# GPUs/goVideoCompressor

Hardware: AMD Instinct MI355X
Metric: encoded frames/sec (whole node), 1080p30->H.264 CRF23 (higher is better)
Workload: dtype uint8 (8-bit 4:2:0 samples, int32 transforms)

## Files before the change

csrc/common/h264_cabac.h:

```cpp
#pragma once
#include <cstddef>
#include <cstdint>

#include "h264_cabac_tables.h"
#include "h264_mb.h"
#include "h264_tables.h"

namespace mivc {
namespace h264 {

#if defined(__HIPCC__) && defined(__HIP_DEVICE_COMPILE__)
MIVC_HD int cabac_clz32(uint32_t v) { return __clz(static_cast<int>(v)); }
#else
MIVC_HD int cabac_clz32(uint32_t v) { return v ? __builtin_clz(v) : 32; }
#endif

struct CabacBuf {
  uint8_t* p;
  size_t cap;
  size_t n;
  int overflow;
  MIVC_HD void put(int b) {
    if (n < cap) p[n] = static_cast<uint8_t>(b);
    else overflow = 1;
// ... 963 lines not shown
    nbits += 3;
    drain();
    if (nbits > 0) {
      low <<= 8 - nbits;
      nbits = 8;
      drain();
    }
    out.finish();
  }
};

template <class Sink>
struct CabacPendingOut {
  Sink sink;
  int pend = -1, nff = 0;
  MIVC_HD bool byte9(uint32_t v) {
    const int b = static_cast<int>(v & 0xFFu);
    bool ok = true;
    if (v >> 8) {
      if (pend < 0) ok = false;
      if (nff > 0) {
        sink.put(pend + 1);
        for (int k = 0; k < nff - 1; ++k) sink.put(0);
        pend = 0;
        nff = 0;
      } else {
        pend += 1;
      }
    }
    if (b == 0xFF) {
      ++nff;
    } else {
      if (pend >= 0) {
        sink.put(pend);
        for (int k = 0; k < nff; ++k) sink.put(0xFF);
      }
      pend = b;
      nff = 0;
    }
    return ok;
  }
  MIVC_HD void finish() {
    if (pend >= 0) sink.put(pend);
    for (int k = 0; k < nff; ++k) sink.put(0xFF);
    pend = -1;
    nff = 0;
  }
};

struct CabacBufRef {
  CabacBuf* b;
  MIVC_HD void put(int v) { b->put(v); }
};

struct CabacSliceStats {
  int skipped = 0, intra = 0, inter = 0;
};

MIVC_HD size_t cabac_write_slice_data(const CabacSliceInfo& si, CabacNb* nb, uint8_t* states, CabacBuf* out,
                                      const MbHeader* hdr, const int16_t* coef, int n, CabacEncoder* enc_out = nullptr,
                                      CabacSliceStats* st = nullptr) {
  const int end = si.first_mb + n;
  for (int a = si.first_mb; a < end; ++a)
    cabac_prepare_mb(si, hdr, a, cabac_block_mask(hdr[a], coef + static_cast<size_t>(a) * kCoefPerMb), nb[a]);
  cabac_qp_chain(si, nb, n);
  CabacEncoder e;
  cabac_init_contexts(states, si.slice_type == SLICE_I ? 0 : 1 , si.slice_qp);
  e.init(states, out);
  CabacMbCoder<CabacEncoder> coder(e, si, nb);
  for (int a = si.first_mb; a < end; ++a) {
    coder.code_mb(a, hdr[a], coef + static_cast<size_t>(a) * kCoefPerMb, a == end - 1);
    if (st) {
      if (nb[a].skip) ++st->skipped;
      else if (mbk_is_intra(nb[a].kind)) ++st->intra;
      else ++st->inter;
    }
  }
  if (enc_out) *enc_out = e;
  return out->n;
}

inline size_t cabac_write_slice_data_symbols(const CabacSliceInfo& si, CabacNb* nb, uint8_t* states, CabacBuf* out,
                                             const MbHeader* hdr, const int16_t* coef, int n, uint16_t* syms,
                                             size_t cap_syms, int* nsyms_out) {
  const int end = si.first_mb + n;
  for (int a = end - 1; a >= si.first_mb; --a)
    cabac_prepare_mb(si, hdr, a, cabac_block_mask(hdr[a], coef + static_cast<size_t>(a) * kCoefPerMb), nb[a]);
  cabac_qp_chain(si, nb, n);
  size_t total = 0;
  for (int a = si.first_mb; a < end; ++a) {
    CabacSymbolPacker<CabacCountEmit> cnt;
    CabacMbCoder<CabacSymbolPacker<CabacCountEmit>> c1(cnt, si, nb);
    c1.code_mb(a, hdr[a], coef + static_cast<size_t>(a) * kCoefPerMb, a == end - 1);
    cnt.flush_bypass();
    if (total + cnt.out.n > cap_syms) return 0;
    CabacSymbolPacker<CabacStoreEmit> st;
    st.out.p = syms + total;
    CabacMbCoder<CabacSymbolPacker<CabacStoreEmit>> c2(st, si, nb);
    c2.code_mb(a, hdr[a], coef + static_cast<size_t>(a) * kCoefPerMb, a == end - 1);
    st.flush_bypass();
    total += st.out.n;
  }
  if (nsyms_out) *nsyms_out = static_cast<int>(total);
  if (total == 0 || syms[total - 1] != 0xC001u) return 0;
  cabac_init_contexts(states, si.slice_type == SLICE_I ? 0 : 1, si.slice_qp);
  CabacSymbolCoder<CabacPendingOut<CabacBufRef>> e;
  e.out.sink.b = out;
  e.init();
  for (size_t i = 0; i + 1 < total; ++i) {
    e.step_nodrain(syms[i], states, 1, &kCabacRangeLPS[0][0], kCabacTransLPS);
    if ((i & 3) == 3) e.drain();
  }
  e.finish();
  return e.bad ? 0 : out->n;
}

}
}
```

csrc/common/h264_mb.h:

```cpp
#pragma once
#include <cstdint>

#include "h264_tables.h"

namespace mivc {
namespace h264 {

enum SliceType { SLICE_P = 0, SLICE_B = 1, SLICE_I = 2 };

enum MbKind : uint8_t {
  MBK_I4x4 = 0,
  MBK_I16x16 = 1,
  MBK_P16x16 = 2,
  MBK_PSKIP = 3,
  MBK_IPCM = 4,
  MBK_P16x8 = 5,
  MBK_P8x16 = 6,
  MBK_P8x8 = 7,
  MBK_I8x8 = 8,
  MBK_B16x16 = 9,
  MBK_B16x8 = 10,
  MBK_B8x16 = 11,
  MBK_B8x8 = 12,
  MBK_BDIRECT = 13,
};

MIVC_HD bool mbk_is_intra(int k) { return k == MBK_I4x4 || k == MBK_I16x16 || k == MBK_IPCM || k == MBK_I8x8; }
MIVC_HD bool mbk_is_b(int k) { return k >= MBK_B16x16 && k <= MBK_BDIRECT; }

enum : int {
  COEF_LUMA = 0,
  COEF_LUMA_DC = 256,
  COEF_CHROMA_DC = 272,
  COEF_CHROMA_AC = 280,
  kCoefPerMb = 408,
};

enum : uint8_t {
  MBF_SKIP = 1,
  MBF_T8x8 = 2,
  MBF_SUB4 = 4,
};

enum : int { kSubEntry = 80 };

struct alignas(16) MbHeader {
  uint8_t kind;
  uint8_t cbp;
  int8_t qp;
  uint8_t i16_mode;
  uint8_t chroma_mode;
  uint8_t flags;
  uint8_t sub_direct;
  uint8_t pad0;
  int8_t ref[2][4];
  int16_t mv[2][4][2];
  uint8_t i4_modes[16];
};
static_assert(sizeof(MbHeader) == 64, "MbHeader must stay 64 bytes (GPU kernels write it)");

}
}
```

csrc/host/bindings.cc:

```cpp
#include <pybind11/numpy.h>
#include <pybind11/pybind11.h>
#include <pybind11/stl.h>

#include <atomic>
#include <cstring>
#include <stdexcept>
#include <string>
#include <thread>

#include "../common/h264_enc_math.h"
#include "annexb.h"
#include "cabac_writer.h"
#include "cavlc_writer.h"
#include "cpu_encoder.h"
#include "decode_batch.h"
#include "h264_decoder.h"
#include "hevc_codec.h"
#include "hevc_dec.h"
#include "lowres.h"

namespace mivc {
int selftest_i4_taps(int trials, uint32_t seed);
namespace hevc {
std::vector<uint8_t> hevc_exercise(uint32_t seed);
}
}

namespace py = pybind11;
using namespace mivc;
using namespace mivc::h264;

namespace {

py::bytes to_bytes(const std::vector<uint8_t>& v) {
  return py::bytes(reinterpret_cast<const char*>(v.data()), v.size());
}

template <class T>
T dget(const py::dict& d, const char* k, T def) {
  if (d.contains(k)) return d[k].cast<T>();
  return def;
}

EncoderConfig cfg_from(const py::dict& d) {
  EncoderConfig c;
  c.width = dget<int>(d, "width", 0);
  c.height = dget<int>(d, "height", 0);
  c.fps = dget<double>(d, "fps", 30.0);
  c.qp = dget<int>(d, "qp", 26);
  c.crf = dget<double>(d, "crf", -1.0);
  c.keyint = dget<int>(d, "keyint", 250);
  c.me_range = dget<int>(d, "me_range", 16);
  c.subpel = dget<int>(d, "subpel", 2);
  c.use_i4x4 = dget<int>(d, "i4x4", 1);
  c.deblock = dget<int>(d, "deblock", 1);
  c.chroma_qp_offset = dget<int>(d, "chroma_qp_offset", 0);
  c.vui = dget<int>(d, "vui", 1);
  c.cabac = dget<int>(d, "cabac", 0);
  c.t8x8 = dget<int>(d, "t8x8", 0);
  c.bframes = dget<int>(d, "bframes", 0);
  c.pyramid = dget<int>(d, "pyramid", 0);
  c.refs = dget<int>(d, "refs", 1);
  c.weighted_bipred = dget<int>(d, "weighted_bipred", 0);
  c.weightp = dget<int>(d, "weightp", 0);
  c.constrained_intra = dget<int>(d, "constrained_intra", 0);
  c.level_idc = dget<int>(d, "level_idc", 0);
  c.bit_depth = dget<int>(d, "bit_depth", 8);
  if (c.bit_depth < 8 || c.bit_depth > 14) throw std::runtime_error("bit_depth in 8..14");
  c.bit_depth_chroma = dget<int>(d, "bit_depth_chroma", 0);
  if (c.bit_depth_chroma != 0 && (c.bit_depth_chroma < 8 || c.bit_depth_chroma > 14))
    throw std::runtime_error("bit_depth_chroma in 8..14");
  c.cqm = dget<int>(d, "cqm", 0);
  c.cqm_coded = dget<int>(d, "cqm_coded", 0xFF);
  if (c.cqm < 0 || c.cqm > 3) throw std::runtime_error("cqm in 0..3");
  if (d.contains("cqm4")) {
    auto a = py::array_t<uint8_t, py::array::c_style | py::array::forcecast>::ensure(d["cqm4"]);
    if (!a || a.size() != 96) throw std::runtime_error("cqm4: 6 x 16 weights");
    std::memcpy(c.cqm4, a.data(), 96);
  }
  if (d.contains("cqm8")) {
    auto a = py::array_t<uint8_t, py::array::c_style | py::array::forcecast>::ensure(d["cqm8"]);
    if (!a || a.size() != 128) throw std::runtime_error("cqm8: 2 x 64 weights");
    std::memcpy(c.cqm8, a.data(), 128);
  }
  if (c.refs < 1 || c.refs > 16) throw std::runtime_error("refs must be in 1..16");
  return c;
}

py::dict picture_to_dict(const DecodedPicture& p) {
  py::dict d;
  d["width"] = p.width;
  d["height"] = p.height;
  d["coded_width"] = p.coded_width;
  d["coded_height"] = p.coded_height;
// ... 520 lines not shown
    size_t bits = bw.bit_pos();
    bw.align_zero();
    return py::make_tuple(to_bytes(bw.bytes()), bits, tc);
  });
  m.def("table", [](const std::string& name) {
    std::vector<std::vector<int>> out;
    auto row = [&](const uint8_t* p, int n) { out.emplace_back(p, p + n); };
    if (name == "coeff_token_len") for (int t = 0; t < 4; ++t) row(kCoeffTokenLen[t], 68);
    else if (name == "coeff_token_bits") for (int t = 0; t < 4; ++t) row(kCoeffTokenBits[t], 68);
    else if (name == "chroma_dc_coeff_token") { row(kChromaDcCoeffTokenLen, 20); row(kChromaDcCoeffTokenBits, 20); }
    else if (name == "total_zeros_len") for (int t = 0; t < 15; ++t) row(kTotalZerosLen[t], 16);
    else if (name == "total_zeros_bits") for (int t = 0; t < 15; ++t) row(kTotalZerosBits[t], 16);
    else if (name == "chroma_dc_total_zeros_len") for (int t = 0; t < 3; ++t) row(kChromaDcTotalZerosLen[t], 4);
    else if (name == "chroma_dc_total_zeros_bits") for (int t = 0; t < 3; ++t) row(kChromaDcTotalZerosBits[t], 4);
    else if (name == "run_before_len") for (int t = 0; t < 7; ++t) row(kRunBeforeLen[t], 15);
    else if (name == "run_before_bits") for (int t = 0; t < 7; ++t) row(kRunBeforeBits[t], 15);
    else if (name == "intra_cbp") row(kGolombToIntraCbp, 48);
    else if (name == "inter_cbp") row(kGolombToInterCbp, 48);
    else if (name == "zigzag") row(kZigzag4x4, 16);
    else if (name == "lambda") out.emplace_back(kLambda, kLambda + 52);
    else if (name == "hevc_dct32") {
      for (int k = 0; k < 32; ++k) {
        std::vector<int> r(32);
        for (int n = 0; n < 32; ++n) r[n] = hevc::dct_coef(k, n);
        out.push_back(r);
      }
    }
    else throw std::runtime_error("unknown table " + name);
    return out;
  });

  m.def("selftest_i4_taps", &mivc::selftest_i4_taps);

  m.def("parameter_sets", [](const py::dict& cfg) {
    EncoderConfig c = cfg_from(cfg);
    return to_bytes(write_parameter_sets(make_sps(c), make_pps(c)));
  });

  m.def(
      "write_slice",
      [](const py::dict& cfg, const py::dict& fp, py::array_t<uint8_t, py::array::c_style> hdr,
         py::array_t<int16_t, py::array::c_style> coef) {
        EncoderConfig c = cfg_from(cfg);
        SPS sps = make_sps(c);
        PPS pps = make_pps(c);
        int nmb = sps.width_mbs * sps.height_mbs;
        if (hdr.size() != static_cast<py::ssize_t>(nmb * sizeof(MbHeader))) throw std::runtime_error("header array has wrong size");
        if (coef.size() != static_cast<py::ssize_t>(nmb) * kCoefPerMb) throw std::runtime_error("coef array has wrong size");
        SliceHeader sh = slice_header_from(c, sps, pps, fp);
        const int num = dget<int>(fp, "num_mbs", nmb - sh.first_mb);
        if (sh.first_mb < 0 || num < 1 || sh.first_mb + num > nmb) throw std::runtime_error("write_slice: bad MB range");
        SliceStats st;
        std::vector<uint8_t> nal;
        {
          py::gil_scoped_release rel;
          const MbHeader* mh = reinterpret_cast<const MbHeader*>(hdr.data());
          nal = pps.entropy_coding_mode ? write_slice_nal_cabac(sps, pps, sh, mh, coef.data(), num, &st)
                                        : write_slice_nal(sps, pps, sh, mh, coef.data(), num, &st);
        }
        py::dict stats;
        stats["bits"] = st.bits;
        stats["skipped"] = st.skipped;
        stats["intra"] = st.intra;
        stats["coded_inter"] = st.coded_inter;
        return py::make_tuple(to_bytes(nal), stats);
      },
      py::arg("cfg"), py::arg("frame"), py::arg("hdr"), py::arg("coef"));

  m.def("cabac_slice_data_two_ways", [](const py::dict& cfg, const py::dict& fp, py::array_t<uint8_t, py::array::c_style> hdr,
                                         py::array_t<int16_t, py::array::c_style> coef) {
    EncoderConfig c = cfg_from(cfg);
    c.cabac = 1;
    SPS sps = make_sps(c);
    PPS pps = make_pps(c);
    int nmb = sps.width_mbs * sps.height_mbs;
    if (hdr.size() != static_cast<py::ssize_t>(nmb * sizeof(MbHeader))) throw std::runtime_error("header array has wrong size");
    if (coef.size() != static_cast<py::ssize_t>(nmb) * kCoefPerMb) throw std::runtime_error("coef array has wrong size");
    SliceHeader sh = slice_header_from(c, sps, pps, fp);
    const MbHeader* mh = reinterpret_cast<const MbHeader*>(hdr.data());
    std::vector<uint8_t> a = cabac_slice_data(sps, pps, sh, mh, coef.data(), nmb);
    int nsyms = 0;
    std::vector<uint8_t> b = cabac_slice_data_symbols(sps, pps, sh, mh, coef.data(), nmb, &nsyms);
    return py::make_tuple(to_bytes(a), to_bytes(b), nsyms);
  });

  m.def(
      "decode",
      [](py::bytes data, bool skip_deblock) {
        std::string s = data;
        Decoder dec;
        dec.set_skip_deblock(skip_deblock);
        {
          py::gil_scoped_release rel;
          dec.decode(reinterpret_cast<const uint8_t*>(s.data()), s.size());
          dec.flush();
        }
        py::list out;
        for (const DecodedPicture& p : dec.out()) out.append(picture_to_dict(p));
        return out;
      },
      py::arg("data"), py::arg("skip_deblock") = false);

  m.def(
      "parse",
      [](const std::vector<py::bytes>& segments, int threads) {
        std::vector<std::string> in;
        for (const py::bytes& b : segments) in.emplace_back(b);
        std::vector<ParsedSegment> res;
        {
          py::gil_scoped_release rel;
          res = h264_parse_many(in, threads);
        }
        py::list out;
        for (ParsedSegment& r : res) out.append(segment_to_dict(r));
        return out;
      },
      py::arg("segments"), py::arg("threads") = 1);

  py::class_<H264Batch>(m, "H264Batch")
      .def("__len__", [](const H264Batch& b) { return b.segs.size(); })
      .def("info", [](const H264Batch& b, int i) { return segment_info(b.segs.at(i)); })
      .def("segment", [](H264Batch& b, int i) { return segment_to_dict(b.segs.at(i)); })
      .def("layout",
           [](const H264Batch& b, int t, const std::vector<int>& slots, int nmb) {
             H264StepLayout L = b.layout(t, slots, nmb);
             py::dict d;
             d["hdr"] = L.hdr;
             d["mask"] = L.mask;
             d["off"] = L.off;
             d["bs"] = L.bs;
             d["wp"] = L.wp;
             d["coef"] = L.coef;
             d["sub"] = L.sub;
             d["total"] = L.total;
             return d;
           })
      .def("pack",
           [](const H264Batch& b, int t, const std::vector<int>& slots, int nmb, uintptr_t dst, size_t capacity,
              int threads) {
             H264StepLayout L = b.layout(t, slots, nmb);
             if (L.total > capacity) throw std::invalid_argument("H264Batch.pack: buffer too small");
             py::gil_scoped_release rel;
             b.pack(t, slots, nmb, reinterpret_cast<uint8_t*>(dst), threads);
           },
           py::arg("t"), py::arg("slots"), py::arg("nmb"), py::arg("dst"), py::arg("capacity"), py::arg("threads") = 4);
  m.def(
      "parse_batch",
      [](const std::vector<py::bytes>& segments, int threads) {
        std::vector<std::string> in;
        for (const py::bytes& b : segments) in.emplace_back(b);
        auto* batch = new H264Batch();
        {
          py::gil_scoped_release rel;
          batch->segs = h264_parse_many(in, threads);
        }
        return batch;
      },
      py::arg("segments"), py::arg("threads") = 1, py::return_value_policy::take_ownership);

  m.def("hevc_parameter_sets", [](const py::dict& cfg) { return to_bytes(hevc::hevc_parameter_sets(hevc_cfg_from(cfg))); });
  m.def(
      "hevc_write_slice",
      [](const py::dict& cfg, const py::dict& fp, py::array_t<uint8_t, py::array::c_style> ctu,
         py::array_t<uint8_t, py::array::c_style> cu, py::array_t<int16_t, py::array::c_style> cy,
         py::array_t<int16_t, py::array::c_style> cb, py::array_t<int16_t, py::array::c_style> cr) {
        hevc::HevcConfig c = hevc_cfg_from(cfg);
// ... 593 lines not shown
```

csrc/host/cabac_writer.cc:

```cpp
#include "cabac_writer.h"

#include <stdexcept>

#include "../common/h264_cabac.h"

namespace mivc {
namespace h264 {

std::vector<uint8_t> cabac_slice_data(const SPS& sps, const PPS& pps, const SliceHeader& sh, const MbHeader* mbs,
                                      const int16_t* coef, int num_mbs, SliceStats* stats) {
  if (!pps.entropy_coding_mode) throw std::runtime_error("CABAC writer called with a CAVLC PPS");
  if (sh.cabac_init_idc != 0) throw std::runtime_error("CABAC writer codes cabac_init_idc 0 only");
  if (pps.constrained_intra_pred) throw std::runtime_error("CABAC writer: constrained intra prediction is CAVLC-only");
  const int nmb = sps.width_mbs * sps.height_mbs;
  if (sh.first_mb < 0 || num_mbs <= 0 || sh.first_mb + num_mbs > nmb) throw std::runtime_error("bad MB range");
  for (int a = sh.first_mb; a < sh.first_mb + num_mbs; ++a) {
    const int k = mbs[a].kind;
    if (k == MBK_IPCM) throw std::runtime_error("I_PCM records are not written by the CABAC writer");
    if (sh.slice_type == SLICE_I && !mbk_is_intra(k)) throw std::runtime_error("inter MB in an I slice");
    if (sh.slice_type == SLICE_P && mbk_is_b(k)) throw std::runtime_error("B MB in a P slice");
    if (sh.slice_type == SLICE_B && !mbk_is_intra(k) && !mbk_is_b(k)) throw std::runtime_error("P MB in a B slice");
    if (k == MBK_I8x8 && !pps.transform_8x8_mode) throw std::runtime_error("I8x8 MB without transform_8x8_mode");
  }
  CabacSliceInfo si{};
  si.slice_type = sh.slice_type;
  si.wmb = sps.width_mbs;
  si.hmb = sps.height_mbs;
  si.first_mb = sh.first_mb;
  si.num_ref[0] = sh.num_ref_idx_l0_active;
  si.num_ref[1] = sh.num_ref_idx_l1_active;
  si.t8x8_mode = pps.transform_8x8_mode;
  si.slice_qp = pps.pic_init_qp + sh.slice_qp_delta;
  std::vector<CabacNb> nb(static_cast<size_t>(nmb));
  std::vector<uint8_t> out(static_cast<size_t>(num_mbs) * 160 + 4096);
  uint8_t states[kCabacContexts];
  for (int attempt = 0; attempt < 2; ++attempt) {
    CabacBuf buf{out.data(), out.size(), 0, 0};
    CabacEncoder e;
    CabacSliceStats st{};
    cabac_write_slice_data(si, nb.data(), states, &buf, mbs, coef, num_mbs, &e, &st);
    if (e.bad) throw std::runtime_error("CABAC carry past the start of the slice");
    if (!buf.overflow) {
      out.resize(buf.n);
      if (stats) {
        stats->skipped = st.skipped;
        stats->intra = st.intra;
        stats->coded_inter = st.inter;
      }
      return out;
    }
    out.assign(buf.n + 64, 0);
  }
  throw std::runtime_error("CABAC output buffer overflow");
}

std::vector<uint8_t> cabac_slice_data_symbols(const SPS& sps, const PPS& pps, const SliceHeader& sh, const MbHeader* mbs,
                                              const int16_t* coef, int num_mbs, int* nsyms) {
  const int nmb = sps.width_mbs * sps.height_mbs;
  CabacSliceInfo si{};
  si.slice_type = sh.slice_type;
  si.wmb = sps.width_mbs;
  si.hmb = sps.height_mbs;
  si.first_mb = sh.first_mb;
  si.num_ref[0] = sh.num_ref_idx_l0_active;
  si.num_ref[1] = sh.num_ref_idx_l1_active;
  si.t8x8_mode = pps.transform_8x8_mode;
  si.slice_qp = pps.pic_init_qp + sh.slice_qp_delta;
  std::vector<CabacNb> nb(static_cast<size_t>(nmb));
  std::vector<uint16_t> syms(static_cast<size_t>(num_mbs) * 20000 + 1024);
  std::vector<uint8_t> out(static_cast<size_t>(num_mbs) * 4000 + 4096);
  uint8_t states[kCabacContexts];
  CabacBuf buf{out.data(), out.size(), 0, 0};
  cabac_write_slice_data_symbols(si, nb.data(), states, &buf, mbs, coef, num_mbs, syms.data(), syms.size(), nsyms);
  if (buf.overflow) throw std::runtime_error("CABAC symbol path overflow");
  out.resize(buf.n);
  return out;
}

std::vector<uint8_t> write_slice_nal_cabac(const SPS& sps, const PPS& pps, const SliceHeader& sh, const MbHeader* mbs,
                                           const int16_t* coef, int num_mbs, SliceStats* stats) {
  BitWriter bw;
  write_slice_header(bw, sh, sps, pps);
  while (!bw.byte_aligned()) bw.put_bit(1);
  std::vector<uint8_t> data = cabac_slice_data(sps, pps, sh, mbs, coef, num_mbs, stats);
  bw.append_bytes(data.data(), data.size());
  std::vector<uint8_t> nal;
  nal.reserve(bw.bytes().size() + bw.bytes().size() / 64 + 16);
  append_nal(nal, sh.nal_ref_idc, sh.nal_unit_type, bw.bytes());
  if (stats) stats->bits = static_cast<int>(nal.size() * 8);
  return nal;
}

}
}
```

csrc/host/cabac_writer.h:

```cpp
#pragma once
#include <cstdint>
#include <vector>

#include "../common/h264_mb.h"
#include "cavlc_writer.h"
#include "h264_syntax.h"

namespace mivc {
namespace h264 {

std::vector<uint8_t> write_slice_nal_cabac(const SPS& sps, const PPS& pps, const SliceHeader& sh, const MbHeader* mbs,
                                           const int16_t* coef, int num_mbs, SliceStats* stats = nullptr);

std::vector<uint8_t> cabac_slice_data(const SPS& sps, const PPS& pps, const SliceHeader& sh, const MbHeader* mbs,
                                      const int16_t* coef, int num_mbs, SliceStats* stats = nullptr);

std::vector<uint8_t> cabac_slice_data_symbols(const SPS& sps, const PPS& pps, const SliceHeader& sh, const MbHeader* mbs,
                                              const int16_t* coef, int num_mbs, int* nsyms);

}
}
```

csrc/kernels/bindings_hip.cc:

```cpp
#include <pybind11/pybind11.h>
#include <pybind11/stl.h>

#include <cstdint>
#include <stdexcept>
#include <vector>

#include "../common/hevc_ctu_coder.h"
#include "hevc_decode.h"
#include "route.h"

namespace py = pybind11;

extern "C" {
long long mivc_hevc_entropy_state_bytes(int W, int H);
int mivc_launch_hevc_entropy(const void* pic, int B, const int* qp, const void* ctu, const void* cu, const void* col,
                             const unsigned long long* nzmap, const int16_t* cy, const int16_t* cb, const int16_t* cr,
                             uint8_t* state, long long state_bytes, uint8_t* out, unsigned cap, unsigned* sizes,
                             int* errs, unsigned long long* offs, unsigned long long* offs_host, uint8_t* dst,
                             unsigned long long dst_cap, int* overflow, void* stream, unsigned long long* prof,
                             int* gprog, void* gctx);
int mivc_launch_hevc_decode(const mivc::gpu::HevcDecParams* p, int stage, void* stream);
void mivc_launch_synth(void* y, void* u, void* v, int width, int height, int slots, int frames, int frame0,
                       uint32_t seed, int bit_depth, int slot0, void* stream, int kind);
void mivc_launch_prep(const uint8_t* in_y, const uint8_t* in_u, const uint8_t* in_v, int w, int h,
                      int64_t in_stride_y, int64_t in_stride_c, int nframes, uint8_t* out_y, uint8_t* out_u,
                      uint8_t* out_v, int ow, int oh, int W, int H, void* stream, const int* fsel);
void mivc_launch_rgb_to_i420(const uint8_t* rgb, int w, int h, int nframes, uint8_t* y, uint8_t* u, uint8_t* v,
                             void* stream);
void mivc_launch_me(int B, int wmb, int hmb, const uint8_t* src_y, const uint8_t* ref_y, const int16_t* pred_mv,
                    int16_t* out_mv, int* out_cost, uint8_t* out_pred, int* out_intra_cost, const int* qp, int range,
                    int subpel, uint8_t* hp, const int8_t* aq, int planes_ready, int early_sad, void* stream,
                    const int* gate_cost, int gate_thresh, const int16_t* cost_mv, const void* route, int nbuf,
                    int role, int want, const int16_t* seed_mv);
void mivc_launch_me_ref_select(int B, int wmb, int hmb, int nref, int16_t* mv, int16_t* mv8, int* cost, uint8_t* pred,
                               const int16_t* xmv, const int* xcost, const uint8_t* xpred, int8_t* mref, const int* qp,
                               const int8_t* aq, void* stream, const void* route);
void mivc_launch_b_spatial(int B, int wmb, int hmb, void* hdr, const void* col, const uint8_t* src, const uint8_t* ref1,
                           const uint8_t* hp1, const uint8_t* const* ref0k, const uint8_t* const* hp0k, const int* w1,
                           int nref, uint8_t* pred_out, int* err, void* stream, const int* intra_cost, int* cost,
                           const int* qp, const int8_t* aq, int bias, const void* route, int nbuf);
void mivc_launch_b_direct(int B, int wmb, int hmb, const void* col, const int* dsf, const int* direct_copy, int nref,
                          int16_t* dmv, int8_t* dref, int16_t* pm0, int16_t* pm1, void* stream, const void* route,
                          int nbuf, uint8_t* czero, const int8_t* cmap);
void mivc_launch_b_spatial_exact(int B, int wmb, int hmb, void* hdr, const int* intra_cost, const int* cost,
                                 const uint8_t* czero, uint8_t* fix, void* stream, const void* route, int slice_rows,
                                 int tol);
void mivc_launch_b_spatial_fixup(int B, int wmb, int hmb, const void* hdr, const uint8_t* fix, const uint8_t* ref0,
                                 const uint8_t* hp0, const uint8_t* ref1, const uint8_t* hp1, uint8_t* pred_out,
                                 void* stream, const void* route, int nbuf);
void mivc_launch_p_refine(int B, int wmb, int hmb, const uint8_t* src_y, const uint8_t* ref, const uint8_t* hp,
                          const int16_t* mv_in, int16_t* mv_out, int* cost, const int16_t* pm, uint8_t* pred,
                          const int* qp, const int8_t* aq, void* stream, const void* route, int nbuf,
                          const uint8_t* chg_in, uint8_t* chg_out);
void mivc_launch_b_decide(int B, int wmb, int hmb, const uint8_t* src_y, const uint8_t* ref0, const uint8_t* ref1,
                          const uint8_t* hp0, const uint8_t* hp1, const int16_t* mv0, const int16_t* mv1,
                          const int* cost0, const int* cost1, const uint8_t* pred0, const uint8_t* pred1,
                          const int16_t* pm0, const int16_t* pm1, const int16_t* dmv, const int* qp, const int8_t* aq,
                          void* hdr, uint8_t* pred_out, int* cost_out, void* stream, const int* w1, int nref,
                          const int8_t* dref, const uint8_t* const* ref0k, const uint8_t* const* hp0k,
                          int direct_only, int bparts, int have_direct, int spatial, int dbias, const void* route,
                          int nbuf, const uint8_t* czero);
void mivc_launch_aq_offsets(int B, int wmb, int hmb, const uint8_t* sy, const uint8_t* su, const uint8_t* sv,
                            float strength, const float* extra, long long extra_stride, int8_t* out, void* stream,
                            const void* route);
void mivc_launch_mbtree(int B, int F, int lbw, int lbh, const int* blk_cost, const int* blk_mv, void* prop,
                        float strength, float* out, void* stream);
void mivc_launch_qp_fixup(int B, int wmb, int hmb, void* hdr, const int16_t* coef, const uint8_t* nz, uint8_t* flags,
                          const int* slice_qp, void* stream, int slice_rows, const uint8_t* pre, const void* route);
int mivc_launch_prep_aq(const uint8_t* in_y, const uint8_t* in_u, const uint8_t* in_v, int w, int h, int64_t in_stride_y,
                        int64_t in_stride_c, int B, uint8_t* out_y, uint8_t* out_u, uint8_t* out_v, int W, int H,
                        const int* fsel, float strength, const float* extra, long long extra_stride, int8_t* out,
                        void* stream, const void* route);
void mivc_launch_aq_terms(int B, int wmb, int hmb, const uint8_t* sy, const uint8_t* su, const uint8_t* sv, float* terms,
                          void* stream);
void mivc_launch_aq_auto_finish(int B, int nmb, const float* terms, int mode, float strength, const float* extra,
                                long long extra_stride, int8_t* out, void* stream, const void* route);
int mivc_launch_prep_aq_terms(const uint8_t* in_y, const uint8_t* in_u, const uint8_t* in_v, int w, int h,
                              int64_t in_stride_y, int64_t in_stride_c, int B, uint8_t* out_y, uint8_t* out_u,
                              uint8_t* out_v, int W, int H, const int* fsel, float* terms, void* stream);
void mivc_launch_me_halfpel(int B, int W, int H, const uint8_t* ref_y, uint8_t* hp, void* stream, const void* route,
                            int nbuf);
void mivc_launch_encode_inter(int B, int wmb, int hmb, const uint8_t* src_y, const uint8_t* src_u,
                              const uint8_t* src_v, const uint8_t* ref_y, const uint8_t* ref_u, const uint8_t* ref_v,
                              uint8_t* rec_y, uint8_t* rec_u, uint8_t* rec_v, const uint8_t* pred_y,
                              const int16_t* mv, const int* me_cost, const int* intra_cost, const int* qp,
                              int chroma_qp_offset, void* hdr, int16_t* coef, uint8_t* nz, uint8_t* intra_flag,
                              int* intra_count, const int8_t* aq, const uint8_t* ref1_u, const uint8_t* ref1_v,
                              int bmode, int t8, const int16_t* mv8, void* stream, const int* w1, int nref,
                              const uint8_t* const* xref_u, const uint8_t* const* xref_v, const int8_t* mref,
                              const int* wp, int trellis, float trellis_lambda, const void* route, int nbuf,
                              uint8_t* qp_flags);
void mivc_launch_wp_stats16(const uint16_t* y, const uint16_t* u, const uint16_t* v, int w, int h, int npics,
                            unsigned long long* out, void* stream);
void mivc_launch_wp_stats(const uint8_t* y, const uint8_t* u, const uint8_t* v, int w, int h, int npics,
                          unsigned long long* out, void* stream);
void mivc_launch_wp_src(const uint8_t* src, uint8_t* dst, const int* wt, int B, long long plane_bytes, void* stream);
void mivc_launch_p_part8(int B, int wmb, int hmb, const uint8_t* src_y, const uint8_t* ref, const uint8_t* hp,
                         const int16_t* mv, const int16_t* pm, int* cost, uint8_t* pred, int16_t* mv8, const int* qp,
                         const int8_t* aq, int overhead, int min_satd, void* stream, const void* route, int nbuf,
                         const int* bits16, const uint8_t* dir16);
void mivc_launch_encode_intra(int B, int wmb, int hmb, const uint8_t* src_y, const uint8_t* src_u,
                              const uint8_t* src_v, uint8_t* rec_y, uint8_t* rec_u, uint8_t* rec_v, const int* qp,
                              int chroma_qp_offset, void* hdr, int16_t* coef, uint8_t* nz,
                              const uint8_t* intra_flag, const int* intra_count, int* err, int use_i4x4,
                              const int8_t* aq, void* stream, int use_i8x8, const void* route, int nbuf,
                              int slice_rows, int trellis, float trellis_lambda, int* gprog, long long gprog_ints);
void mivc_launch_deblock(int B, int wmb, int hmb, uint8_t* rec_y, uint8_t* rec_u, uint8_t* rec_v, const void* hdr,
                         const uint8_t* nz, int chroma_qp_offset, int alpha_off, int beta_off, int* err,
                         void* stream, const void* route, int nbuf);
void mivc_launch_decode_picture_dpb(int B, int wmb, int hmb, int dpb_n, uint8_t* dpb_y, uint8_t* dpb_u, uint8_t* dpb_v,
                                    const int16_t* cur_idx, const int16_t* reftab, const int16_t* wp, const int16_t* sub,
                                    const void* hdr, const uint32_t* mask, const uint32_t* off,
                                    const int16_t* coef, const int8_t* run, int any_inter, int chroma_qp_offset,
                                    uint8_t* nz, int* err, void* stream);
void mivc_launch_deblock_dpb(int B, int wmb, int hmb, int dpb_n, uint8_t* dpb_y, uint8_t* dpb_u, uint8_t* dpb_v,
                             const int16_t* cur_idx, const void* hdr, const uint8_t* nz, const uint8_t* bs,
                             int chroma_qp_offset, int alpha_off, int beta_off, int* err, void* stream);
void mivc_launch_decode_picture_dpb16(int B, int wmb, int hmb, int dpb_n, uint16_t* dpb_y, uint16_t* dpb_u,
                                      uint16_t* dpb_v, const int16_t* cur_idx, const int16_t* reftab, const int16_t* wp,
                                      const int16_t* sub, const void* hdr, const uint32_t* mask, const uint32_t* off,
                                      const int16_t* coef, const int8_t* run, int any_inter, int chroma_qp_offset, int bd,
                                      uint8_t* nz, int* err, void* stream);
void mivc_launch_deblock_dpb16(int B, int wmb, int hmb, int dpb_n, uint16_t* dpb_y, uint16_t* dpb_u, uint16_t* dpb_v,
                               const int16_t* cur_idx, const void* hdr, const uint8_t* bs, int chroma_qp_offset,
                               int alpha_off, int beta_off, int bd, int* err, void* stream);
int mivc_launch_scale(const void* in, int w, int h, long long in_stride, long long in_pitch, void* out, int ow, int oh,
                      int W, int H, long long out_stride, long long out_pitch, int nframes, const int* fx,
                      const int16_t* cx, int tx, const int* fy, const int16_t* cy, int ty, int tile_w, int tile_h,
                      int in_cols, int in_rows, int bd, void* stream);
void mivc_launch_hevc_intra(int B, int W, int H, const uint16_t* sy, const uint16_t* su, const uint16_t* sv,
                            uint16_t* ry, uint16_t* ru, uint16_t* rv, void* ctu, void* cu, int16_t* cy, int16_t* cu_,
                            int16_t* cv, const int* qp, const int8_t* run, int* cand, int bd, int analyze, int recon,
                            int* err, int sdh, const uint8_t* ctb_mask, void* stream, int ctu64);
void mivc_launch_hevc_inter(int B, int W, int H, const uint16_t* sy, const uint16_t* su, const uint16_t* sv,
                            const uint16_t* fy, const uint16_t* fu, const uint16_t* fv, uint16_t* ry, uint16_t* ru,
                            uint16_t* rv, void* ctu, void* cu, int16_t* cy, int16_t* cu_, int16_t* cv, const int* qp,
                            const int8_t* run, const int* cand, const int16_t* mv, const int* me_cost, int bd,
                            int tu_split, int sdh, int intra_bias, void* stream, const int16_t* mvb,
                            const uint8_t* dirb, const uint16_t* f1y, const uint16_t* f1u, const uint16_t* f1v,
                            const int16_t* wp, const uint16_t* const* xref, const int16_t* mv8);
void mivc_launch_hevc_b(int mode, int B, int wmb, int hmb, const uint8_t* src_y, const uint8_t* ref0, const uint8_t* ref1,
                        const uint8_t* hp0, const uint8_t* hp1, const int16_t* mv0, const int16_t* mv1, const int* cost0,
                        const int* cost1, const int16_t* pm0, const int16_t* pm1, const int16_t* tmv, const uint8_t* tdir,
                        const int16_t* mvb_in, const uint8_t* dir_in, int16_t* mvb_out, uint8_t* dir_out, int* cost,
                        int* bits, const int* qp, const int8_t* aq, void* stream, int bslice, int max_merge, int ctu64, const uint8_t* chg_in, uint8_t* chg_out,
                        int nref0, const uint8_t* const* xref, const uint8_t* const* xhp, const int16_t* xmv,
                        const int* xcost, const int16_t* xpm);
void mivc_launch_hevc_deblock(int B, int W, int H, int bd, uint16_t* y, uint16_t* u, uint16_t* v, const void* cu,
                              const void* ctu, const int8_t* run, void* stream);
void mivc_launch_hevc_aq(int B, int W, int H, int bd, const uint16_t* sy, const uint16_t* su, const uint16_t* sv,
                         const int* qp, float strength, const float* extra, long long extra_stride, int extra_rows,
                         int* ctb_qp, int8_t* mb_aq, void* stream);
void mivc_launch_hevc_pack_levels(int B, int W, int H, const int16_t* cy, const int16_t* cb, const int16_t* cr,
                                  unsigned long long* nzmap, int* cnt, unsigned* off, long long cap_blocks, int16_t* out,
                                  int* err, void* stream);
void mivc_launch_hevc_merge_refine(int B, int wmb, int hmb, const uint8_t* src_y, const uint8_t* ref, const uint8_t* hp,
                                   const int16_t* mv_in, int16_t* mv_out, int* cost, const int16_t* pm, const int* qp,
                                   const int8_t* aq, void* stream);
void mivc_launch_hevc_aq_terms(int B, int W, int H, int bd, const uint16_t* sy, const uint16_t* su, const uint16_t* sv,
                               float* terms, void* stream);
void mivc_launch_hevc_aq_auto_finish(int B, int W, int H, const float* terms, const int* qp, int mode, float strength,
                                     const float* extra, long long extra_stride, int extra_rows, int* ctb_qp,
                                     int8_t* mb_aq, void* stream);
void mivc_launch_hevc_qp_fixup(int B, int W, int H, void* ctu, const void* cu, const int* qp, const int8_t* run,
                               int wpp, void* stream, int ctu64);
void mivc_launch_hevc_sao(int B, int W, int H, int bd, const uint16_t* dy, const uint16_t* du, const uint16_t* dv,
                          uint16_t* y, uint16_t* u, uint16_t* v, const uint16_t* sy, const uint16_t* su,
                          const uint16_t* sv, void* ctu, const int* qp, const int8_t* run, int enable, void* stream, int ctu64);
size_t mivc_cavlc_mb_bytes();
size_t mivc_cabac_nb_bytes();
int mivc_cabac_gap();
void mivc_launch_cabac_bin(int B, int wmb, int hmb, const void* hdr, const int16_t* coef, uint32_t* mask, void* nb,
                           int* cnt, long long* off, int* tot, uint16_t* pool, long long pool_cap,
                           long long* pool_used, long long* base, int* total, const int* slot_qp, int slice_type,
                           int num_ref_l0, int num_ref_l1, int t8x8_mode, int* err, void* stream, const void* route,
                           int slice_rows);
void mivc_launch_cabac_code(int L, int B, uint16_t* pool, const long long* base, const int* total,
                            const uint32_t* hdr_bits, const int* hdr_nbits, const int* slot_qp,
                            unsigned long long itypes, int* bytes, uint8_t* out, long long* out_off, int* err,
                            uint8_t* host_out, long long host_cap, void* stream);
void mivc_launch_cavlc(int B, int wmb, int hmb, const void* hdr, const int16_t* coef, void* mbs, int* len,
                       long long* off, int* trail, long long* total_bits, int* slot_bytes, uint32_t* words,
                       long long cap_words, const uint32_t* hdr_bits, const int* hdr_nbits, int pslice, int slice_qp,
                       const int* slot_qp, uint8_t* out, long long* out_off, const uint8_t* nz, void* stream);
void mivc_launch_satd_blocks(const uint8_t* src, const uint8_t* pred, int* out, int n, int mode, void* stream);
void mivc_launch_trellis_blocks(const int* w, int* out, int n, int qp, int mode, int skip_dc, void* stream);
void mivc_launch_sse(int B, int W, int H, int w, int h, const uint8_t* sy, const uint8_t* su, const uint8_t* sv,
                     const uint8_t* ry, const uint8_t* ru, const uint8_t* rv, unsigned long long* sse,
                     float* ssim_sum, void* stream, const void* route, int nbuf);
long long mivc_lookahead_low_bytes(int w, int h, int N);
int mivc_launch_lookahead_multi(const uint8_t* low, int w, int h, int N, int F, const int* blk_cost, const int* blk_mv,
                                int D, int range, unsigned long long* out, void* stream, const float* wt);
int mivc_launch_hevc_prep_frame(int B, const void* sy, const void* su, const void* sv, long long ss_y, long long ss_c,
                                int pitch_y, int pitch_c, int bps, int w, int h, uint16_t* dy, uint16_t* du,
                                uint16_t* dv, uint8_t* d8, int W, int H, int shift, int bd, void* stream);
int mivc_launch_hevc_proxy8(const uint16_t* src, uint8_t* dst, long long n, int shift, void* stream);
int mivc_launch_lookahead(const uint8_t* y, int w, int h, long long fstride, int N, int F, uint8_t* low,
                          unsigned long long* frame_cost, int* blk_cost, int* blk_mv, int range, void* stream,
                          uint8_t* low4, int* mv4, unsigned long long* cost4, float* wt, unsigned long long* wstats,
                          float thr_mean, float thr_scale, int stage);
long long mivc_lookahead_quarter_bytes(int w, int h, int N);
}

namespace {
template <class T>
T* P(uintptr_t p) {
  return reinterpret_cast<T*>(p);
}
void* S(uintptr_t s) { return reinterpret_cast<void*>(s); }
}

PYBIND11_MODULE(_hip, m) {
  m.doc() = "govideocompressor_amd gfx950 kernels (raw-pointer launch shims)";
  m.attr("arch") = "gfx950";
  m.def("route_bytes", []() { return static_cast<int>(sizeof(mivc::gpu::SlotRoute)); });

  m.def("synth", [](uintptr_t y, uintptr_t u, uintptr_t v, int w, int h, int slots, int frames, int frame0,
                    uint32_t seed, uintptr_t stream, int bit_depth, int slot0, int kind) {
    if (bit_depth != 8 && bit_depth != 10) throw std::invalid_argument("synth: bit_depth must be 8 or 10");
    if (kind < 0 || kind > 6) throw std::invalid_argument("synth: content kind 0..6");
    mivc_launch_synth(P<void>(y), P<void>(u), P<void>(v), w, h, slots, frames, frame0, seed, bit_depth, slot0,
                      S(stream), kind);
  }, py::arg("y"), py::arg("u"), py::arg("v"), py::arg("w"), py::arg("h"), py::arg("slots"), py::arg("frames"),
     py::arg("frame0"), py::arg("seed"), py::arg("stream"), py::arg("bit_depth") = 8, py::arg("slot0") = 0,
     py::arg("kind") = 0);
  m.def("prep", [](uintptr_t iy, uintptr_t iu, uintptr_t iv, int w, int h, int64_t sy, int64_t sc, int n,
                   uintptr_t oy, uintptr_t ou, uintptr_t ov, int ow, int oh, int W, int H, uintptr_t stream,
                   uintptr_t fsel) {
    if (ow != w || oh != h) throw std::invalid_argument("prep: resample with ops.scale (scale.hip) first");
    if (W < w || H < h || w < 2 || h < 2) throw std::invalid_argument("prep: bad geometry");
    mivc_launch_prep(P<uint8_t>(iy), P<uint8_t>(iu), P<uint8_t>(iv), w, h, sy, sc, n, P<uint8_t>(oy), P<uint8_t>(ou),
                     P<uint8_t>(ov), ow, oh, W, H, S(stream), P<int>(fsel));
  }, py::arg("iy"), py::arg("iu"), py::arg("iv"), py::arg("w"), py::arg("h"), py::arg("sy"), py::arg("sc"), py::arg("n"),
     py::arg("oy"), py::arg("ou"), py::arg("ov"), py::arg("ow"), py::arg("oh"), py::arg("W"), py::arg("H"),
     py::arg("stream"), py::arg("fsel") = 0);
  m.def("rgb_to_i420", [](uintptr_t rgb, int w, int h, int n, uintptr_t y, uintptr_t u, uintptr_t v,
                          uintptr_t stream) {
    mivc_launch_rgb_to_i420(P<uint8_t>(rgb), w, h, n, P<uint8_t>(y), P<uint8_t>(u), P<uint8_t>(v), S(stream));
  });
  m.def("me", [](int B, int wmb, int hmb, uintptr_t src, uintptr_t ref, uintptr_t pred_mv, uintptr_t out_mv,
                 uintptr_t out_cost, uintptr_t out_pred, uintptr_t out_intra, uintptr_t qp, int range, int subpel,
                 uintptr_t stream, uintptr_t hp, uintptr_t aq, int planes_ready, int early_sad, uintptr_t gate_cost,
                 int gate_thresh, uintptr_t cost_mv, uintptr_t route, int nbuf, int role, int want, uintptr_t seed_mv) {
    if (planes_ready && !hp) throw std::invalid_argument("me: planes_ready needs the hp buffer");
    if (route && (nbuf < 1 || role < 0 || role > 4 || (want != 0 && want != 1) || !planes_ready))
      throw std::invalid_argument("me: a routed search needs nbuf, a role (list-0 0..3 / list-1 4), want P/B and the planes");
    mivc_launch_me(B, wmb, hmb, P<uint8_t>(src), P<uint8_t>(ref), P<int16_t>(pred_mv), P<int16_t>(out_mv),
                   P<int>(out_cost), P<uint8_t>(out_pred), P<int>(out_intra), P<int>(qp), range, subpel,
                   P<uint8_t>(hp), P<int8_t>(aq), planes_ready, early_sad, S(stream), P<int>(gate_cost), gate_thresh,
                   P<int16_t>(cost_mv), P<void>(route), nbuf, role, want, P<int16_t>(seed_mv));
  }, py::arg("B"), py::arg("wmb"), py::arg("hmb"), py::arg("src"), py::arg("ref"), py::arg("pred_mv"),
     py::arg("out_mv"), py::arg("out_cost"), py::arg("out_pred"), py::arg("out_intra"), py::arg("qp"),
     py::arg("range"), py::arg("subpel"), py::arg("stream"), py::arg("hp") = 0, py::arg("aq") = 0,
     py::arg("planes_ready") = 0, py::arg("early_sad") = 0, py::arg("gate_cost") = 0, py::arg("gate_thresh") = 0,
     py::arg("cost_mv") = 0, py::arg("route") = 0, py::arg("nbuf") = 0, py::arg("role") = 0, py::arg("want") = 0,
     py::arg("seed_mv") = 0);
  m.def("me_ref_select", [](int B, int wmb, int hmb, int nref, uintptr_t mv, uintptr_t mv8, uintptr_t cost,
                            uintptr_t pred, uintptr_t xmv, uintptr_t xcost, uintptr_t xpred, uintptr_t mref,
                            uintptr_t qp, uintptr_t aq, uintptr_t stream, uintptr_t route) {
    if (nref < 2 || nref > 4) throw std::invalid_argument("me_ref_select: nref in 2..4");
    mivc_launch_me_ref_select(B, wmb, hmb, nref, P<int16_t>(mv), P<int16_t>(mv8), P<int>(cost), P<uint8_t>(pred),
                              P<int16_t>(xmv), P<int>(xcost), P<uint8_t>(xpred), P<int8_t>(mref), P<int>(qp),
                              P<int8_t>(aq), S(stream), P<void>(route));
  }, py::arg("B"), py::arg("wmb"), py::arg("hmb"), py::arg("nref"), py::arg("mv"), py::arg("mv8"), py::arg("cost"),
     py::arg("pred"), py::arg("xmv"), py::arg("xcost"), py::arg("xpred"), py::arg("mref"), py::arg("qp"), py::arg("aq"),
     py::arg("stream"), py::arg("route") = 0);
  m.def("b_spatial", [](int B, int wmb, int hmb, uintptr_t hdr, uintptr_t col, uintptr_t src, uintptr_t ref1,
                        uintptr_t hp1, std::vector<uintptr_t> ref0k, std::vector<uintptr_t> hp0k, std::vector<int> w1,
                        uintptr_t pred_out, uintptr_t err, uintptr_t stream, uintptr_t intra_cost, uintptr_t cost,
                        uintptr_t qp, uintptr_t aq, int bias, uintptr_t route, int nbuf) {
    const size_t n = ref0k.size();
    if (n < 1 || n > 4 || hp0k.size() != n || w1.size() != n)
      throw std::invalid_argument("b_spatial: 1..4 list-0 pictures with planes and weights");
    if (hmb > 272 || wmb > 480) throw std::invalid_argument("b_spatial: at most 272 MB rows and 480 columns");
    const uint8_t* rk[4];
    const uint8_t* hk[4];
    for (size_t i = 0; i < n; ++i) {
      rk[i] = P<uint8_t>(ref0k[i]);
      hk[i] = P<uint8_t>(hp0k[i]);
    }
    mivc_launch_b_spatial(B, wmb, hmb, P<void>(hdr), P<void>(col), P<uint8_t>(src), P<uint8_t>(ref1), P<uint8_t>(hp1),
                          rk, hk, w1.data(), static_cast<int>(n), P<uint8_t>(pred_out), P<int>(err), S(stream),
                          P<int>(intra_cost), P<int>(cost), P<int>(qp), P<int8_t>(aq), bias, P<void>(route), nbuf);
  }, py::arg("B"), py::arg("wmb"), py::arg("hmb"), py::arg("hdr"), py::arg("col"), py::arg("src"), py::arg("ref1"),
     py::arg("hp1"), py::arg("ref0k"), py::arg("hp0k"), py::arg("w1"), py::arg("pred_out"), py::arg("err"),
     py::arg("stream"), py::arg("intra_cost"), py::arg("cost"), py::arg("qp"), py::arg("aq"), py::arg("bias"),
     py::arg("route") = 0, py::arg("nbuf") = 0);
  m.def("b_direct", [](int B, int wmb, int hmb, uintptr_t col, std::vector<int> dsf, std::vector<int> direct_copy,
                       uintptr_t dmv, uintptr_t pm0, uintptr_t pm1, uintptr_t stream, uintptr_t dref, uintptr_t route,
                       int nbuf, uintptr_t czero, uintptr_t cmap) {
    if (dsf.empty() || dsf.size() > 4 || dsf.size() != direct_copy.size())
      throw std::invalid_argument("b_direct: one (dsf, direct_copy) pair per list-0 picture, at most 4");
    if (route && nbuf < 1) throw std::invalid_argument("b_direct: a routed launch needs the pool size");
    if (cmap && !dref) throw std::invalid_argument("b_direct: a co-located map needs the dref output");
    mivc_launch_b_direct(B, wmb, hmb, P<void>(col), dsf.data(), direct_copy.data(), static_cast<int>(dsf.size()),
                         P<int16_t>(dmv), P<int8_t>(dref), P<int16_t>(pm0), P<int16_t>(pm1), S(stream), P<void>(route),
                         nbuf, P<uint8_t>(czero), P<int8_t>(cmap));
// ... 48 lines not shown
      hk[i] = P<uint8_t>(hp0k[i - 1]);
    }
    mivc_launch_b_decide(B, wmb, hmb, P<uint8_t>(src), P<uint8_t>(ref0), P<uint8_t>(ref1), P<uint8_t>(hp0),
                         P<uint8_t>(hp1), P<int16_t>(mv0), P<int16_t>(mv1), P<int>(cost0), P<int>(cost1),
                         P<uint8_t>(pred0), P<uint8_t>(pred1), P<int16_t>(pm0), P<int16_t>(pm1), P<int16_t>(dmv),
                         P<int>(qp), P<int8_t>(aq), P<void>(hdr), P<uint8_t>(pred_out), P<int>(cost_out), S(stream),
                         w1.data(), static_cast<int>(n), (n > 1 || route) ? P<int8_t>(dref) : nullptr, rk, hk, direct_only,
                         bparts, have_direct, spatial, dbias, P<void>(route), nbuf, P<uint8_t>(czero));
  }, py::arg("B"), py::arg("wmb"), py::arg("hmb"), py::arg("src"), py::arg("ref0"), py::arg("ref1"), py::arg("hp0"),
     py::arg("hp1"), py::arg("mv0"), py::arg("mv1"), py::arg("cost0"), py::arg("cost1"), py::arg("pred0"),
     py::arg("pred1"), py::arg("pm0"), py::arg("pm1"), py::arg("dmv"), py::arg("qp"), py::arg("aq"), py::arg("hdr"),
     py::arg("pred_out"), py::arg("cost_out"), py::arg("stream"), py::arg("w1") = std::vector<int>{32},
     py::arg("dref") = 0, py::arg("ref0k") = std::vector<uintptr_t>{}, py::arg("hp0k") = std::vector<uintptr_t>{},
     py::arg("direct_only") = 0, py::arg("bparts") = 0, py::arg("have_direct") = 0, py::arg("spatial") = 0, py::arg("dbias") = 0,
     py::arg("route") = 0, py::arg("nbuf") = 0, py::arg("czero") = 0);
  m.def("aq_offsets", [](int B, int wmb, int hmb, uintptr_t sy, uintptr_t su, uintptr_t sv, float strength,
                         uintptr_t out, uintptr_t stream, uintptr_t extra, long long extra_stride, uintptr_t route) {
    mivc_launch_aq_offsets(B, wmb, hmb, P<uint8_t>(sy), P<uint8_t>(su), P<uint8_t>(sv), strength, P<float>(extra),
                           extra_stride, P<int8_t>(out), S(stream), P<void>(route));
  }, py::arg("B"), py::arg("wmb"), py::arg("hmb"), py::arg("sy"), py::arg("su"), py::arg("sv"), py::arg("strength"),
     py::arg("out"), py::arg("stream"), py::arg("extra") = 0, py::arg("extra_stride") = 0, py::arg("route") = 0);
  m.def("mbtree", [](int B, int F, int lbw, int lbh, uintptr_t blk_cost, uintptr_t blk_mv, uintptr_t prop,
                     float strength, uintptr_t out, uintptr_t stream) {
    mivc_launch_mbtree(B, F, lbw, lbh, P<int>(blk_cost), P<int>(blk_mv), P<void>(prop), strength, P<float>(out),
                       S(stream));
  });
  m.def("qp_fixup", [](int B, int wmb, int hmb, uintptr_t hdr, uintptr_t coef, uintptr_t nz, uintptr_t flags,
                       uintptr_t slice_qp, uintptr_t stream, int slice_rows, uintptr_t pre, uintptr_t route) {
    if ((pre != 0) != (route != 0)) throw std::invalid_argument("qp_fixup: pre and route go together");
    mivc_launch_qp_fixup(B, wmb, hmb, P<void>(hdr), P<int16_t>(coef), P<uint8_t>(nz), P<uint8_t>(flags),
                         P<int>(slice_qp), S(stream), slice_rows, P<uint8_t>(pre), P<void>(route));
  }, py::arg("B"), py::arg("wmb"), py::arg("hmb"), py::arg("hdr"), py::arg("coef"), py::arg("nz"), py::arg("flags"),
     py::arg("slice_qp"), py::arg("stream"), py::arg("slice_rows") = 0, py::arg("pre") = 0, py::arg("route") = 0);
  m.def("prep_aq", [](uintptr_t iy, uintptr_t iu, uintptr_t iv, int w, int h, int64_t sy, int64_t sc, int n,
                      uintptr_t oy, uintptr_t ou, uintptr_t ov, int W, int H, float strength, uintptr_t out,
                      uintptr_t stream, uintptr_t fsel, uintptr_t extra, long long extra_stride, uintptr_t route) {
    if (W < w || H < h || w < 2 || h < 2) throw std::invalid_argument("prep_aq: bad geometry");
    if (!out) throw std::invalid_argument("prep_aq: needs the offset buffer");
    return mivc_launch_prep_aq(P<uint8_t>(iy), P<uint8_t>(iu), P<uint8_t>(iv), w, h, sy, sc, n, P<uint8_t>(oy),
                               P<uint8_t>(ou), P<uint8_t>(ov), W, H, P<int>(fsel), strength, P<float>(extra),
                               extra_stride, P<int8_t>(out), S(stream), P<void>(route)) != 0;
  }, py::arg("iy"), py::arg("iu"), py::arg("iv"), py::arg("w"), py::arg("h"), py::arg("sy"), py::arg("sc"), py::arg("n"),
     py::arg("oy"), py::arg("ou"), py::arg("ov"), py::arg("W"), py::arg("H"), py::arg("strength"), py::arg("out"),
     py::arg("stream"), py::arg("fsel") = 0, py::arg("extra") = 0, py::arg("extra_stride") = 0, py::arg("route") = 0);
  m.def("aq_terms", [](int B, int wmb, int hmb, uintptr_t sy, uintptr_t su, uintptr_t sv, uintptr_t terms,
                       uintptr_t stream) {
    if (B < 1 || wmb < 1 || hmb < 1) throw std::invalid_argument("aq_terms: bad geometry");
    if (!sy || !su || !sv || !terms) throw std::invalid_argument("aq_terms: needs the planes and the term buffer");
    mivc_launch_aq_terms(B, wmb, hmb, P<uint8_t>(sy), P<uint8_t>(su), P<uint8_t>(sv), P<float>(terms), S(stream));
  }, py::arg("B"), py::arg("wmb"), py::arg("hmb"), py::arg("sy"), py::arg("su"), py::arg("sv"), py::arg("terms"),
     py::arg("stream"));
  m.def("prep_aq_terms", [](uintptr_t iy, uintptr_t iu, uintptr_t iv, int w, int h, int64_t sy, int64_t sc, int n,
                            uintptr_t oy, uintptr_t ou, uintptr_t ov, int W, int H, uintptr_t terms, uintptr_t stream,
                            uintptr_t fsel) {
    if (W < w || H < h || w < 2 || h < 2 || n < 1) throw std::invalid_argument("prep_aq_terms: bad geometry");
    if (!terms) throw std::invalid_argument("prep_aq_terms: needs the term buffer");
    return mivc_launch_prep_aq_terms(P<uint8_t>(iy), P<uint8_t>(iu), P<uint8_t>(iv), w, h, sy, sc, n, P<uint8_t>(oy),
                                     P<uint8_t>(ou), P<uint8_t>(ov), W, H, P<int>(fsel), P<float>(terms),
                                     S(stream)) != 0;
  }, py::arg("iy"), py::arg("iu"), py::arg("iv"), py::arg("w"), py::arg("h"), py::arg("sy"), py::arg("sc"), py::arg("n"),
     py::arg("oy"), py::arg("ou"), py::arg("ov"), py::arg("W"), py::arg("H"), py::arg("terms"), py::arg("stream"),
     py::arg("fsel") = 0);
  m.def("aq_auto_finish", [](int B, int nmb, uintptr_t terms, int mode, float strength, uintptr_t out, uintptr_t stream,
                             uintptr_t extra, long long extra_stride, uintptr_t route) {
    if (B < 1 || nmb < 1) throw std::invalid_argument("aq_auto_finish: bad geometry");
    if (mode != 2 && mode != 3) throw std::invalid_argument("aq_auto_finish: mode must be 2 or 3");
    if (!terms || !out) throw std::invalid_argument("aq_auto_finish: needs the term and the offset buffer");
    mivc_launch_aq_auto_finish(B, nmb, P<float>(terms), mode, strength, P<float>(extra), extra_stride, P<int8_t>(out),
                               S(stream), P<void>(route));
  }, py::arg("B"), py::arg("nmb"), py::arg("terms"), py::arg("mode"), py::arg("strength"), py::arg("out"),
     py::arg("stream"), py::arg("extra") = 0, py::arg("extra_stride") = 0, py::arg("route") = 0);
  m.def("me_halfpel", [](int B, int W, int H, uintptr_t ref, uintptr_t hp, uintptr_t stream, uintptr_t route, int nbuf) {
    if (route && nbuf < 1) throw std::invalid_argument("me_halfpel: a routed launch needs the pool size");
    mivc_launch_me_halfpel(B, W, H, P<uint8_t>(ref), P<uint8_t>(hp), S(stream), P<void>(route), nbuf);
  }, py::arg("B"), py::arg("W"), py::arg("H"), py::arg("ref"), py::arg("hp"), py::arg("stream"), py::arg("route") = 0,
     py::arg("nbuf") = 0);
  m.def("encode_inter",
        [](int B, int wmb, int hmb, uintptr_t sy, uintptr_t su, uintptr_t sv, uintptr_t fy, uintptr_t fu,
           uintptr_t fv, uintptr_t ry, uintptr_t ru, uintptr_t rv, uintptr_t pred, uintptr_t mv, uintptr_t me_cost,
           uintptr_t intra_cost, uintptr_t qp, int cqo, uintptr_t hdr, uintptr_t coef, uintptr_t nz,
           uintptr_t intra_flag, uintptr_t intra_count, uintptr_t stream, uintptr_t aq, uintptr_t ref1_u,
           uintptr_t ref1_v, int bmode, int t8, uintptr_t mv8, std::vector<int> w1, std::vector<uintptr_t> xref_u,
           std::vector<uintptr_t> xref_v, uintptr_t mref, uintptr_t wp, int trellis, float trellis_lambda,
           uintptr_t route, int nbuf, uintptr_t qp_flags) {
          if (bmode && (!ref1_u || !ref1_v)) throw std::invalid_argument("encode_inter: B mode needs the list-1 chroma");
          const size_t n = xref_u.size() + 1;
          if (n > 4 || xref_v.size() != xref_u.size()) throw std::invalid_argument("encode_inter: at most 4 list-0 pictures");
          if ((n > 1 || route) && !bmode && !mref)
            throw std::invalid_argument("encode_inter: P pictures with several references need mref");
          if (route && (nbuf < 1 || n > 1)) throw std::invalid_argument("encode_inter: routed launches take pools");
          std::vector<int> w(n, w1.empty() ? 32 : w1[0]);
          for (size_t i = 0; i < n && i < w1.size(); ++i) w[i] = w1[i];
          const uint8_t* xu[4] = {nullptr, nullptr, nullptr, nullptr};
          const uint8_t* xv[4] = {nullptr, nullptr, nullptr, nullptr};
          for (size_t i = 1; i < n; ++i) {
            xu[i] = P<uint8_t>(xref_u[i - 1]);
            xv[i] = P<uint8_t>(xref_v[i - 1]);
          }
          mivc_launch_encode_inter(B, wmb, hmb, P<uint8_t>(sy), P<uint8_t>(su), P<uint8_t>(sv), P<uint8_t>(fy),
                                   P<uint8_t>(fu), P<uint8_t>(fv), P<uint8_t>(ry), P<uint8_t>(ru), P<uint8_t>(rv),
                                   P<uint8_t>(pred), P<int16_t>(mv), P<int>(me_cost), P<int>(intra_cost), P<int>(qp),
                                   cqo, P<void>(hdr), P<int16_t>(coef), P<uint8_t>(nz), P<uint8_t>(intra_flag),
                                   P<int>(intra_count), P<int8_t>(aq), P<uint8_t>(ref1_u), P<uint8_t>(ref1_v), bmode,
                                   t8, P<int16_t>(mv8), S(stream), w.data(), static_cast<int>(n), xu, xv,
                                   bmode ? nullptr : P<int8_t>(mref), P<int>(wp), trellis, trellis_lambda, P<void>(route),
                                   nbuf, P<uint8_t>(qp_flags));
        }, py::arg("B"), py::arg("wmb"), py::arg("hmb"), py::arg("sy"), py::arg("su"), py::arg("sv"), py::arg("fy"),
        py::arg("fu"), py::arg("fv"), py::arg("ry"), py::arg("ru"), py::arg("rv"), py::arg("pred"), py::arg("mv"),
        py::arg("me_cost"), py::arg("intra_cost"), py::arg("qp"), py::arg("cqo"), py::arg("hdr"), py::arg("coef"),
        py::arg("nz"), py::arg("intra_flag"), py::arg("intra_count"), py::arg("stream"), py::arg("aq") = 0,
        py::arg("ref1_u") = 0, py::arg("ref1_v") = 0, py::arg("bmode") = 0, py::arg("t8") = 0, py::arg("mv8") = 0,
        py::arg("w1") = std::vector<int>{32}, py::arg("xref_u") = std::vector<uintptr_t>{},
        py::arg("xref_v") = std::vector<uintptr_t>{}, py::arg("mref") = 0, py::arg("wp") = 0, py::arg("trellis") = 0,
        py::arg("trellis_lambda") = 1.0f, py::arg("route") = 0, py::arg("nbuf") = 0, py::arg("qp_flags") = 0);
  m.def("wp_stats16", [](uintptr_t y, uintptr_t u, uintptr_t v, int w, int h, int npics, uintptr_t out, uintptr_t stream) {
    if (w % 2 || h % 2 || npics <= 0) throw std::invalid_argument("wp_stats16: even picture sizes, npics > 0");
    mivc_launch_wp_stats16(P<uint16_t>(y), P<uint16_t>(u), P<uint16_t>(v), w, h, npics, P<unsigned long long>(out),
                           S(stream));
  });
  m.def("wp_stats", [](uintptr_t y, uintptr_t u, uintptr_t v, int w, int h, int npics, uintptr_t out, uintptr_t stream) {
    if (w % 2 || h % 2 || (w * h) % 4) throw std::invalid_argument("wp_stats: even picture sizes");
    mivc_launch_wp_stats(P<uint8_t>(y), P<uint8_t>(u), P<uint8_t>(v), w, h, npics, P<unsigned long long>(out),
                         S(stream));
  });
  m.def("wp_src", [](uintptr_t src, uintptr_t dst, uintptr_t wt, int B, long long plane_bytes, uintptr_t stream) {
    if (plane_bytes % 4) throw std::invalid_argument("wp_src: plane size must be a multiple of 4");
    mivc_launch_wp_src(P<uint8_t>(src), P<uint8_t>(dst), P<int>(wt), B, plane_bytes, S(stream));
  });
  m.def("p_part8", [](int B, int wmb, int hmb, uintptr_t src, uintptr_t ref, uintptr_t hp, uintptr_t mv, uintptr_t pm,
                      uintptr_t cost, uintptr_t pred, uintptr_t mv8, uintptr_t qp, uintptr_t aq, int overhead,
                      int min_satd, uintptr_t stream, uintptr_t route, int nbuf, uintptr_t bits16, uintptr_t dir16) {
    if (!hp || !mv8) throw std::invalid_argument("p_part8: needs the half-sample planes and an mv8 buffer");
    if (!pred && !bits16) throw std::invalid_argument("p_part8: the H.264 form rewrites pred");
    mivc_launch_p_part8(B, wmb, hmb, P<uint8_t>(src), P<uint8_t>(ref), P<uint8_t>(hp), P<int16_t>(mv), P<int16_t>(pm),
                        P<int>(cost), P<uint8_t>(pred), P<int16_t>(mv8), P<int>(qp), P<int8_t>(aq), overhead, min_satd,
                        S(stream), P<void>(route), nbuf, P<int>(bits16), P<uint8_t>(dir16));
  }, py::arg("B"), py::arg("wmb"), py::arg("hmb"), py::arg("src"), py::arg("ref"), py::arg("hp"), py::arg("mv"),
     py::arg("pm"), py::arg("cost"), py::arg("pred"), py::arg("mv8"), py::arg("qp"), py::arg("aq"), py::arg("overhead"),
     py::arg("min_satd"), py::arg("stream"), py::arg("route") = 0, py::arg("nbuf") = 0, py::arg("bits16") = 0,
     py::arg("dir16") = 0);
  m.def("encode_intra", [](int B, int wmb, int hmb, uintptr_t sy, uintptr_t su, uintptr_t sv, uintptr_t ry,
                           uintptr_t ru, uintptr_t rv, uintptr_t qp, int cqo, uintptr_t hdr, uintptr_t coef,
                           uintptr_t nz, uintptr_t intra_flag, uintptr_t intra_count, uintptr_t err, int use_i4x4,
                           uintptr_t stream, uintptr_t aq, int use_i8x8, uintptr_t route, int nbuf, int slice_rows,
                           int trellis, float trellis_lambda, uintptr_t gprog, long long gprog_ints) {
    mivc_launch_encode_intra(B, wmb, hmb, P<uint8_t>(sy), P<uint8_t>(su), P<uint8_t>(sv), P<uint8_t>(ry),
                             P<uint8_t>(ru), P<uint8_t>(rv), P<int>(qp), cqo, P<void>(hdr), P<int16_t>(coef),
                             P<uint8_t>(nz), P<uint8_t>(intra_flag), P<int>(intra_count), P<int>(err), use_i4x4,
                             P<int8_t>(aq), S(stream), use_i8x8, P<void>(route), nbuf, slice_rows, trellis,
                             trellis_lambda, P<int>(gprog), gprog_ints);
  }, py::arg("B"), py::arg("wmb"), py::arg("hmb"), py::arg("sy"), py::arg("su"), py::arg("sv"), py::arg("ry"),
     py::arg("ru"), py::arg("rv"), py::arg("qp"), py::arg("cqo"), py::arg("hdr"), py::arg("coef"), py::arg("nz"),
     py::arg("intra_flag"), py::arg("intra_count"), py::arg("err"), py::arg("use_i4x4"), py::arg("stream"),
     py::arg("aq") = 0, py::arg("use_i8x8") = 0, py::arg("route") = 0, py::arg("nbuf") = 0, py::arg("slice_rows") = 0,
     py::arg("trellis") = 0, py::arg("trellis_lambda") = 1.0f, py::arg("gprog") = 0, py::arg("gprog_ints") = 0);
  m.def("deblock", [](int B, int wmb, int hmb, uintptr_t ry, uintptr_t ru, uintptr_t rv, uintptr_t hdr, uintptr_t nz,
                      int cqo, int alpha_off, int beta_off, uintptr_t err, uintptr_t stream, uintptr_t route, int nbuf) {
    mivc_launch_deblock(B, wmb, hmb, P<uint8_t>(ry), P<uint8_t>(ru), P<uint8_t>(rv), P<void>(hdr), P<uint8_t>(nz),
                        cqo, alpha_off, beta_off, P<int>(err), S(stream), P<void>(route), nbuf);
  }, py::arg("B"), py::arg("wmb"), py::arg("hmb"), py::arg("ry"), py::arg("ru"), py::arg("rv"), py::arg("hdr"),
     py::arg("nz"), py::arg("cqo"), py::arg("alpha_off"), py::arg("beta_off"), py::arg("err"), py::arg("stream"),
     py::arg("route") = 0, py::arg("nbuf") = 0);
  m.def("decode_picture_dpb", [](int B, int wmb, int hmb, int dpb_n, uintptr_t y, uintptr_t u, uintptr_t v,
                                 uintptr_t cur_idx, uintptr_t reftab, uintptr_t wp, uintptr_t sub,
                                 uintptr_t hdr, uintptr_t mask, uintptr_t off, uintptr_t coef, uintptr_t run,
                                 int any_inter, int cqo, uintptr_t nz, uintptr_t err, uintptr_t stream) {
    if (dpb_n < 1 || dpb_n > 32767) throw std::invalid_argument("decode_picture_dpb: dpb_n must be 1..32767");
    mivc_launch_decode_picture_dpb(B, wmb, hmb, dpb_n, P<uint8_t>(y), P<uint8_t>(u), P<uint8_t>(v), P<int16_t>(cur_idx),
                                   P<int16_t>(reftab), P<int16_t>(wp), P<int16_t>(sub), P<void>(hdr),
                                   P<uint32_t>(mask), P<uint32_t>(off), P<int16_t>(coef), P<int8_t>(run), any_inter,
                                   cqo, P<uint8_t>(nz), P<int>(err), S(stream));
  });
  m.def("deblock_dpb", [](int B, int wmb, int hmb, int dpb_n, uintptr_t y, uintptr_t u, uintptr_t v, uintptr_t cur_idx,
                          uintptr_t hdr, uintptr_t nz, uintptr_t bs, int cqo, int alpha_off, int beta_off, uintptr_t err,
                          uintptr_t stream) {
    if (dpb_n < 1 || dpb_n > 32767) throw std::invalid_argument("deblock_dpb: dpb_n must be 1..32767");
    mivc_launch_deblock_dpb(B, wmb, hmb, dpb_n, P<uint8_t>(y), P<uint8_t>(u), P<uint8_t>(v), P<int16_t>(cur_idx),
                            P<void>(hdr), P<uint8_t>(nz), P<uint8_t>(bs), cqo, alpha_off, beta_off, P<int>(err),
                            S(stream));
  });
  m.def("decode_picture_dpb16", [](int B, int wmb, int hmb, int dpb_n, uintptr_t y, uintptr_t u, uintptr_t v,
                                   uintptr_t cur_idx, uintptr_t reftab, uintptr_t wp, uintptr_t sub,
                                   uintptr_t hdr, uintptr_t mask, uintptr_t off, uintptr_t coef, uintptr_t run,
                                   int any_inter, int cqo, int bit_depth, uintptr_t nz, uintptr_t err,
                                   uintptr_t stream) {
    if (dpb_n < 1 || dpb_n > 32767) throw std::invalid_argument("decode_picture_dpb16: dpb_n must be 1..32767");
    if (bit_depth != 9 && bit_depth != 10) throw std::invalid_argument("decode_picture_dpb16: bit_depth must be 9 or 10");
    mivc_launch_decode_picture_dpb16(B, wmb, hmb, dpb_n, P<uint16_t>(y), P<uint16_t>(u), P<uint16_t>(v),
                                     P<int16_t>(cur_idx), P<int16_t>(reftab), P<int16_t>(wp), P<int16_t>(sub),
                                     P<void>(hdr), P<uint32_t>(mask), P<uint32_t>(off), P<int16_t>(coef),
                                     P<int8_t>(run), any_inter, cqo, bit_depth, P<uint8_t>(nz), P<int>(err), S(stream));
  });
  m.def("deblock_dpb16", [](int B, int wmb, int hmb, int dpb_n, uintptr_t y, uintptr_t u, uintptr_t v,
                            uintptr_t cur_idx, uintptr_t hdr, uintptr_t bs, int cqo, int alpha_off, int beta_off,
                            int bit_depth, uintptr_t err, uintptr_t stream) {
    if (dpb_n < 1 || dpb_n > 32767) throw std::invalid_argument("deblock_dpb16: dpb_n must be 1..32767");
    if (bit_depth != 9 && bit_depth != 10) throw std::invalid_argument("deblock_dpb16: bit_depth must be 9 or 10");
// ... 175 lines not shown
  m.def("hevc_qp_fixup", [](int B, int W, int H, uintptr_t ctu, uintptr_t cu, uintptr_t qp, uintptr_t run, int wpp,
                            uintptr_t stream, int ctu64) {
    mivc_launch_hevc_qp_fixup(B, W, H, P<void>(ctu), P<void>(cu), P<int>(qp), P<int8_t>(run), wpp, S(stream), ctu64);
  }, py::arg("B"), py::arg("W"), py::arg("H"), py::arg("ctu"), py::arg("cu"), py::arg("qp"), py::arg("run"),
     py::arg("wpp"), py::arg("stream"), py::arg("ctu64") = 0);
  m.def("hevc_sao", [](int B, int W, int H, int bd, uintptr_t dy, uintptr_t du, uintptr_t dv, uintptr_t y, uintptr_t u,
                       uintptr_t v, uintptr_t sy, uintptr_t su, uintptr_t sv, uintptr_t ctu, uintptr_t qp, uintptr_t run,
                       int enable, uintptr_t stream, int ctu64) {
    mivc_launch_hevc_sao(B, W, H, bd, P<uint16_t>(dy), P<uint16_t>(du), P<uint16_t>(dv), P<uint16_t>(y), P<uint16_t>(u),
                         P<uint16_t>(v), P<uint16_t>(sy), P<uint16_t>(su), P<uint16_t>(sv), P<void>(ctu), P<int>(qp),
                         P<int8_t>(run), enable, S(stream), ctu64);
  }, py::arg("B"), py::arg("W"), py::arg("H"), py::arg("bd"), py::arg("dy"), py::arg("du"), py::arg("dv"), py::arg("y"),
     py::arg("u"), py::arg("v"), py::arg("sy"), py::arg("su"), py::arg("sv"), py::arg("ctu"), py::arg("qp"),
     py::arg("run"), py::arg("enable"), py::arg("stream"), py::arg("ctu64") = 0);
  m.def("hevc_decode_stage", [](const py::dict& p, int stage, uintptr_t stream) {
    mivc::gpu::HevcDecParams a{};
    auto I = [&](const char* k) -> long long {
      if (!p.contains(k)) throw std::runtime_error(std::string("hevc_decode_stage: missing ") + k);
      return p[k].cast<long long>();
    };
    auto Q = [&](const char* k) -> uintptr_t { return p.contains(k) ? p[k].cast<uintptr_t>() : 0; };
    a.B = static_cast<int>(I("B"));
    a.W = static_cast<int>(I("W"));
    a.H = static_cast<int>(I("H"));
    a.D = static_cast<int>(I("D"));
    a.bd = static_cast<int>(I("bd"));
    a.bdc = static_cast<int>(I("bdc"));
    a.log2_ctb = static_cast<int>(I("log2_ctb"));
    a.wctb = static_cast<int>(I("wctb"));
    a.hctb = static_cast<int>(I("hctb"));
    const std::vector<uintptr_t> dpb = p["dpb"].cast<std::vector<uintptr_t>>();
    const std::vector<uintptr_t> res = p["res"].cast<std::vector<uintptr_t>>();
    const std::vector<uintptr_t> tmp = p["tmp"].cast<std::vector<uintptr_t>>();
    for (int c = 0; c < 3; ++c) {
      a.dpb[c] = reinterpret_cast<uint16_t*>(dpb.at(c));
      a.res[c] = reinterpret_cast<int16_t*>(res.at(c));
      a.tmp[c] = reinterpret_cast<uint16_t*>(tmp.at(c));
    }
    a.cur = P<int8_t>(Q("cur"));
    a.reftab = P<int8_t>(Q("reftab"));
    a.run = P<int8_t>(Q("run"));
    a.meta = P<int32_t>(Q("meta"));
    a.mvf = P<uint8_t>(Q("mvf"));
    a.mvf_sub = P<uint8_t>(Q("mvf_sub"));
    a.bs = P<uint8_t>(Q("bs"));
    a.ctbs = P<uint8_t>(Q("ctbs"));
    a.sao = P<uint8_t>(Q("sao"));
    a.tus = P<uint8_t>(Q("tus"));
    a.tu_base = P<int32_t>(Q("tu_base"));
    a.coefs = P<int16_t>(Q("coefs"));
    a.coef_base = P<int64_t>(Q("coef_base"));
    a.ops = P<uint8_t>(Q("ops"));
    a.op_base = P<int32_t>(Q("op_base"));
    a.ctb_ops = P<uint32_t>(Q("ctb_ops"));
    a.refs = P<uint8_t>(Q("refs"));
    a.ref_base = P<int32_t>(Q("ref_base"));
    a.slices = P<uint8_t>(Q("slices"));
    a.slice_base = P<int32_t>(Q("slice_base"));
    a.scaling = P<uint8_t>(Q("scaling"));
    a.max_tus = static_cast<int>(I("max_tus"));
    a.err = P<int>(Q("err"));
    if (p.contains("out")) {
      const std::vector<uintptr_t> out = p["out"].cast<std::vector<uintptr_t>>();
      for (int c = 0; c < 3; ++c) a.out[c] = reinterpret_cast<void*>(out.at(c));
      a.out_u8 = static_cast<int>(I("out_u8"));
      a.Fo = static_cast<int>(I("Fo"));
      a.out_w = static_cast<int>(I("out_w"));
      a.out_h = static_cast<int>(I("out_h"));
      a.crop_x = static_cast<int>(I("crop_x"));
      a.crop_y = static_cast<int>(I("crop_y"));
      a.disp = P<int16_t>(Q("disp"));
    }
    if (!a.cur || !a.run || !a.meta || !a.mvf || !a.err) throw std::runtime_error("hevc_decode_stage: null pointer");
    const int r = mivc_launch_hevc_decode(&a, stage, S(stream));
    if (r != 0) throw std::runtime_error("hevc_decode_stage: launch failed (" + std::to_string(r) + ")");
  });
  m.def("cavlc_mb_bytes", []() { return mivc_cavlc_mb_bytes(); });
  m.def("cabac_nb_bytes", []() { return mivc_cabac_nb_bytes(); });
  m.def("cabac_gap", []() { return mivc_cabac_gap(); });
  m.def("cabac_bin", [](int B, int wmb, int hmb, uintptr_t hdr, uintptr_t coef, uintptr_t mask, uintptr_t nb,
                        uintptr_t cnt, uintptr_t off, uintptr_t tot, uintptr_t pool, long long pool_cap,
                        uintptr_t pool_used, uintptr_t base, uintptr_t total, uintptr_t slot_qp, int slice_type,
                        int num_ref_l0, int num_ref_l1, int t8x8_mode, uintptr_t err, uintptr_t stream, uintptr_t route,
                        int slice_rows) {
    if ((pool & 15) != 0) throw std::invalid_argument("cabac_bin: symbol pool must be 16-byte aligned");
    if (B < 1 || wmb < 1 || hmb < 1) throw std::invalid_argument("cabac_bin: bad geometry");
    mivc_launch_cabac_bin(B, wmb, hmb, P<void>(hdr), P<int16_t>(coef), P<uint32_t>(mask), P<void>(nb), P<int>(cnt),
                          P<long long>(off), P<int>(tot), P<uint16_t>(pool), pool_cap, P<long long>(pool_used),
                          P<long long>(base), P<int>(total), P<int>(slot_qp), slice_type, num_ref_l0, num_ref_l1,
                          t8x8_mode, P<int>(err), S(stream), P<void>(route), slice_rows);
  }, py::arg("B"), py::arg("wmb"), py::arg("hmb"), py::arg("hdr"), py::arg("coef"), py::arg("mask"), py::arg("nb"),
     py::arg("cnt"), py::arg("off"), py::arg("tot"), py::arg("pool"), py::arg("pool_cap"), py::arg("pool_used"),
     py::arg("base"), py::arg("total"), py::arg("slot_qp"), py::arg("slice_type"), py::arg("num_ref_l0"),
     py::arg("num_ref_l1"), py::arg("t8x8_mode"), py::arg("err"), py::arg("stream"), py::arg("route") = 0,
     py::arg("slice_rows") = 0);
  m.def("cabac_code", [](int L, int B, uintptr_t pool, uintptr_t base, uintptr_t total, uintptr_t hdr_bits,
                         uintptr_t hdr_nbits, uintptr_t slot_qp, unsigned long long itypes, uintptr_t bytes,
                         uintptr_t out, uintptr_t out_off, uintptr_t err, uintptr_t stream, uintptr_t host_out,
                         long long host_cap) {
    if (B < 1 || L < 1 || L % B != 0 || L / B > 64) throw std::invalid_argument("cabac_code: L must be G * B, G <= 64");
    if ((out & 15) || (host_out & 15)) throw std::invalid_argument("cabac_code: output buffers must be 16-byte aligned");
    mivc_launch_cabac_code(L, B, P<uint16_t>(pool), P<long long>(base), P<int>(total), P<uint32_t>(hdr_bits),
                           P<int>(hdr_nbits), P<int>(slot_qp), itypes, P<int>(bytes), P<uint8_t>(out),
                           P<long long>(out_off), P<int>(err), P<uint8_t>(host_out), host_cap, S(stream));
  });
  m.def("cavlc", [](int B, int wmb, int hmb, uintptr_t hdr, uintptr_t coef, uintptr_t mbs, uintptr_t len, uintptr_t off,
                    uintptr_t trail, uintptr_t total_bits, uintptr_t slot_bytes, uintptr_t words, long long cap_words,
                    uintptr_t hdr_bits, uintptr_t hdr_nbits, int pslice, int slice_qp, uintptr_t slot_qp,
                    uintptr_t out, uintptr_t out_off, uintptr_t stream, uintptr_t nz) {
    mivc_launch_cavlc(B, wmb, hmb, P<void>(hdr), P<int16_t>(coef), P<void>(mbs), P<int>(len), P<long long>(off),
                      P<int>(trail), P<long long>(total_bits), P<int>(slot_bytes), P<uint32_t>(words), cap_words,
                      P<uint32_t>(hdr_bits), P<int>(hdr_nbits), pslice, slice_qp, P<int>(slot_qp), P<uint8_t>(out),
                      P<long long>(out_off), P<uint8_t>(nz), S(stream));
  }, py::arg("B"), py::arg("wmb"), py::arg("hmb"), py::arg("hdr"), py::arg("coef"), py::arg("mbs"), py::arg("len"),
     py::arg("off"), py::arg("trail"), py::arg("total_bits"), py::arg("slot_bytes"), py::arg("words"),
     py::arg("cap_words"), py::arg("hdr_bits"), py::arg("hdr_nbits"), py::arg("pslice"), py::arg("slice_qp"),
     py::arg("slot_qp"), py::arg("out"), py::arg("out_off"), py::arg("stream"), py::arg("nz") = 0);
  m.def("sse", [](int B, int W, int H, int w, int h, uintptr_t sy, uintptr_t su, uintptr_t sv, uintptr_t ry,
                  uintptr_t ru, uintptr_t rv, uintptr_t sse, uintptr_t ssim, uintptr_t stream, uintptr_t route, int nbuf) {
    if (B <= 0 || W <= 0 || H <= 0 || W % 16 || H % 2) throw std::invalid_argument("sse: coded width must be a multiple of 16, height even");
    if (w < 2 || h < 2 || w > W || h > H || w % 2 || h % 2)
      throw std::invalid_argument("sse: the display window must be even and lie inside the coded size");
    if (route && nbuf < 1) throw std::invalid_argument("sse: a routed launch needs the pool size");
    mivc_launch_sse(B, W, H, w, h, P<uint8_t>(sy), P<uint8_t>(su), P<uint8_t>(sv), P<uint8_t>(ry), P<uint8_t>(ru),
                    P<uint8_t>(rv), P<unsigned long long>(sse), P<float>(ssim), S(stream), P<void>(route), nbuf);
  }, py::arg("B"), py::arg("W"), py::arg("H"), py::arg("w"), py::arg("h"), py::arg("sy"), py::arg("su"), py::arg("sv"),
     py::arg("ry"), py::arg("ru"), py::arg("rv"), py::arg("sse"), py::arg("ssim"), py::arg("stream"),
     py::arg("route") = 0, py::arg("nbuf") = 0);
  m.def("satd_blocks", [](uintptr_t src, uintptr_t pred, uintptr_t out, int n, int mode, uintptr_t stream) {
    if (n <= 0) throw std::invalid_argument("satd_blocks: n must be positive");
    mivc_launch_satd_blocks(P<uint8_t>(src), P<uint8_t>(pred), P<int>(out), n, mode, S(stream));
  });
  m.def("trellis_blocks", [](uintptr_t w, uintptr_t out, int n, int qp, int mode, int skip_dc, uintptr_t stream) {
    if (n <= 0 || qp < 0 || qp > 51) throw std::invalid_argument("trellis_blocks: n > 0, 0 <= qp <= 51");
    mivc_launch_trellis_blocks(P<int>(w), P<int>(out), n, qp, mode, skip_dc, S(stream));
  });
  m.def("lookahead_low_bytes", [](int w, int h, int n) { return mivc_lookahead_low_bytes(w, h, n); });
  m.def("lookahead_quarter_bytes", [](int w, int h, int n) { return mivc_lookahead_quarter_bytes(w, h, n); });
  m.def("lookahead_multi", [](uintptr_t low, int w, int h, int n, int f, uintptr_t blk_cost, uintptr_t blk_mv, int D,
                              int range, uintptr_t out, uintptr_t stream, uintptr_t wt) {
    const int r = mivc_launch_lookahead_multi(P<uint8_t>(low), w, h, n, f, P<int>(blk_cost), P<int>(blk_mv), D, range,
                                              P<unsigned long long>(out), S(stream), P<float>(wt));
    if (r != 0) throw std::invalid_argument("lookahead_multi: bad arguments (" + std::to_string(r) + ")");
  }, py::arg("low"), py::arg("w"), py::arg("h"), py::arg("n"), py::arg("f"), py::arg("blk_cost"), py::arg("blk_mv"),
     py::arg("D"), py::arg("range"), py::arg("out"), py::arg("stream"), py::arg("wt") = 0);
  m.def("lookahead", [](uintptr_t y, int w, int h, long long fstride, int n, int f, uintptr_t low, uintptr_t frame_cost,
                        uintptr_t blk_cost, int range, uintptr_t stream, uintptr_t blk_mv, uintptr_t low4, uintptr_t mv4,
                        uintptr_t cost4, uintptr_t wt, uintptr_t wstats, float thr_mean, float thr_scale, int stage) {
    int rc = mivc_launch_lookahead(P<uint8_t>(y), w, h, fstride, n, f, P<uint8_t>(low),
                                   P<unsigned long long>(frame_cost), P<int>(blk_cost), P<int>(blk_mv), range,
                                   S(stream), P<uint8_t>(low4), P<int>(mv4), P<unsigned long long>(cost4), P<float>(wt),
                                   P<unsigned long long>(wstats), thr_mean, thr_scale, stage);
    if (rc != 0) throw std::invalid_argument("lookahead: bad geometry or range (4, 6, 8)");
  }, py::arg("y"), py::arg("w"), py::arg("h"), py::arg("fstride"), py::arg("n"), py::arg("f"), py::arg("low"),
     py::arg("frame_cost"), py::arg("blk_cost"), py::arg("range"), py::arg("stream"), py::arg("blk_mv") = 0,
     py::arg("low4") = 0, py::arg("mv4") = 0, py::arg("cost4") = 0, py::arg("wt") = 0, py::arg("wstats") = 0,
     py::arg("thr_mean") = 2.0f, py::arg("thr_scale") = 0.08f, py::arg("stage") = 3);
}
```

csrc/kernels/cabac.hip:

```cpp
#include "kcommon.h"
#include "../common/h264_cabac.h"

namespace mivc {
namespace gpu {

using h264::CabacNb;
using h264::CabacSliceInfo;
using h264::MbHeader;

constexpr int kCabacGap = 64;
constexpr int kArithReadAhead = 160;

struct CabacBinArgs {
  Geom g;
  const MbHeader* hdr;
  const int16_t* coef;
  uint32_t* mask;
  CabacNb* nb;
  int* cnt;
  long long* off;
  int* tot;
  uint16_t* pool;
  long long pool_cap;
  long long* pool_used;
  long long* base;
  int* total;
  const int* slot_qp;
  int slice_type;
  int num_ref_l0, num_ref_l1;
  int t8x8_mode;
  int* err;
  const SlotRoute* rt;
  int slice_mbs, per_slot;
};

__device__ __forceinline__ int slice_first(const CabacBinArgs& a, int mb) { return (mb / a.slice_mbs) * a.slice_mbs; }
__device__ __forceinline__ int slice_end(const CabacBinArgs& a, int mb) {
  return min(slice_first(a, mb) + a.slice_mbs, a.g.nmb());
}
__device__ __forceinline__ int slice_index(const CabacBinArgs& a, int slot, int mb) {
  return slot * a.per_slot + mb / a.slice_mbs;
}

__device__ __forceinline__ CabacSliceInfo slice_info(const CabacBinArgs& a, int slot, int mb) {
  CabacSliceInfo si{};
  si.slice_type = a.rt ? a.rt[slot].kind : a.slice_type;
  si.wmb = a.g.wmb;
  si.hmb = a.g.hmb;
  si.first_mb = slice_first(a, mb);
  si.num_ref[0] = a.rt ? (a.rt[slot].kind == SK_I ? 1 : a.rt[slot].n0) : a.num_ref_l0;
  si.num_ref[1] = a.num_ref_l1;
  si.t8x8_mode = a.t8x8_mode;
  si.slice_qp = a.slot_qp[slot];
  return si;
}

constexpr int kMaskSpan = 16;

__global__ __launch_bounds__(64) void cabac_mask(CabacBinArgs a) {
  const Geom& g = a.g;
  const int lane = threadIdx.x, sub = lane & 31;
  const int slot = blockIdx.y;
  for (int it = 0; it < kMaskSpan; ++it) {
  const int mb = (blockIdx.x * kMaskSpan + it) * 2 + (lane >> 5);
  if ((blockIdx.x * kMaskSpan + it) * 2 >= g.nmb()) break;
  const bool live = mb < g.nmb();
  const size_t o = static_cast<size_t>(slot) * g.nmb() + (live ? mb : 0);
  const int16_t* c = a.coef + o * h264::kCoefPerMb;
  const bool i16 = a.hdr[o].kind == h264::MBK_I16x16;
  bool nz = false;
  if (sub < 16 || (sub >= 19 && sub < 27)) {
    const int16_t* p = sub < 16 ? c + h264::COEF_LUMA + sub * 16 : c + h264::COEF_CHROMA_AC + (sub - 19) * 16;
    const uint4 q0 = reinterpret_cast<const uint4*>(p)[0];
    const uint4 q1 = reinterpret_cast<const uint4*>(p)[1];
    const bool skip_dc = sub >= 19 || i16;
    nz = ((skip_dc ? (q0.x & 0xFFFF0000u) : q0.x) | q0.y | q0.z | q0.w | q1.x | q1.y | q1.z | q1.w) != 0;
  } else if (sub == 16) {
    const uint4 q0 = reinterpret_cast<const uint4*>(c + h264::COEF_LUMA_DC)[0];
    const uint4 q1 = reinterpret_cast<const uint4*>(c + h264::COEF_LUMA_DC)[1];
    nz = i16 && (q0.x | q0.y | q0.z | q0.w | q1.x | q1.y | q1.z | q1.w) != 0;
  } else if (sub == 17 || sub == 18) {
    const uint2 q = reinterpret_cast<const uint2*>(c + h264::COEF_CHROMA_DC)[sub - 17];
    nz = (q.x | q.y) != 0;
  }
  const unsigned long long bal = __ballot(nz);
  const uint32_t m = static_cast<uint32_t>((bal >> (lane & 32)) & 0x7FFFFFFull);
  if (live && sub == 0) a.mask[o] = m;
  }
}

static_assert(sizeof(CabacNb) % 16 == 0, "CabacNb rows leave as 16-byte chunks");
__global__ __launch_bounds__(64) void cabac_prep(CabacBinArgs a) {
  __shared__ __attribute__((aligned(16))) CabacNb s_nb[64];
  const int mb0 = blockIdx.x * 64, mb = mb0 + threadIdx.x, slot = blockIdx.y, nmb = a.g.nmb();
  const size_t base = static_cast<size_t>(slot) * nmb;
  if (mb < nmb) {
    const CabacSliceInfo si = slice_info(a, slot, mb);
    h264::cabac_prepare_mb(si, a.hdr + base, mb, a.mask[base + mb], s_nb[threadIdx.x]);
  }
  __syncthreads();
  const int n16 = min(64, nmb - mb0) * static_cast<int>(sizeof(CabacNb) / 16);
  const uint4* src = reinterpret_cast<const uint4*>(s_nb);
  uint4* dst = reinterpret_cast<uint4*>(a.nb + base + mb0);
  for (int i = threadIdx.x; i < n16; i += 64) dst[i] = src[i];
}

__device__ __forceinline__ long long wave_scan_add(long long v) {
  const int lane = threadIdx.x & 63;
#pragma unroll
  for (int o = 1; o < 64; o <<= 1) {
    const long long y = __shfl_up(v, o, 64);
    if (lane >= o) v += y;
  }
  return v;
}
__device__ __forceinline__ int wave_scan_max(int v) {
  const int lane = threadIdx.x & 63;
#pragma unroll
  for (int o = 1; o < 64; o <<= 1) {
    const int y = __shfl_up(v, o, 64);
    if (lane >= o) v = max(v, y);
  }
  return v;
}

__global__ __launch_bounds__(64) void cabac_chain(CabacBinArgs a) {
  const int slot = blockIdx.x / a.per_slot, first = (blockIdx.x - slot * a.per_slot) * a.slice_mbs;
  const int n = min(a.g.nmb() - first, a.slice_mbs), lane = threadIdx.x;
  CabacNb* nb = a.nb + static_cast<size_t>(slot) * a.g.nmb() + first;
  const int per = (n + 63) / 64;
  const int i0 = lane * per, i1 = min(n, i0 + per);
  auto has = [&](int i) { return !nb[i].skip && (nb[i].cbp != 0 || nb[i].kind == h264::MBK_I16x16); };
  int ld = -1;
  for (int i = i0; i < i1; ++i)
    if (has(i)) ld = i;
  const int incl = wave_scan_max(ld);
  ld = __shfl_up(incl, 1, 64);
  if (lane == 0) ld = -1;
  int last_qp = ld >= 0 ? nb[ld].qp : a.slot_qp[slot];
  for (int i = i0; i < i1; ++i) {
    if (has(i)) {
      int d = nb[i].qp - last_qp;
      if (d < -26) d += 52;
      if (d > 25) d -= 52;
      nb[i].dqp = static_cast<int8_t>(d);
      last_qp = nb[i].qp;
    } else {
      nb[i].dqp = 0;
    }
  }
  __builtin_amdgcn_fence(__ATOMIC_RELEASE, "workgroup");
  __builtin_amdgcn_wave_barrier();
  __builtin_amdgcn_fence(__ATOMIC_ACQUIRE, "workgroup");
  for (int i = lane; i < n; i += 64)
    nb[i].prev_dqp_nz = static_cast<uint8_t>(i > 0 && has(i - 1) && nb[i - 1].dqp != 0);
}

__global__ __launch_bounds__(64) void cabac_count(CabacBinArgs a) {
  const int mb = blockIdx.x * 64 + threadIdx.x, slot = blockIdx.y, n = a.g.nmb();
  if (mb >= n) return;
  const CabacSliceInfo si = slice_info(a, slot, mb);
  const size_t base = static_cast<size_t>(slot) * n;
  h264::CabacSymbolPacker<h264::CabacCountEmit> s;
  h264::CabacMbCoder<h264::CabacSymbolPacker<h264::CabacCountEmit>> coder(s, si, a.nb + base);
  coder.code_mb(mb, a.hdr[base + mb], a.coef + (base + mb) * h264::kCoefPerMb, mb == slice_end(a, mb) - 1);
  s.flush_bypass();
  a.cnt[base + mb] = s.out.n;
}

__global__ __launch_bounds__(64) void cabac_offsets(CabacBinArgs a) {
// ... 231 lines not shown
    uint4 t[8];
#pragma unroll
    for (int k = 0; k < 8; ++k) t[k] = q[k];
#pragma unroll
    for (int k = 0; k < 8; ++k) my[k] = t[k];
  }
  const int hbytes = a.hdr_nbits[l] >> 3;
  for (int i = 0; i < hbytes; ++i) c.out.put(static_cast<uint8_t>(a.hdr_bits[l * 16 + (i >> 2)] >> (24 - 8 * (i & 3))));
  c.out.start(hbytes);
  c.init();
  const int n = total - 1;
  for (int b0 = 0; b0 < n; b0 += kArithBlock) {
    const uint4* nq = q + (b0 >> 3) + 8;
    const uint4 n0 = nq[0], n1 = nq[1], n2 = nq[2], n3 = nq[3], n4 = nq[4], n5 = nq[5], n6 = nq[6], n7 = nq[7];
    const int m = min(kArithBlock, n - b0);
    for (int ch = 0; ch * 8 < m; ++ch) {
      const uint4 cw = my[ch];
      const int mm = min(8, m - ch * 8);
      auto sym = [&](uint32_t w, int k) { return k < mm ? w : 0x8000u; };
      fast_step(c, sym(cw.x & 0xFFFFu, 0), st + lane, tab);
      fast_step(c, sym(cw.x >> 16, 1), st + lane, tab);
      fast_step(c, sym(cw.y & 0xFFFFu, 2), st + lane, tab);
      fast_step(c, sym(cw.y >> 16, 3), st + lane, tab);
      c.drain();
      fast_step(c, sym(cw.z & 0xFFFFu, 4), st + lane, tab);
      fast_step(c, sym(cw.z >> 16, 5), st + lane, tab);
      fast_step(c, sym(cw.w & 0xFFFFu, 6), st + lane, tab);
      fast_step(c, sym(cw.w >> 16, 7), st + lane, tab);
      c.drain();
    }
    my[0] = n0;
    my[1] = n1;
    my[2] = n2;
    my[3] = n3;
    my[4] = n4;
    my[5] = n5;
    my[6] = n6;
    my[7] = n7;
    c.out.flush_words();
  }
  c.finish();
  const bool bad = c.bad || c.out.n > c.out.cap;
  a.bytes[l] = bad ? -1 : static_cast<int>(c.out.n);
  if (bad) atomicOr(a.err, 8);
}

__global__ __launch_bounds__(256) void cabac_compact(CabacCodeArgs a) {
  const int l = blockIdx.x;
  __shared__ unsigned long long s_off, s_tot;
  if (threadIdx.x == 0) s_off = s_tot = 0;
  __syncthreads();
  unsigned long long part = 0, tot = 0;
  for (int s = threadIdx.x; s < a.L; s += blockDim.x) {
    const unsigned long long r16 = a.bytes[s] > 0 ? ((static_cast<unsigned long long>(a.bytes[s]) + 15ull) & ~15ull) : 0ull;
    tot += r16;
    if (s < l) part += r16;
  }
  atomicAdd(&s_off, part);
  atomicAdd(&s_tot, tot);
  __syncthreads();
  const long long off = static_cast<long long>(s_off);
  const bool host = a.host_out && static_cast<long long>(s_tot) <= a.host_cap;
  if (threadIdx.x == 0) a.out_off[l] = off;
  const int nbytes = a.bytes[l];
  if (nbytes <= 0) return;
  const uint4* src = reinterpret_cast<const uint4*>(a.pool + a.base[l]);
  uint4* dst = reinterpret_cast<uint4*>((host ? a.host_out : a.out) + off);
  for (int i = threadIdx.x; i < (nbytes + 15) / 16; i += blockDim.x) dst[i] = src[i];
}

}
}

using namespace mivc::gpu;

extern "C" size_t mivc_cabac_nb_bytes() { return sizeof(CabacNb); }
extern "C" int mivc_cabac_gap() { return kCabacGap; }
extern "C" int mivc_cabac_read_ahead() { return kArithReadAhead; }

extern "C" void mivc_launch_cabac_bin(int B, int wmb, int hmb, const void* hdr, const int16_t* coef, uint32_t* mask,
                                      void* nb, int* cnt, long long* off, int* tot, uint16_t* pool,
                                      long long pool_cap, long long* pool_used, long long* base, int* total,
                                      const int* slot_qp, int slice_type, int num_ref_l0, int num_ref_l1,
                                      int t8x8_mode, int* err, void* stream, const void* route, int slice_rows) {
  CabacBinArgs a;
  const int rows = (slice_rows > 0 && slice_rows < hmb) ? slice_rows : hmb;
  a.slice_mbs = rows * wmb;
  a.per_slot = (hmb + rows - 1) / rows;
  a.rt = static_cast<const SlotRoute*>(route);
  a.g = Geom{B, wmb, hmb, wmb * 16, hmb * 16};
  a.hdr = static_cast<const MbHeader*>(hdr);
  a.coef = coef;
  a.mask = mask;
  a.nb = static_cast<CabacNb*>(nb);
  a.cnt = cnt;
  a.off = off;
  a.tot = tot;
  a.pool = pool;
  a.pool_cap = pool_cap;
  a.pool_used = pool_used;
  a.base = base;
  a.total = total;
  a.slot_qp = slot_qp;
  a.slice_type = slice_type;
  a.num_ref_l0 = num_ref_l0;
  a.num_ref_l1 = num_ref_l1;
  a.t8x8_mode = t8x8_mode;
  a.err = err;
  hipStream_t s = static_cast<hipStream_t>(stream);
  const int nmb = wmb * hmb;
  const dim3 mbgrid((nmb + 63) / 64, B);
  hipLaunchKernelGGL(cabac_mask, dim3((nmb + 2 * kMaskSpan - 1) / (2 * kMaskSpan), B), dim3(64), 0, s, a);
  hipLaunchKernelGGL(cabac_prep, mbgrid, dim3(64), 0, s, a);
  hipLaunchKernelGGL(cabac_chain, dim3(B * a.per_slot), dim3(64), 0, s, a);
  hipLaunchKernelGGL(cabac_count, mbgrid, dim3(64), 0, s, a);
  hipLaunchKernelGGL(cabac_offsets, dim3(B * a.per_slot), dim3(64), 0, s, a);
  hipLaunchKernelGGL(cabac_alloc, dim3(1), dim3(64), 0, s, a);
  hipLaunchKernelGGL(cabac_bins, mbgrid, dim3(64), 0, s, a);
}

extern "C" void mivc_launch_cabac_code(int L, int B, uint16_t* pool, const long long* base, const int* total,
                                       const uint32_t* hdr_bits, const int* hdr_nbits, const int* slot_qp,
                                       unsigned long long itypes, int* bytes, uint8_t* out, long long* out_off,
                                       int* err, uint8_t* host_out, long long host_cap, void* stream) {
  CabacCodeArgs a;
  a.L = L;
  a.B = B;
  a.pool = pool;
  a.base = base;
  a.total = total;
  a.hdr_bits = hdr_bits;
  a.hdr_nbits = hdr_nbits;
  a.slot_qp = slot_qp;
  a.itypes = itypes;
  a.bytes = bytes;
  a.out = out;
  a.out_off = out_off;
  a.err = err;
  a.host_out = nullptr;
  a.host_cap = 0;
  if (host_out) {
    void* dp = nullptr;
    if (hipHostGetDevicePointer(&dp, host_out, 0) == hipSuccess && dp) {
      a.host_out = static_cast<uint8_t*>(dp);
      a.host_cap = host_cap;
    }
  }
  hipStream_t s = static_cast<hipStream_t>(stream);
  a.lpw = 64;
  hipLaunchKernelGGL(cabac_arith, dim3((L + 63) / 64), dim3(64), 0, s, a);
  hipLaunchKernelGGL(cabac_compact, dim3(L), dim3(256), 0, s, a);
}
```

csrc/kernels/encode_inter.hip:

```cpp
#include "h264_trellis.h"
#include "mb_row.h"

namespace mivc {
namespace gpu {

using h264::MbHeader;

struct InterArgs {
  Geom g;
  const uint8_t *src_y, *src_u, *src_v;
  const uint8_t *ref_y, *ref_u, *ref_v;
  uint8_t *rec_y, *rec_u, *rec_v;
  const uint8_t* pred_y;
  const int16_t* mv;
  const int16_t* mv8;
  const int* me_cost;
  const int* intra_cost;
  const int* qp;
  const int8_t* aq;
  int chroma_qp_offset;
  MbHeader* hdr;
  int16_t* coef;
  uint8_t* nz;
  uint8_t* intra_flag;
  int* intra_count;
  const uint8_t *ref1_u, *ref1_v;
  int bmode;
  int w1[4];
  int t8;
  const uint8_t* refs_u[4];
  const uint8_t* refs_v[4];
  const int8_t* mref;
  const int* wp;
  int trellis;
  float trellis_lambda;
  const SlotRoute* rt;
  int nbuf;
  uint8_t* qp_flags;
};


__device__ __forceinline__ int wp_sample(int p, int w, int o, int d) {
  return h264::clip1((d >= 1 ? ((p * w + (1 << (d - 1))) >> d) : p * w) + o);
}


typedef unsigned short v2u16 __attribute__((ext_vector_type(2)));
__device__ __forceinline__ v2u16 as_v2u16(uint32_t x) { return __builtin_bit_cast(v2u16, x); }
__device__ __forceinline__ uint32_t as_u32(v2u16 x) { return __builtin_bit_cast(uint32_t, x); }
__device__ __forceinline__ v2u16 splat_u16(int v) {
  return v2u16{static_cast<unsigned short>(v), static_cast<unsigned short>(v)};
}
__device__ __forceinline__ int pair_lo(uint32_t p) { return static_cast<int>(p & 0xFFFFu); }
__device__ __forceinline__ int pair_hi(uint32_t p) { return static_cast<int>(p >> 16); }
__device__ __forceinline__ uint32_t make_pair(int lo, int hi) {
  return static_cast<uint32_t>(lo) | (static_cast<uint32_t>(hi) << 16);
}
__device__ __forceinline__ uint32_t pairs_to_u8x4(const uint32_t (&p)[2]) {
  return __builtin_amdgcn_perm(p[1], p[0], 0x06040200u);
}

__device__ __forceinline__ void chroma_mc4x4(const uint8_t* refc, int cw, int CH, int px0, int py0, int mvx, int mvy,
                                             uint32_t (&pp)[4][2]) {
  const int xf = mvx & 7, yf = mvy & 7;
  const int xi = px0 + (mvx >> 3), yi = py0 + (mvy >> 3);
  uint32_t ra[5][2], rb[5][2];
  if (xi >= 0 && xi + 8 <= cw && yi >= 0 && yi + 5 <= CH) {
    const uint32_t s = static_cast<uint32_t>(xi & 3) * 0x00010001u;
    const uint32_t sa0 = 0x0c010c00u + s, sa1 = 0x0c030c02u + s, sb0 = 0x0c020c01u + s, sb1 = 0x0c040c03u + s;
#pragma unroll
    for (int r = 0; r < 5; ++r) {
      const uint8_t* row = refc + static_cast<size_t>(yi + r) * cw;
      const int a = xi & ~3;
      const uint32_t w0 = *reinterpret_cast<const uint32_t*>(row + a), w1 = *reinterpret_cast<const uint32_t*>(row + a + 4);
      ra[r][0] = __builtin_amdgcn_perm(w1, w0, sa0);
      ra[r][1] = __builtin_amdgcn_perm(w1, w0, sa1);
      rb[r][0] = __builtin_amdgcn_perm(w1, w0, sb0);
      rb[r][1] = __builtin_amdgcn_perm(w1, w0, sb1);
    }
  } else {
#pragma unroll
    for (int r = 0; r < 5; ++r) {
      const uint8_t* row = refc + static_cast<size_t>(clampi(yi + r, 0, CH - 1)) * cw;
      int c[5];
#pragma unroll
      for (int i = 0; i < 5; ++i) c[i] = row[clampi(xi + i, 0, cw - 1)];
      ra[r][0] = make_pair(c[0], c[1]);
      ra[r][1] = make_pair(c[2], c[3]);
      rb[r][0] = make_pair(c[1], c[2]);
      rb[r][1] = make_pair(c[3], c[4]);
    }
  }
  const v2u16 wA = splat_u16((8 - xf) * (8 - yf)), wB = splat_u16(xf * (8 - yf)), wC = splat_u16((8 - xf) * yf),
              wD = splat_u16(xf * yf), half = splat_u16(32);
#pragma unroll
  for (int y = 0; y < 4; ++y)
#pragma unroll
    for (int h = 0; h < 2; ++h)
      pp[y][h] = as_u32((half + wA * as_v2u16(ra[y][h]) + wB * as_v2u16(rb[y][h]) + wC * as_v2u16(ra[y + 1][h]) +
                         wD * as_v2u16(rb[y + 1][h])) >> 6);
}

__device__ __forceinline__ void store_levels(int16_t* dst, const int* v) {
  uint32_t w[8];
#pragma unroll
  for (int i = 0; i < 8; ++i) w[i] = (static_cast<uint32_t>(v[2 * i]) & 0xFFFFu) | (static_cast<uint32_t>(v[2 * i + 1]) << 16);
  reinterpret_cast<uint4*>(dst)[0] = make_uint4(w[0], w[1], w[2], w[3]);
  reinterpret_cast<uint4*>(dst)[1] = make_uint4(w[4], w[5], w[6], w[7]);
}

__device__ __forceinline__ int decimate_score(const int* scan, int start) {
  int score = 0, last = start - 1;
  bool big = false;
#pragma unroll
  for (int i = 0; i < 16; ++i) {
    if (i < start) continue;
    const int v = scan[i];
    const bool nzv = v != 0;
    big |= v > 1 || v < -1;
    const int run = i - last - 1;
    const int t = run == 0 ? 3 : (run <= 2 ? 2 : (run <= 5 ? 1 : 0));
// ... 148 lines not shown
          uint32_t w = 0;
#pragma unroll
          for (int b = 0; b < 4; ++b) w |= ((__builtin_popcount(col & (4 * j + b)) & 1) ? 0xFFu : 0x01u) << (8 * b);
          hp[j] = static_cast<int>(w);
          hn[j] = static_cast<int>(w ^ 0xFEFEFEFEu);
        }
        int sa = 0;
#pragma unroll
        for (int t = 0; t < 4; ++t) {
          const bool neg = __builtin_popcount(t & grp) & 1;
          mfma_i32x4 d = __builtin_amdgcn_mfma_i32_16x16x64_i8(neg ? hn : hp, sop, mfma_i32x4{0, 0, 0, 0}, 0, 0, 0);
          d = __builtin_amdgcn_mfma_i32_16x16x64_i8(neg ? hp : hn, pop, d, 0, 0, 0);
          sa += abs(d[0]) + abs(d[1]) + abs(d[2]) + abs(d[3]);
        }
        sa = sum_row_groups(sa);
        const int sa8d = __shfl(sum4((sa + 2) >> 2), 4 * q, 64);
        const int satd16 = sum16(satd);
        use8 = mine && sa8d < satd16;
        use8_wave = __ballot(use8);
        wave_sync();
        if (use8_wave) {
          if (use8) {
            dct8_pass(dd + (2 * k) * 8, 1);
            dct8_pass(dd + (2 * k + 1) * 8, 1);
          }
          wave_sync();
          if (use8) {
            dct8_pass(dd + 2 * k, 8);
            dct8_pass(dd + 2 * k + 1, 8);
          }
          wave_sync();
          const int qbits8 = 16 + qp / 6;
          const int m = qp % 6;
          if (a.trellis >= 2) {
            float z[16];
            int nzc = 0;
            if (use8) {
              const float inv = exp2f(-static_cast<float>(qbits8));
#pragma unroll
              for (int i = 0; i < 16; ++i) {
                const int pos = kZz8[k * 16 + i];
                const int mf8 = kQuant8MF[m][pos8(pos & 7, pos >> 3)];
                z[i] = static_cast<float>(dd[pos]) * static_cast<float>(mf8) * inv;
                nzc |= h264::quant_coef(dd[pos], mf8, qbits8, 11) != 0;
              }
            }
            const int nz1 = quad_bcast<1>(nzc), nz2 = quad_bcast<2>(nzc), nz3 = quad_bcast<3>(nzc);
            const bool later = (k < 1 && nz1) || (k < 2 && nz2) || (k < 3 && nz3);
            if (use8) trellis_lite8_chunk(z, lv, a.trellis_lambda * 0.136f, later);
          } else if (use8) {
#pragma unroll
            for (int i = 0; i < 16; ++i) {
              const int pos = kZz8[k * 16 + i];
              lv[i] = h264::quant_coef(dd[pos], kQuant8MF[m][pos8(pos & 7, pos >> 3)], qbits8, 11);
            }
          }
          int lastnz = -1, firstnz = -1, inner = 0, big = 0;
          if (use8) {
#pragma unroll
            for (int i = 0; i < 16; ++i) {
              const int idx = k * 16 + i;
              const int v = lv[i];
              const bool nzv = v != 0;
              big |= v > 1 || v < -1;
              const int run = idx - lastnz - 1;
              inner += (nzv && firstnz >= 0) ? (run <= 3 ? 3 : (run <= 11 ? 2 : (run <= 23 ? 1 : 0))) : 0;
              firstnz = (nzv && firstnz < 0) ? idx : firstnz;
              lastnz = nzv ? idx : lastnz;
            }
          }
          const int l0 = quad_bcast<0>(lastnz), l1 = quad_bcast<1>(lastnz), l2 = quad_bcast<2>(lastnz);
          const int prev = max(k > 0 ? l0 : -1, max(k > 1 ? l1 : -1, k > 2 ? l2 : -1));
          const int run0 = firstnz - prev - 1;
          const int sc = inner + (firstnz >= 0 ? (run0 <= 3 ? 3 : (run0 <= 11 ? 2 : (run0 <= 23 ? 1 : 0))) : 0);
          const int big8 = sum4(big), sc8 = sum4(sc);
          const int scb = big8 ? 9 : sc8;
          const int total8 = sum16(k == 0 ? scb : 0);
          keep8 = use8 && scb >= 4 && total8 >= 6;
        }
      }
    }

    bool any = false;
    if (use8_wave) {
      if (use8) {
#pragma unroll
        for (int i = 0; i < 16; ++i) lv[i] = keep8 ? lv[i] : 0;
        store_levels(coef + h264::COEF_LUMA + l * 16, lv);
        const int m = qp % 6, q6 = qp / 6;
#pragma unroll
        for (int i = 0; i < 16; ++i) {
          const int pos = kZz8[k * 16 + i];
          const int ls = 16 * kNorm8[m][pos8(pos & 7, pos >> 3)];
          const int c = lv[i];
          dd[pos] = q6 >= 6 ? (c * ls) << (q6 - 6) : (c * ls + (1 << (5 - q6))) >> (6 - q6);
        }
      }
      wave_sync();
      if (use8) {
        idct8_pass(dd + (2 * k) * 8, 1);
        idct8_pass(dd + (2 * k + 1) * 8, 1);
      }
      wave_sync();
      if (use8) {
        idct8_pass(dd + 2 * k, 8);
        idct8_pass(dd + 2 * k + 1, 8);
      }
      wave_sync();
      if (use8) {
        any = keep8;
#pragma unroll
        for (int y = 0; y < 4; ++y)
#pragma unroll
          for (int x = 0; x < 4; ++x) res[y * 4 + x] = (dd[(oy + y) * 8 + ox + x] + 32) >> 6;
      }
    }
    if (work && !use8) {
      int sv[16];
#pragma unroll
      for (int i = 0; i < 16; ++i) {
        sv[i] = keep4 ? lv[h264::kZigzag4x4[i]] : 0;
        any |= sv[i] != 0;
      }
      store_levels(coef + h264::COEF_LUMA + l * 16, sv);
      int dv[3];
#pragma unroll
      for (int c = 0; c < 3; ++c) dv[c] = h264::kDequantV[qp % 6][c];
#pragma unroll
      for (int r = 0; r < 16; ++r) res[r] = keep4 ? (lv[r] * dv[h264::kPosClass[r]]) << (qp / 6) : 0;
      if (any) h264::inverse_core4x4(res);
    }
    const bool t8_coded = ((__ballot(keep8) >> (16 * q)) & 0xFFFFu) != 0;
    if (a.qp_flags) {
      const uint64_t luma_any = __ballot(any);
      if (live && l == 0) a.qp_flags[o] = !work ? 2 : (((luma_any >> (16 * q)) & 0xFFFFu) != 0 ? 1 : 0);
    }
    if (work) {
      uint8_t* recy = a.rec_y + rcur * g.ysize() + static_cast<size_t>(Y0 + lby) * W + X0 + lbx;
#pragma unroll
      for (int y = 0; y < 4; ++y) {
        int v4[4];
#pragma unroll
        for (int x = 0; x < 4; ++x)
          v4[x] = h264::clip1(static_cast<int>(__builtin_amdgcn_ubfe(prw[y], 8 * x, 8)) + (any ? res[y * 4 + x] : 0));
        *reinterpret_cast<uint32_t*>(recy + static_cast<size_t>(y) * W) = pack4_u8(v4);
      }
      a.nz[o * 16 + (lbx >> 2) + lby] = any;
      if (l < 2) reinterpret_cast<uint4*>(coef + h264::COEF_LUMA_DC)[l] = make_uint4(0, 0, 0, 0);
      if (l == 0) {
        h->qp = static_cast<int8_t>(qp);
        h->i16_mode = 0;
        h->chroma_mode = 0;
        h->flags = t8_coded ? h264::MBF_T8x8 : 0;
        a.intra_flag[o] = 0;
        if (!a.bmode) {
          const int mvx = a.mv[o * 2], mvy = a.mv[o * 2 + 1];
          const uint32_t mvw = (static_cast<uint32_t>(mvx) & 0xFFFFu) | (static_cast<uint32_t>(mvy) << 16);
          uint4 q4 = make_uint4(mvw, mvw, mvw, mvw);
          if (a.mv8) q4 = *reinterpret_cast<const uint4*>(a.mv8 + o * 8);
          h->kind = (q4.x == q4.y && q4.z == q4.w) ? (q4.x == q4.z ? h264::MBK_P16x16 : h264::MBK_P16x8)
                                                   : ((q4.x == q4.z && q4.y == q4.w) ? h264::MBK_P8x16 : h264::MBK_P8x8);
          uint4* mvp = reinterpret_cast<uint4*>(&h->mv[0][0][0]);
          mvp[0] = q4;
          const uint32_t r = a.mref ? static_cast<uint32_t>(a.mref[o]) * 0x01010101u : 0u;
          *reinterpret_cast<uint2*>(&h->ref[0][0]) = make_uint2(r, 0xFFFFFFFFu);
        }
      }
    }
  }

}

__global__ __launch_bounds__(64) void encode_inter_chroma(InterArgs a) {
  const Geom& g = a.g;
  const int lane = threadIdx.x, m = lane >> 3, comp = (lane >> 2) & 1, cb = lane & 3;
  const int nmb = g.nmb();
  int ux, slot;
  xcd_unit_slot(ux, slot);
  if (!route_active(a.rt, slot, a.bmode ? SK_B : SK_P)) return;
  const size_t rcur = route_index(a.rt, a.nbuf, slot, RO_CUR);
  const int cw = g.cw(), CH = g.ch();
  const int mb0 = ux * kMbsPerChromaWave;
  const bool live = mb0 + m < nmb;
  const int dm = live ? m : nmb - 1 - mb0;
  int mx = mb0 % g.wmb + dm, my = mb0 / g.wmb;
  while (__ballot(mx >= g.wmb)) {
    const bool wrap = mx >= g.wmb;
    mx -= wrap ? g.wmb : 0;
    my += wrap ? 1 : 0;
  }
  const size_t o = static_cast<size_t>(slot) * nmb + mb0 + dm;
  const bool work = live && !(a.intra_cost[o] < a.me_cost[o]);
  const int qpc = h264::chroma_qp(clampi(a.qp[slot] + (a.aq ? a.aq[o] : 0), 0, 51), a.chroma_qp_offset);
  const MbHeader* h = a.hdr + o;
  int16_t* coef = a.coef + o * h264::kCoefPerMb;
  const int cbx = (cb & 1) * 4, cby = (cb >> 1) * 4;

  int lv[16];
  int res[16];
  uint32_t prw[4];
  int mfc[3], dvc[3];
  int dc = 0, score = 0;
  if (work) {
#pragma unroll
    for (int c = 0; c < 3; ++c) {
      mfc[c] = h264::kQuantMF[qpc % 6][c];
      dvc[c] = h264::kDequantV[qpc % 6][c];
    }
    const uint8_t* srcc = (comp == 0 ? a.src_u : a.src_v) + slot * g.csize();
    const int px0 = mx * 8 + cbx, py0 = my * 8 + cby;
    uint32_t pp[4][2];
    if (!a.bmode) {
      const int cmx = a.mv8 ? a.mv8[o * 8 + cb * 2] : a.mv[o * 2], cmy = a.mv8 ? a.mv8[o * 8 + cb * 2 + 1] : a.mv[o * 2 + 1];
      const int r = a.mref ? a.mref[o] : 0;
      chroma_mc4x4((comp == 0 ? a.refs_u[r] : a.refs_v[r]) + route_index(a.rt, a.nbuf, slot, RO_L0 + r) * g.csize(), cw,
                   CH, px0, py0, cmx, cmy, pp);
      if (a.wp && r == 0) {
        const int* wt = a.wp + slot * 8;
        const int w = wt[3 + 2 * comp], wo = wt[4 + 2 * comp], d = wt[7];
        if (w != (1 << d) || wo != 0) {
#pragma unroll
          for (int y = 0; y < 4; ++y)
#pragma unroll
            for (int hh = 0; hh < 2; ++hh)
              pp[y][hh] = make_pair(wp_sample(pair_lo(pp[y][hh]), w, wo, d), wp_sample(pair_hi(pp[y][hh]), w, wo, d));
        }
      }
    } else {
      const int r0 = h->ref[0][cb];
      const bool u0 = r0 >= 0, u1 = h->ref[1][cb] >= 0;
      const int w1 = a.rt ? a.rt[slot].w1[r0 & 3] : a.w1[r0 & 3];
      uint32_t p1[4][2];
      if (u0) chroma_mc4x4((comp == 0 ? a.refs_u[r0 & 3] : a.refs_v[r0 & 3]) +
                               route_index(a.rt, a.nbuf, slot, RO_L0 + (r0 & 3)) * g.csize(), cw, CH, px0, py0,
                           h->mv[0][cb][0], h->mv[0][cb][1], pp);
      if (u1) chroma_mc4x4((comp == 0 ? a.ref1_u : a.ref1_v) + route_index(a.rt, a.nbuf, slot, RO_L1) * g.csize(), cw,
                           CH, px0, py0,
                           h->mv[1][cb][0], h->mv[1][cb][1], p1);
      const bool bi = u0 && u1;
      if (__ballot(bi && (w1 < 0 || w1 > 64)) == 0) {
        const v2u16 k0 = splat_u16(64 - w1), k1 = splat_u16(w1), half = splat_u16(32);
#pragma unroll
        for (int y = 0; y < 4; ++y)
#pragma unroll
          for (int hh = 0; hh < 2; ++hh) {
            const uint32_t b2 = as_u32((half + as_v2u16(pp[y][hh]) * k0 + as_v2u16(p1[y][hh]) * k1) >> 6);
            pp[y][hh] = u0 ? (u1 ? b2 : pp[y][hh]) : p1[y][hh];
          }
      } else {
#pragma unroll
        for (int y = 0; y < 4; ++y)
#pragma unroll
          for (int hh = 0; hh < 2; ++hh) {
            const int lo = h264::clip1((pair_lo(pp[y][hh]) * (64 - w1) + pair_lo(p1[y][hh]) * w1 + 32) >> 6);
            const int hi = h264::clip1((pair_hi(pp[y][hh]) * (64 - w1) + pair_hi(p1[y][hh]) * w1 + 32) >> 6);
            pp[y][hh] = u0 ? (u1 ? make_pair(lo, hi) : pp[y][hh]) : p1[y][hh];
          }
      }
    }
    uint32_t sw[4];
#pragma unroll
    for (int y = 0; y < 4; ++y) sw[y] = *reinterpret_cast<const uint32_t*>(srcc + static_cast<size_t>(py0 + y) * cw + px0);
#pragma unroll
    for (int y = 0; y < 4; ++y) {
#pragma unroll
      for (int x = 0; x < 4; ++x)
        res[y * 4 + x] = static_cast<int>(__builtin_amdgcn_ubfe(sw[y], 8 * x, 8)) -
                         ((x & 1) ? pair_hi(pp[y][x >> 1]) : pair_lo(pp[y][x >> 1]));
      prw[y] = pairs_to_u8x4(pp[y]);
    }
    h264::forward_core4x4(res);
    dc = res[0];
    const int qbits = 15 + qpc / 6;
    if (a.trellis >= 2) {
      trellis_lite4x4(res, lv, mfc, qbits, trellis_lambda4(a.trellis_lambda, qpc), 1);
    } else {
#pragma unroll
      for (int r = 0; r < 16; ++r)
        lv[r] = r == 0 ? 0 : h264::quant_coef(res[r], mfc[h264::kPosClass[r]], qbits, 11);
    }
    int scan[16];
#pragma unroll
    for (int i = 0; i < 16; ++i) scan[i] = lv[h264::kZigzag4x4[i]];
    score = decimate_score(scan, 1);
  }
  const int d0 = quad_bcast<0>(dc), d1 = quad_bcast<1>(dc), d2 = quad_bcast<2>(dc), d3 = quad_bcast<3>(dc);
  const int score_c = sum4(score);
  const bool keep_ac = score_c >= 7;
  bool any_c = false;
  if (work) {
    const int f[4] = {d0 + d1 + d2 + d3, d0 - d1 + d2 - d3, d0 + d1 - d2 - d3, d0 - d1 - d2 + d3};
    int cl[4];
#pragma unroll
    for (int i = 0; i < 4; ++i) cl[i] = h264::quant_coef(f[i], mfc[0], 15 + qpc / 6 + 1, 11);
    int sv[16];
    bool any_ac = false;
#pragma unroll
    for (int i = 0; i < 16; ++i) {
      sv[i] = (keep_ac && i > 0) ? lv[h264::kZigzag4x4[i]] : 0;
      any_ac |= sv[i] != 0;
    }
    store_levels(coef + h264::COEF_CHROMA_AC + (comp * 4 + cb) * 16, sv);
    if (cb == 0) {
      auto p2 = [](int lo, int hi) { return (static_cast<uint32_t>(lo) & 0xFFFFu) | (static_cast<uint32_t>(hi) << 16); };
      *reinterpret_cast<uint2*>(coef + h264::COEF_CHROMA_DC + comp * 4) = make_uint2(p2(cl[0], cl[1]), p2(cl[2], cl[3]));
    }
    const int c0 = cl[0], c1 = cl[1], c2 = cl[2], c3 = cl[3];
    const int fcb = cb == 0 ? c0 + c1 + c2 + c3 : (cb == 1 ? c0 - c1 + c2 - c3 : (cb == 2 ? c0 + c1 - c2 - c3 : c0 - c1 - c2 + c3));
    const int ls = 16 * dvc[0];
#pragma unroll
    for (int r = 0; r < 16; ++r) res[r] = (keep_ac && r > 0) ? (lv[r] * dvc[h264::kPosClass[r]]) << (qpc / 6) : 0;
    res[0] = ((fcb * ls) << (qpc / 6)) >> 5;
    const bool any = any_ac || c0 || c1 || c2 || c3;
    any_c = any;
    if (any) h264::inverse_core4x4(res);
    uint8_t* recc = (comp == 0 ? a.rec_u : a.rec_v) + rcur * g.csize() + static_cast<size_t>(my * 8 + cby) * cw + mx * 8 + cbx;
#pragma unroll
    for (int y = 0; y < 4; ++y) {
      int v4[4];
#pragma unroll
      for (int x = 0; x < 4; ++x)
        v4[x] = h264::clip1(static_cast<int>(__builtin_amdgcn_ubfe(prw[y], 8 * x, 8)) + (any ? res[y * 4 + x] : 0));
      *reinterpret_cast<uint32_t*>(recc + static_cast<size_t>(y) * cw) = pack4_u8(v4);
    }
  }
  if (a.qp_flags) {
    const uint64_t chroma_any = __ballot(any_c);
    if (work && (lane & 7) == 0 && ((chroma_any >> (8 * m)) & 0xFFu) != 0) a.qp_flags[o] = 1;
  }
}

}
}

using namespace mivc::gpu;

extern "C" void mivc_launch_encode_inter(int B, int wmb, int hmb, const uint8_t* src_y, const uint8_t* src_u,
                                         const uint8_t* src_v, const uint8_t* ref_y, const uint8_t* ref_u,
                                         const uint8_t* ref_v, uint8_t* rec_y, uint8_t* rec_u, uint8_t* rec_v,
                                         const uint8_t* pred_y, const int16_t* mv, const int* me_cost,
                                         const int* intra_cost, const int* qp, int chroma_qp_offset, void* hdr,
                                         int16_t* coef, uint8_t* nz, uint8_t* intra_flag, int* intra_count,
                                         const int8_t* aq, const uint8_t* ref1_u, const uint8_t* ref1_v, int bmode,
                                         int t8, const int16_t* mv8, void* stream, const int* w1, int nref,
                                         const uint8_t* const* xref_u, const uint8_t* const* xref_v,
                                         const int8_t* mref, const int* wp, int trellis, float trellis_lambda,
                                         const void* route, int nbuf, uint8_t* qp_flags) {
  InterArgs a;
  a.qp_flags = qp_flags;
  a.rt = static_cast<const SlotRoute*>(route);
  a.nbuf = nbuf;
  a.trellis = trellis;
  a.trellis_lambda = trellis_lambda;
  a.wp = bmode ? nullptr : wp;
  for (int r = 0; r < 4; ++r) {
    const int rr = r < nref ? r : 0;
    a.refs_u[r] = rr == 0 ? ref_u : xref_u[rr];
    a.refs_v[r] = rr == 0 ? ref_v : xref_v[rr];
  }
  a.mref = mref;
  for (int r = 0; r < 4; ++r) a.w1[r] = w1[r < nref ? r : 0];
  a.g = Geom{B, wmb, hmb, wmb * 16, hmb * 16};
  a.src_y = src_y;
  a.src_u = src_u;
  a.src_v = src_v;
  a.ref_y = ref_y;
  a.ref_u = ref_u;
  a.ref_v = ref_v;
  a.rec_y = rec_y;
  a.rec_u = rec_u;
  a.rec_v = rec_v;
  a.pred_y = pred_y;
  a.mv = mv;
  a.mv8 = bmode ? nullptr : mv8;
  a.me_cost = me_cost;
  a.intra_cost = intra_cost;
  a.qp = qp;
  a.chroma_qp_offset = chroma_qp_offset;
  a.hdr = static_cast<MbHeader*>(hdr);
  a.coef = coef;
  a.nz = nz;
  a.intra_flag = intra_flag;
  a.intra_count = intra_count;
  a.aq = aq;
  a.ref1_u = ref1_u;
  a.ref1_v = ref1_v;
  a.bmode = bmode;
  a.t8 = t8;
  hipLaunchKernelGGL(encode_inter_mb, dim3(mb_row_grid(wmb * hmb), B), dim3(64), 0, static_cast<hipStream_t>(stream), a);
  hipLaunchKernelGGL(encode_inter_chroma, dim3(chroma_wave_grid(wmb * hmb), B), dim3(64), 0, static_cast<hipStream_t>(stream), a);
}
```

govideocompressor_amd/models/h264_gpu.py:

```python
from __future__ import annotations

import concurrent.futures as cf
import math
import os
import time
from dataclasses import dataclass

import numpy as np
import torch

from ..ops import native
from .gop import PicPlan, col_to_list0, dpb_frames, fixed_types, gop_plan, h264_plan

MB_HDR_BYTES = 64
NO_COST = 0x3FFFFFFF
ROUTE_DTYPE = np.dtype([("kind", "i1"), ("cur", "i1"), ("n0", "i1"), ("l1", "i1"), ("l0", "i1", (4,)),
                        ("w1", "<i2", (4,)), ("dsf", "<i2", (4,)), ("dcopy", "i1", (4,)), ("flags", "u1"),
                        ("col_l1", "i1"), ("disp", "<i2")])
assert ROUTE_DTYPE.itemsize == 32
COL_NONE = -128


def col_map_row(cur: PicPlan, col: PicPlan) -> np.ndarray:
    return np.array([[COL_NONE if m is None else m - r for r, m in enumerate(row)] for row in col_to_list0(cur, col)],
# ... 229 lines not shown
            raise ValueError("entropy must be 'gpu' or 'cpu'")
        if isinstance(params.aq_mode, bool) or params.aq_mode not in (0, 1, 2, 3):
            raise ValueError("aq_mode must be 0 (off), 1 (variance), 2 (auto-variance) or 3 (auto-variance, biased)")
        if params.eff_slices() > 1 and params.direct == "spatial" and params.eff_bframes() and params.spatial_wavefront:
            raise ValueError("slices > 1: spatial direct needs the fast path (spatial_wavefront=False)")
        self.entropy = entropy
        self.p = params
        self.slice_rows = params.slice_rows()
        self.S = params.eff_slices()
        self.B = int(slots)
        self.dev = _resolve(device)
        self.hip = native.hip()
        self.host = native.host()
        self.aq_strength = float(params.aq_strength) if params.aq_mode else 0.0
        self.aq_auto = int(params.aq_mode) if (params.aq_mode in (2, 3) and self.aq_strength > 0) else 0
        if self.aq_auto and not hasattr(self.hip, "aq_auto_finish"):
            raise RuntimeError("aq_mode 2 / 3 need a kernel library with the auto-variance AQ kernels (rebuild)")
        self.wmb = (params.width + 15) // 16
        self.hmb = (params.height + 15) // 16
        self.W, self.H = self.wmb * 16, self.hmb * 16
        self.nmb = self.wmb * self.hmb
        self._mbtree = None
        self._wp = self._wp_steps = None
        B, H, W, nmb, dev = self.B, self.H, self.W, self.nmb, self.dev
        u8, i16, i32 = torch.uint8, torch.int16, torch.int32

        def planes():
            return (torch.zeros((B, H, W), dtype=u8, device=dev),
                    torch.zeros((B, H // 2, W // 2), dtype=u8, device=dev),
                    torch.zeros((B, H // 2, W // 2), dtype=u8, device=dev))

        self.src = planes()
        self.nb = params.eff_bframes()
        self.nref = params.eff_refs()
        self.nref_frames = dpb_frames(self.nref, params.eff_pyramid(), self.nb)
        self.nbuf = self.nref_frames + 2
        NB = self.nbuf
        self.rec_pool = (torch.zeros((B, NB, H, W), dtype=u8, device=dev),
                         torch.zeros((B, NB, H // 2, W // 2), dtype=u8, device=dev),
                         torch.zeros((B, NB, H // 2, W // 2), dtype=u8, device=dev))
        self.rec = [tuple(p[:, i] for p in self.rec_pool) for i in range(NB)]
        self.hp_bytes = 3 * (H + 8) * (W + 8)
        self.hp_pool = torch.empty(B * NB * self.hp_bytes + 64, dtype=u8, device=dev)
        self.hdr = [torch.zeros((B, nmb, MB_HDR_BYTES), dtype=u8, device=dev) for _ in range(2)]
        self.coef = [torch.zeros((B, nmb, COEF_PER_MB), dtype=i16, device=dev) for _ in range(2)]
        self.nz = torch.zeros((B, nmb, 16), dtype=u8, device=dev)
        self.mv = torch.zeros((B, nmb, 2), dtype=i16, device=dev)
        self.mv_tmp = torch.zeros((B, nmb, 2), dtype=i16, device=dev)
        self.mv8 = torch.zeros((B, nmb, 4, 2), dtype=i16, device=dev)
        self.prev_mv = torch.zeros((B, nmb, 2), dtype=i16, device=dev)
        self.me_cost = torch.zeros((B, nmb), dtype=i32, device=dev)
        self.intra_cost = torch.zeros((B, nmb), dtype=i32, device=dev)
        self.pred = torch.zeros((B, nmb, 256), dtype=u8, device=dev)
        self.mref = torch.zeros((B, nmb), dtype=torch.int8, device=dev)
        self.dref = torch.zeros((B, nmb, 4), dtype=torch.int8, device=dev)
        self.seed = [torch.zeros((B, nmb, 2), dtype=i16, device=dev) for _ in range(2)]
        self._slot_ar = torch.arange(B, device=dev)
        if self.nref > 1:
            K = self.nref - 1
            self.xmv = torch.zeros((K, B, nmb, 2), dtype=i16, device=dev)
            self.xcost = torch.zeros((K, B, nmb), dtype=i32, device=dev)
            self.xpred = torch.zeros((K, B, nmb, 256), dtype=u8, device=dev)
            self.xpm = torch.zeros((B, nmb, 2), dtype=i16, device=dev)
        if self.nb:
            self.mv1 = torch.zeros((B, nmb, 2), dtype=i16, device=dev)
            self.me_cost1 = torch.zeros((B, nmb), dtype=i32, device=dev)
            self.pred1 = torch.zeros((B, nmb, 256), dtype=u8, device=dev)
            self.pred_b = torch.zeros((B, nmb, 256), dtype=u8, device=dev)
            self.cost_b = torch.zeros((B, nmb), dtype=i32, device=dev)
            self.pm0 = torch.zeros((B, nmb, 2), dtype=i16, device=dev)
            self.pm1 = torch.zeros((B, nmb, 2), dtype=i16, device=dev)
            self.dmv = torch.zeros((B, nmb, 16), dtype=i16, device=dev)
            self.czero = torch.zeros((B, nmb), dtype=u8, device=dev)
            self.sfix = torch.zeros((B, nmb), dtype=u8, device=dev)
            self.col_pool = torch.zeros((B, NB, nmb, MB_HDR_BYTES), dtype=u8, device=dev)
        if params.eff_weightp():
            self.src_me = torch.zeros((B, H, W), dtype=u8, device=dev)
        self.intra_flag = torch.zeros((B, nmb), dtype=u8, device=dev)
        self.aq = torch.zeros((B, nmb), dtype=torch.int8, device=dev)
        if self.aq_auto:
            self.aq_terms = torch.zeros((B, nmb), dtype=torch.float32, device=dev)
        self.qp_flags = torch.zeros((B, nmb), dtype=u8, device=dev)
        self.qp_pre = torch.zeros((B, nmb), dtype=u8, device=dev)
        self.intra_count = torch.zeros((B,), dtype=i32, device=dev)
        self.qp = torch.zeros((B,), dtype=i32, device=dev)
        self.err_bufs = [torch.zeros((1,), dtype=i32, device=dev) for _ in range(2)]
        self.err = self.err_bufs[0]
        self.h_err = [torch.zeros((1,), dtype=i32).pin_memory() for _ in range(2)]
        self._batch_no = 0
        self._ring_last: list = [None, None]
        self._inflight: list = []
        self.p_intra_mbs = torch.zeros((), dtype=torch.int64, device=dev)
        self.far_ref_mbs = torch.zeros((), dtype=torch.int64, device=dev)
        self.sfix_mbs = torch.zeros((), dtype=torch.int64, device=dev)
        self.sconv_mbs = torch.zeros((), dtype=torch.int64, device=dev)
        self.una_mbs = torch.zeros((), dtype=torch.int64, device=dev)
        self._una_count = bool(params.eff_pyramid() and params.direct == "temporal")
        self.keep_records = False
        self.last_records = None
        if entropy == "cpu":
            self.h_hdr = [torch.empty((B, nmb, MB_HDR_BYTES), dtype=u8).pin_memory() for _ in range(2)]
            self.h_coef = [torch.empty((B, nmb, COEF_PER_MB), dtype=i16).pin_memory() for _ in range(2)]
        elif params.cabac:
            self._alloc_cabac(cabac_group)
        else:
            i64 = torch.int64
            mbb = int(self.hip.cavlc_mb_bytes())
            self.cap_words = nmb * 128 + 64
            self.cav_mbs = torch.zeros((B, nmb, mbb), dtype=u8, device=dev)
            self.cav_len = torch.zeros((B, nmb), dtype=i32, device=dev)
            self.cav_off = torch.zeros((B, nmb), dtype=i64, device=dev)
            self.cav_trail = torch.zeros((B,), dtype=i32, device=dev)
            self.cav_total = torch.zeros((B,), dtype=i64, device=dev)
            self.cav_words = torch.zeros((B, self.cap_words), dtype=torch.int32, device=dev)
            self.cav_out_off = torch.zeros((B,), dtype=i64, device=dev)
            self.cav_hdr_bits = [torch.zeros((B, 16), dtype=i32, device=dev) for _ in range(2)]
            self.cav_hdr_nbits = [torch.zeros((B,), dtype=i32, device=dev) for _ in range(2)]
            self.h_hdr_bits = [torch.zeros((B, 16), dtype=i32).pin_memory() for _ in range(2)]
            self.h_hdr_nbits = [torch.zeros((B,), dtype=i32).pin_memory() for _ in range(2)]
            self.cav_sizes = [torch.zeros((B,), dtype=i32, device=dev) for _ in range(2)]
            self.h_sizes = [torch.zeros((B,), dtype=i32).pin_memory() for _ in range(2)]
            self.cav_out = [torch.zeros((B * self.cap_words * 4,), dtype=u8, device=dev) for _ in range(2)]
            self.h_out: list = [None, None, None]
            self.out_done = [torch.cuda.Event() for _ in range(2)]
            self.copy_pool = cf.ThreadPoolExecutor(max_workers=1)
        self.copy_stream = torch.cuda.Stream(device=dev)
        self.copy_done = [torch.cuda.Event() for _ in range(2)]
        self.compute_done = [torch.cuda.Event() for _ in range(2)]
        nthreads = entropy_threads or min(16, max(2, (os.cpu_count() or 4)))
        self.entropy_threads = nthreads
        self.pool = cf.ThreadPoolExecutor(max_workers=nthreads)
        self.cfg = params.host_cfg()
        self.timings: dict[str, float] = {}
        self.stats: dict[str, float] = {}
        from ..obs.timers import EventTimer
        self.stage_timer = EventTimer(enabled=os.environ.get("MIVC_STAGE_TIMING", "0") == "1")

    def _alloc_cabac(self, group: int | None, grow: int = 1):
        B, nmb, dev = self.B, self.nmb, self.dev
        u8, i32, i64 = torch.uint8, torch.int32, torch.int64
        G = int(group or os.environ.get("MIVC_CABAC_GROUP", 20))
        if not 1 <= G <= 64:
            raise ValueError("cabac_group must be in 1..64")
        self.cab_G = G
        per_mb = int(os.environ.get("MIVC_CABAC_SYMS_PER_MB", 96)) * grow
        peak_mb = int(os.environ.get("MIVC_CABAC_PEAK_SYMS_PER_MB", 768)) * grow
        self.cab_grow = grow
        gap = int(self.hip.cabac_gap())
        L = G * B * self.S
        self.cab_pool_cap = B * nmb * (G * per_mb + peak_mb) + L * (gap + 8) + 64
        self.cab_pool = [torch.empty((self.cab_pool_cap + 64,), dtype=torch.int16, device=dev) for _ in range(2)]
        self.cab_pool_used = torch.zeros((2,), dtype=i64, device=dev)
        comp_cap = (self.cab_pool_cap * 5) // 4 + 80 * L
        self.cab_comp = [torch.empty((comp_cap,), dtype=u8, device=dev) for _ in range(2)]
        self.cab_comp_off = [torch.zeros((L,), dtype=i64, device=dev) for _ in range(2)]
        self.cab_base = [torch.zeros((L,), dtype=i64, device=dev) for _ in range(2)]
        self.cab_total = [torch.zeros((L,), dtype=i32, device=dev) for _ in range(2)]
        self.cab_bytes = [torch.zeros((L,), dtype=i32, device=dev) for _ in range(2)]
        self.h_cab_bytes = [torch.zeros((L,), dtype=i32).pin_memory() for _ in range(2)]
        self.h_pool_used = [torch.zeros((1,), dtype=i64).pin_memory() for _ in range(2)]
        self.cab_hdr_bits = [torch.zeros((L, 16), dtype=i32, device=dev) for _ in range(2)]
        self.cab_hdr_nbits = [torch.zeros((L,), dtype=i32, device=dev) for _ in range(2)]
        self.h_cab_hdr_bits = [torch.zeros((L, 16), dtype=i32).pin_memory() for _ in range(2)]
        self.h_cab_hdr_nbits = [torch.zeros((L,), dtype=i32).pin_memory() for _ in range(2)]
        self.cab_mask = torch.zeros((B, nmb), dtype=i32, device=dev)
        self.cab_nb = torch.zeros((B, nmb, int(self.hip.cabac_nb_bytes())), dtype=u8, device=dev)
        self.cab_cnt = torch.zeros((B, nmb), dtype=i32, device=dev)
        self.cab_off = torch.zeros((B, nmb), dtype=i64, device=dev)
        self.cab_tot = torch.zeros((B * self.S,), dtype=i32, device=dev)
        self.entropy_stream = torch.cuda.Stream(device=dev)
        self.cab_bin_done = [torch.cuda.Event() for _ in range(2)]
        self.cab_done = [torch.cuda.Event() for _ in range(2)]
        from ..runtime.device import pinned_budget
        self.cab_host_cap = min(comp_cap, int(os.environ.get("MIVC_CABAC_HOST_MB", 1024)) << 20, pinned_budget() // 4)
        self.h_cab_out = [torch.empty((self.cab_host_cap,), dtype=u8).pin_memory() for _ in range(2)]
        self.copy_pool = cf.ThreadPoolExecutor(max_workers=1)

    @staticmethod
    def _ptr(t: torch.Tensor) -> int:
        return t.data_ptr()

    def _stream(self) -> int:
        return torch.cuda.current_stream(self.dev).cuda_stream

    def parameter_sets(self) -> bytes:
        return self.host.parameter_sets(self.cfg)

    def _prep(self, y, u, v, t: int):
        B, F, h, w = y.shape
        cs = u.shape[2] * u.shape[3]
        self.hip.prep(y[:, t].data_ptr(), u[:, t].data_ptr(), v[:, t].data_ptr(), w, h, F * h * w, F * cs, B,
                      self._ptr(self.src[0]), self._ptr(self.src[1]), self._ptr(self.src[2]),
                      self.p.width, self.p.height, self.W, self.H, self._stream())

    def _mbtree_rows(self) -> tuple[int, int]:
        mbt = self._mbtree
        if mbt is not None and mbt.shape[2] == self.nmb:
            return mbt.data_ptr(), mbt.shape[1] * self.nmb
        return 0, 0

    def _prep_step(self, y, u, v, disp: np.ndarray, disp_d: torch.Tensor, st: dict | None = None):
        B, F, h, w = y.shape
        cs = u.shape[2] * u.shape[3]
        same = bool((disp == disp[0]).all())
        with self.stage_timer("prep"):
            if st is not None:
                st["aq_done"] = st["aq_terms_done"] = False
                if self.aq_auto:
                    t = int(disp[0]) if same else 0
                    st["aq_terms_done"] = self.hip.prep_aq_terms(
                        y[:, t].data_ptr(), u[:, t].data_ptr(), v[:, t].data_ptr(), w, h, F * h * w, F * cs, B,
                        self._ptr(self.src[0]), self._ptr(self.src[1]), self._ptr(self.src[2]), self.W, self.H,
                        self._ptr(self.aq_terms), self._stream(), 0 if same else disp_d.data_ptr())
                    if st["aq_terms_done"]:
                        return
                elif self.aq_strength > 0 and hasattr(self.hip, "prep_aq"):
                    t = int(disp[0]) if same else 0
                    extra, stride = self._mbtree_rows()
                    st["aq_done"] = self.hip.prep_aq(
                        y[:, t].data_ptr(), u[:, t].data_ptr(), v[:, t].data_ptr(), w, h, F * h * w, F * cs, B,
                        self._ptr(self.src[0]), self._ptr(self.src[1]), self._ptr(self.src[2]), self.W, self.H,
                        self.aq_strength, self._ptr(self.aq), self._stream(),
                        0 if same else disp_d.data_ptr(), extra, stride, st["route"])
                    if st["aq_done"]:
                        return
            if same:
                return self._prep(y, u, v, int(disp[0]))
            self.hip.prep(y.data_ptr(), u.data_ptr(), v.data_ptr(), w, h, F * h * w, F * cs, B,
                          self._ptr(self.src[0]), self._ptr(self.src[1]), self._ptr(self.src[2]),
                          self.p.width, self.p.height, self.W, self.H, self._stream(), disp_d.data_ptr())

    @staticmethod
    def _dist_scale(poc: int, poc0: int, poc1: int) -> tuple[int, int]:
        def tdiv(x: int, y: int) -> int:
            q = abs(x) // abs(y)
            return q if (x >= 0) == (y >= 0) else -q
        tb = max(-128, min(127, poc - poc0))
        td = max(-128, min(127, poc1 - poc0))
        if td == 0:
            return 0, 1
        tx = tdiv(16384 + abs(tdiv(td, 2)), td)
        return max(-1024, min(1023, (tb * tx + 32) >> 6)), 0

    def _encode_step(self, st: dict, hdr, coef, cut=None):
        s = self._stream()
        B, wmb, hmb = self.B, self.wmb, self.hmb
        P = self._ptr
        sy, su, sv = (P(x) for x in self.src)
        py, pu, pv = (P(x) for x in self.rec_pool)
        hpp = P(self.hp_pool)
        rt, NB = st["route"], self.nbuf
        aq = 0
        mbt = self._mbtree
        stt = self.stage_timer
        if self.aq_strength > 0 or mbt is not None:
            aq = P(self.aq)
            if self.aq_auto:
                extra, stride = self._mbtree_rows()
                with stt("aq"):
                    if not st.get("aq_terms_done"):
                        self.hip.aq_terms(B, wmb, hmb, sy, su, sv, P(self.aq_terms), s)
                    self.hip.aq_auto_finish(B, self.nmb, P(self.aq_terms), self.aq_auto, self.aq_strength, aq, s,
                                            extra, stride, rt)
            elif not st.get("aq_done"):
                extra, stride = self._mbtree_rows()
                with stt("aq"):
                    self.hip.aq_offsets(B, wmb, hmb, sy, su, sv, self.aq_strength, aq, s, extra, stride, rt)
        cqo = self.p.chroma_qp_offset
        inter = st["P"] or st["B"]
        pre = {"qp_flags": P(self.qp_pre)} if (aq and inter and hasattr(self.hip, "prep_aq")) else {}
        if inter:
            self.intra_count.zero_()
        seed0 = seed1 = 0
        if inter and self._la_mv is not None:
            v = self._la_mv[self._slot_ar, st["disp_d"].long()].reshape(B, self.nmb)
            dxy = torch.stack((((v << 16) >> 16), v >> 16), -1).float()
            self.seed[0].copy_((dxy * st["sscale"][0][:, None, None]).round_().clamp_(-2048, 2047))
            seed0 = P(self.seed[0])
            if st["B"]:
                self.seed[1].copy_((dxy * st["sscale"][1][:, None, None]).round_().clamp_(-2048, 2047))
                seed1 = P(self.seed[1])
        if st["P"]:
            sy_me, wp = sy, 0
            if st["wp"] is not None:
                wp = st["wp"].data_ptr()
                with stt("weightp"):
                    self.hip.wp_src(sy, P(self.src_me), st["wp_src"].data_ptr(), B, self.H * self.W, s)
                sy_me = P(self.src_me)
            with stt("me_p"):
                self.hip.me(B, wmb, hmb, sy_me, py, P(self.prev_mv), P(self.mv), P(self.me_cost), P(self.pred),
                            P(self.intra_cost), P(self.qp), self.p.me_range, self.p.subpel, s, hpp, aq, 1,
                            self.p.p_early_sad, 0, 0, 0, rt, NB, 0, SK["P"], seed0)
                if getattr(self, "_chg", None) is None:
                    self._chg = [torch.zeros((B, self.nmb), dtype=torch.uint8, device=self.dev) for _ in range(2)]
                for it in range(int(self.p.skip_refine)):
                    a_, b_ = (self.mv, self.mv_tmp) if it % 2 == 0 else (self.mv_tmp, self.mv)
                    self.hip.p_refine(B, wmb, hmb, sy_me, py, hpp, P(a_), P(b_), P(self.me_cost), P(self.prev_mv),
                                      P(self.pred), P(self.qp), aq, s, rt, NB,
                                      0 if (it == 0 or not self.p.refine_skip) else P(self._chg[(it - 1) % 2]),
                                      P(self._chg[it % 2]) if self.p.refine_skip else 0)
                if int(self.p.skip_refine) % 2:
                    self.mv.copy_(torch.where(st["pmask"][:, None, None], self.mv_tmp, self.mv))
            mv8 = 0
            if self.p.eff_partitions():
                with stt("part"):
                    self.hip.p_part8(B, wmb, hmb, sy_me, py, hpp, P(self.mv), P(self.prev_mv), P(self.me_cost),
                                     P(self.pred), P(self.mv8), P(self.qp), aq, int(self.p.part_overhead),
                                     int(self.p.part_min_satd), s, rt, NB)
                mv8 = P(self.mv8)
            self.prev_mv.copy_(torch.where(st["pmask"][:, None, None], self.mv, self.prev_mv))
            nr = st["maxn0"]
            if nr > 1:
                with stt("me_ref"):
                    for k in range(1, nr):
                        self.xpm.copy_((self.mv.float() * st["xscale"][k - 1][:, None, None]).round_().clamp_(-2048, 2047))
                        self.hip.me(B, wmb, hmb, sy, py, P(self.xpm), P(self.xmv[k - 1]), P(self.xcost[k - 1]),
                                    P(self.xpred[k - 1]), 0, P(self.qp), int(self.p.ref_range), self.p.subpel, s,
                                    hpp, aq, 1, self.p.p_early_sad, P(self.me_cost), self._ref_gate(),
                                    P(self.prev_mv), rt, NB, k, SK["P"])
                    self.hip.me_ref_select(B, wmb, hmb, nr, P(self.mv), mv8, P(self.me_cost), P(self.pred),
                                           P(self.xmv), P(self.xcost), P(self.xpred), P(self.mref), P(self.qp), aq,
                                           s, rt)
                    self.far_ref_mbs += ((self.mref > 0) & st["pmask"][:, None]).sum()
            else:
                self.mref.zero_()
            if cut is not None:
                self.intra_cost.masked_fill_(cut[:, None], -1)
            with stt("inter"):
                self.hip.encode_inter(B, wmb, hmb, sy, su, sv, py, pu, pv, py, pu, pv, P(self.pred), P(self.mv),
                                      P(self.me_cost), P(self.intra_cost), P(self.qp), cqo, P(hdr), P(coef),
                                      P(self.nz), P(self.intra_flag), P(self.intra_count), s, aq,
                                      t8=int(self.p.eff_t8x8()), mv8=mv8, mref=P(self.mref), wp=wp,
                                      trellis=int(self.p.trellis), trellis_lambda=float(self.p.trellis_lambda),
                                      route=rt, nbuf=NB, **pre)
        if st["B"]:
            br = self.p.b_me_range
            spatial = self.p.direct == "spatial"
            sfast = spatial and not self.p.spatial_wavefront
            mode = 2 if sfast else int(spatial)
            bg = int(self.p.b_gate) if (not spatial or sfast or self.p.spatial_gate) else 0
            dbias = int(self.p.tdirect_bias) if not spatial else (int(self.p.direct_bias) if sfast else 0)
            with stt("me_b"):
                self.hip.b_direct(B, wmb, hmb, P(self.col_pool), [0], [1], P(self.dmv), P(self.pm0), P(self.pm1), s,
                                  P(self.dref), rt, NB, P(self.czero), st["cmap"])
                if self._una_count:
                    self.una_mbs += ((self.dref < 0).any(dim=2) & st["bmask"][:, None]).sum()
                if bg != 0 or sfast:
                    self.hip.b_decide(B, wmb, hmb, sy, py, py, hpp, hpp, P(self.mv), P(self.mv1), P(self.me_cost),
                                      P(self.me_cost1), P(self.pred), P(self.pred1), P(self.pm0), P(self.pm1),
                                      P(self.dmv), P(self.qp), aq, P(hdr), P(self.pred_b), P(self.cost_b), s, [32],
                                      P(self.dref), [], [], 1, spatial=mode, route=rt, nbuf=NB, czero=P(self.czero))
                gate = P(self.cost_b) if bg != 0 else 0
                self.hip.me(B, wmb, hmb, sy, py, P(self.pm0), P(self.mv), P(self.me_cost), P(self.pred),
                            P(self.intra_cost), P(self.qp), br, self.p.subpel, s, hpp, aq, 1, self.p.b_early_sad,
                            gate, bg, 0, rt, NB, 0, SK["B"], seed0)
                self.hip.me(B, wmb, hmb, sy, py, P(self.pm1), P(self.mv1), P(self.me_cost1), P(self.pred1), 0,
                            P(self.qp), br, self.p.subpel, s, hpp, aq, 1, self.p.b_early_sad, gate, bg, 0, rt, NB,
                            4, SK["B"], seed1)
            with stt("b_decide"):
                self.hip.b_decide(B, wmb, hmb, sy, py, py, hpp, hpp, P(self.mv), P(self.mv1), P(self.me_cost),
                                  P(self.me_cost1), P(self.pred), P(self.pred1), P(self.pm0), P(self.pm1),
                                  P(self.dmv), P(self.qp), aq, P(hdr), P(self.pred_b), P(self.cost_b), s, [32],
                                  P(self.dref), [], [], 0, int(self.p.eff_partitions() and self.p.bpartitions),
                                  int(bg != 0 or sfast), mode, dbias, route=rt, nbuf=NB, czero=P(self.czero))
            if sfast:
                with stt("b_spatial"):
                    self.hip.b_spatial_exact(B, wmb, hmb, P(hdr), P(self.intra_cost), P(self.cost_b), P(self.czero),
                                             P(self.sfix), s, rt, self.slice_rows, int(self.p.spatial_fix_tol))
                    self.sfix_mbs += (self.sfix == 1).sum()
                    self.sconv_mbs += (self.sfix == 2).sum()
                    self.hip.b_spatial_fixup(B, wmb, hmb, P(hdr), P(self.sfix), py, hpp, py, hpp, P(self.pred_b), s,
                                             rt, NB)
            elif spatial:
                with stt("b_spatial"):
                    self.hip.b_spatial(B, wmb, hmb, P(hdr), P(self.col_pool), sy, py, hpp, [py], [hpp], [32],
                                       P(self.pred_b), P(self.err), s, P(self.intra_cost), P(self.cost_b), P(self.qp),
                                       aq, int(self.p.direct_bias), rt, NB)
            with stt("inter"):
                self.hip.encode_inter(B, wmb, hmb, sy, su, sv, py, pu, pv, py, pu, pv, P(self.pred_b), P(self.mv),
                                      P(self.cost_b), P(self.intra_cost), P(self.qp), cqo, P(hdr), P(coef),
                                      P(self.nz), P(self.intra_flag), P(self.intra_count), s, aq, pu, pv, 1,
                                      int(self.p.eff_t8x8()), 0, [32], [], [], 0, 0, int(self.p.trellis),
                                      float(self.p.trellis_lambda), rt, NB, **pre)
        if inter:
            self.p_intra_mbs += self.intra_count.sum()
            flag_ptr, count_ptr = P(self.intra_flag), P(self.intra_count)
        else:
            self.prev_mv.zero_()
            flag_ptr, count_ptr = 0, 0
        trial = not inter or self.p.i4x4_in_p or cut is not None
        if getattr(self, "_intra_prog", None) is None:
            per = -(-hmb // self.slice_rows) if self.slice_rows > 0 else 1
            self._intra_prog = torch.zeros(B * per * 272, dtype=torch.int32, device=self.dev)
        with stt("intra"):
            self.hip.encode_intra(B, wmb, hmb, sy, su, sv, py, pu, pv, P(self.qp), cqo, P(hdr), P(coef), P(self.nz),
                                  flag_ptr, count_ptr, P(self.err), int(self.p.i4x4 and trial), s, aq,
                                  int(self.p.i8x8 and self.p.eff_t8x8() and trial), rt, NB, self.slice_rows,
                                  trellis=self.p.eff_intra_trellis(), trellis_lambda=float(self.p.trellis_lambda),
                                  gprog=P(self._intra_prog), gprog_ints=self._intra_prog.numel())
        if aq:
            with stt("qp_fixup"):
                if pre:
                    self.hip.qp_fixup(B, wmb, hmb, P(hdr), P(coef), P(self.nz), P(self.qp_flags), P(self.qp), s,
                                      self.slice_rows, pre=pre["qp_flags"], route=rt)
                else:
                    self.hip.qp_fixup(B, wmb, hmb, P(hdr), P(coef), P(self.nz), P(self.qp_flags), P(self.qp), s,
                                      self.slice_rows)
        if self.p.deblock and st["deblock"]:
            with stt("deblock"):
                self.hip.deblock(B, wmb, hmb, py, pu, pv, P(hdr), P(self.nz), cqo, 0, 0, P(self.err), s, rt, NB)
        if st["ref"]:
            with stt("halfpel"):
                self.hip.me_halfpel(B, self.W, self.H, py, hpp, s, rt, NB)
            if self.nb and st["col_dst"] is not None:
                self.col_pool.view(B * NB, self.nmb, MB_HDR_BYTES).index_copy_(
                    0, st["col_dst"], hdr.index_select(0, st["col_src"]))

    def _plans(self, F: int, cuts_h: np.ndarray, anchors_at) -> list[list[PicPlan]]:
        per_slot = (isinstance(anchors_at, (list, tuple)) and len(anchors_at) == self.B and len(anchors_at) > 0
                    and all(isinstance(a, (list, tuple, set, frozenset)) for a in anchors_at))
        common = set() if per_slot else {int(d) for d in anchors_at}
        cache: dict[str, list[PicPlan]] = {}
        plans = []
        multi = getattr(self, "_la_multi", None)
        multi_intra = getattr(self, "_la_multi_intra", None) if self.p.badapt_guard else None
        adaptive = multi is not None and multi.shape[:2] == (self.B, F)
        shared = None
        if adaptive:
            from ..rc.badapt import b_adapt_types, with_anchors
            if self.p.badapt_shared:
                mi = None if multi_intra is None else multi_intra.sum(axis=0)
                shared = b_adapt_types(self._la_costs[:, :, 1].sum(axis=0), multi.sum(axis=0), multi[:, :, 0].sum(axis=0),
                                       self.nb, self._la_blocks * self.B, common, int(self.p.b_bias), mi)
        for b in range(self.B):
            forced = {int(d) for d in anchors_at[b]} if per_slot else common
            forced = forced | {d for d in range(1, F) if cuts_h[b, d]}
            if shared is not None:
                ty = with_anchors(shared, forced)
            elif adaptive:
                ty = b_adapt_types(self._la_costs[b, :, 1], multi[b], multi[b, :, 0], self.nb, self._la_blocks, forced,
                                   int(self.p.b_bias), None if multi_intra is None else multi_intra[b])
            else:
                ty = fixed_types(F, self.nb, forced)
            if ty not in cache:
                cache[ty] = h264_plan(ty, self.nref, self.p.eff_pyramid(), self.nref_frames)
            plans.append(cache[ty])
        return plans

    def _step_tables(self, plans: list[list[PicPlan]], F: int) -> list[dict]:
        B, NB, dev = self.B, self.nbuf, self.dev
        rt = np.zeros((F, B), dtype=ROUTE_DTYPE)
        rt["l1"] = -1
        rt["l0"] = -1
        rt["disp"] = -1
        rt["w1"] = 32
        rt["dcopy"] = 1
        K = max(1, self.nref - 1)
        xscale = np.zeros((F, K, B), dtype=np.float32)
        sscale = np.zeros((F, 2, B), dtype=np.float32)
        deblock_nonref = bool(self._full_recon)
        col = {}
        use_cmap = self.p.direct == "temporal"
        cmap = np.zeros((F, B, 2, 4), dtype=np.int8)
        colcache: dict[int, tuple] = {}
        for b in range(B):
            key = id(plans[b])
# ... 76 lines not shown
                st["col_dst"] = flat_d[1, a0:a1]
            steps.append(st)
        return steps

    def _ref_gate(self) -> int:
        return int(self.p.ref_gate)

    def _frame_params(self, b: int, pic: PicPlan, t: int, qp_frame: int, idr_ids: list[int]) -> dict:
        fp = dict(idr=int(pic.kind == "I"), frame_num=pic.frame_num, idr_pic_id=idr_ids[b] & 0xFFFF, qp=qp_frame,
                  slice_type=pic.slice_type, nal_ref_idc=pic.nal_ref_idc, poc=pic.poc,
                  direct_spatial=int(pic.kind == "B" and self.p.direct == "spatial"))
        if pic.kind != "I":
            fp["num_ref_l0"] = max(1, len(pic.refs0))
            fp["num_ref_l1"] = 1
            if pic.mod_l0:
                fp["mod_l0"] = [tuple(m) for m in pic.mod_l0]
        if pic.kind == "P" and self._wp is not None and any(
                int(x) != (1 << WP_LOG2 if i % 2 == 0 else 0) for i, x in enumerate(self._wp[t, b])):
            fp["wp"] = [WP_LOG2, WP_LOG2] + [int(x) for x in self._wp[t, b]]
        return fp

    def _weights(self, y, u, v, plans: list[list[PicPlan]]) -> None:
        self._wp = None
        self._wp_steps = None
        if not self.p.eff_weightp() or not any(pic.kind == "P" for plan in plans for pic in plan):
            return
        B, F, h, w = y.shape
        st = torch.empty((B, F, 6), dtype=torch.int64, device=self.dev)
        self.hip.wp_stats(y.data_ptr(), u.data_ptr(), v.data_ptr(), w, h, B * F, st.data_ptr(), self._stream())
        sh = st.cpu().numpy().astype(np.float64)
        n = np.array([w * h, w * h / 4, w * h / 4])
        mean = sh[..., 0::2] / n
        var = np.maximum(sh[..., 1::2] / n - mean ** 2, 0.0)
        one = 1 << WP_LOG2
        bs, ts, ds, rs = [], [], [], []
        for b, plan in enumerate(plans):
            for t, pic in enumerate(plan):
                if pic.kind == "P":
                    bs.append(b)
                    ts.append(t)
                    ds.append(pic.d)
                    rs.append(pic.l0)
        bs, ts, ds, rs = (np.array(a, dtype=np.int64) for a in (bs, ts, ds, rs))
        m1, m0 = mean[bs, ds], mean[bs, rs]
        v1, v0 = var[bs, ds], var[bs, rs]
        scale = np.where(v0 > 1e-3, np.sqrt(v1 / np.maximum(v0, 1e-3)), 1.0)
        use = (np.abs(m1[:, 0] - m0[:, 0]) >= self.p.wp_min_mean) | (np.abs(scale[:, 0] - 1) >= self.p.wp_min_scale)
        if not use.any():
            return
        wq = np.clip(np.round(scale * one), 0, 127)
        oq = np.clip(np.round(m1 - wq / one * m0), -128, 127)
        wp = np.zeros((F, B, 6), dtype=np.int32)
        wp[:, :, 0::2] = one
        for c in range(3):
            wp[ts[use], bs[use], 2 * c] = wq[use, c]
            wp[ts[use], bs[use], 2 * c + 1] = oq[use, c]
        on = np.zeros(F, dtype=bool)
        on[ts[use]] = True
        self._wp = wp
        dev8 = np.zeros((F, B, 8), dtype=np.int32)
        dev8[..., 0], dev8[..., 1], dev8[..., 2] = wp[..., 0], wp[..., 1], WP_LOG2
        dev8[..., 3:7], dev8[..., 7] = wp[..., 2:6], WP_LOG2
        wp_dev = torch.from_numpy(dev8).to(self.dev)
        wp_src = torch.from_numpy(np.ascontiguousarray(dev8[..., :3])).to(self.dev)
        self._wp_steps = [(wp_dev[t], wp_src[t]) if on[t] else None for t in range(F)]
        self.stats["weightp_pictures"] = int(use.sum())

    @staticmethod
    def _cabac_groups(F: int, G: int) -> list[tuple[int, int]]:
        head = [1] if (F > 2 and G > 1) else []
        R = F - len(head)
        sizes = [G] * (R // G) + ([R % G] if R % G else [])
        if sizes and sizes[-1] > max(1, G // 2):
            last = sizes.pop()
            sizes += [(last + 1) // 2, last // 2]
        sizes = head + sizes
        out, t0 = [], 0
        for n in sizes:
            out.append((t0, n))
            t0 += n
        return out

    def _gpu_cabac_bin(self, k: int, g: int, j: int, t: int, pics: list[PicPlan], qps_t, idr_ids: list[int],
                       qp_dev: torch.Tensor, route: int):
        B, BS = self.B, self.B * self.S
        r = g & 1
        if j == 0:
            self.cab_pool_used[r].zero_()
        self._header_bits_into(self.h_cab_hdr_bits[r][j * BS:(j + 1) * BS], self.h_cab_hdr_nbits[r][j * BS:(j + 1) * BS],
                               self.cab_hdr_bits[r][j * BS:(j + 1) * BS], self.cab_hdr_nbits[r][j * BS:(j + 1) * BS],
                               pics, t, qps_t, idr_ids)
        P = self._ptr
        self.hip.cabac_bin(B, self.wmb, self.hmb, P(self.hdr[k]), P(self.coef[k]), P(self.cab_mask), P(self.cab_nb),
                           P(self.cab_cnt), P(self.cab_off), P(self.cab_tot), P(self.cab_pool[r]), self.cab_pool_cap,
                           self.cab_pool_used[r].data_ptr(), self.cab_base[r][j * BS:].data_ptr(),
                           self.cab_total[r][j * BS:].data_ptr(), P(qp_dev), pics[0].slice_type, 1, 1,
                           int(self.p.eff_t8x8()), P(self.err), self.copy_stream.cuda_stream, route, self.slice_rows)

    def _gpu_cabac_code(self, g: int, t0: int, n: int, qps_d: torch.Tensor, err_to: torch.Tensor | None = None):
        BS = self.B * self.S
        r = g & 1
        self.cab_bin_done[r].record(self.copy_stream)
        itypes = 1 if t0 == 0 else 0
        P = self._ptr
        es = self.entropy_stream
        with torch.cuda.stream(es):
            es.wait_event(self.cab_bin_done[r])
            self.hip.cabac_code(n * BS, BS, P(self.cab_pool[r]), P(self.cab_base[r]), P(self.cab_total[r]),
                                P(self.cab_hdr_bits[r]), P(self.cab_hdr_nbits[r]), qps_d[t0].data_ptr(), itypes,
                                P(self.cab_bytes[r]), P(self.cab_comp[r]), P(self.cab_comp_off[r]), P(self.err),
                                es.cuda_stream, P(self.h_cab_out[r]), self.cab_host_cap)
            self.h_cab_bytes[r][: n * BS].copy_(self.cab_bytes[r][: n * BS], non_blocking=True)
            self.h_pool_used[r].copy_(self.cab_pool_used[r:r + 1], non_blocking=True)
            if err_to is not None:
                err_to.copy_(self.err, non_blocking=True)
            self.cab_done[r].record(es)

    def _copy_out_group(self, g: int, t0: int, n: int, copied, wrap_futs, steps_pics: list[list[PicPlan]], groups):
        B = self.B * self.S
        r = g & 1
        t_0 = time.perf_counter()
        self.cab_done[r].synchronize()
        t_1 = time.perf_counter()
        sizes = self.h_cab_bytes[r][: n * B].numpy().astype(np.int64)
        used = int(self.h_pool_used[r][0])
        self.stats["cabac_pool_peak"] = max(self.stats.get("cabac_pool_peak", 0.0), used / self.cab_pool_cap)
        self.stats["cabac_syms_per_mb_peak"] = max(self.stats.get("cabac_syms_per_mb_peak", 0.0),
                                                   used / (n * B * self.nmb))
        if (sizes < 0).any():
            err = int(self.err.item())
            for f in range(t0, t0 + n):
                wrap_futs[f] = self.pool.submit(lambda: [(b"", 0)] * self.B)
            copied[g].set()
            if err & 4:
                raise CabacPoolExhausted("GPU CABAC: symbol pool exhausted (raise MIVC_CABAC_SYMS_PER_MB / "
                                         "MIVC_CABAC_PEAK_SYMS_PER_MB or lower cabac_group)")
            raise RuntimeError("GPU CABAC: arithmetic coder error")
        r16 = (sizes + 15) & ~15
        total = int(r16.sum())
        buf = self.h_cab_out[r]
        if total > self.cab_host_cap:
            buf = torch.empty((total,), dtype=torch.uint8).pin_memory()
            with torch.cuda.device(self.dev), torch.cuda.stream(self.entropy_stream):
                buf.copy_(self.cab_comp[r][:total], non_blocking=True)
                ev = torch.cuda.Event()
                ev.record(self.entropy_stream)
            ev.synchronize()
            self.stats["cabac_host_spills"] = self.stats.get("cabac_host_spills", 0) + 1
        t_2 = time.perf_counter()
        self.timings["entropy_wait_gpu_s"] = self.timings.get("entropy_wait_gpu_s", 0.0) + (t_1 - t_0)
        self.timings["d2h_s"] = self.timings.get("d2h_s", 0.0) + (t_2 - t_1)
        off = 0
        for jj in range(n):
            sz = sizes[jj * B:(jj + 1) * B]
            nb = int(r16[jj * B:(jj + 1) * B].sum())
            wrap_futs[t0 + jj] = self.pool.submit(self._wrap, buf[off:off + nb], nb, sz.tolist(), steps_pics[t0 + jj], 16)
            off += nb
        copied[g].set()

    def _header_bits(self, k: int, t: int, pics: list[PicPlan], qps_t, idr_ids: list[int]):
        self._header_bits_into(self.h_hdr_bits[k], self.h_hdr_nbits[k], self.cav_hdr_bits[k], self.cav_hdr_nbits[k],
                               pics, t, qps_t, idr_ids)

    def _header_bits_into(self, hb, hn, db, dn, pics: list[PicPlan], t: int, qps_t, idr_ids: list[int]):
        hbn, hnn = hb.numpy(), hn.numpy()
        cache = {}
        wp = self._wp
        S, first = self.S, self.slice_rows * self.wmb
        for b in range(self.B):
            pic = pics[b]
            for si in range(S):
                key = (id(pic), int(qps_t[b]), idr_ids[b] & 0xFFFF if pic.kind == "I" else -1,
                       tuple(wp[t, b]) if (wp is not None and pic.kind == "P") else None, si)
                if key not in cache:
                    fp = self._frame_params(b, pic, t, int(qps_t[b]), idr_ids)
                    if si:
                        fp["first_mb"] = si * first
                    cache[key] = self.host.slice_header_bits(self.cfg, fp)
                words, nbits = cache[key]
                ln = b * S + si
# ... 253 lines not shown
        self._weights(y, u, v, plans)
        if qps is None:
            qps_h = np.full((B, F), qp_p, dtype=np.int32)
            qps_h[:, 0] = qp_i
        else:
            qps_h = np.clip(np.asarray(qps, dtype=np.int32).reshape(B, F), 0, 51)
        if self.nb and (qps is None or self._from_la):
            from ..rc.ratecontrol import b_qps_from_refs
            qps_h = b_qps_from_refs(qps_h, plans, float(self.p.b_qp_offset))
        if qp_delta is not None:
            from ..rc.abr import apply_delta
            qps_h = apply_delta(qps_h, qp_delta)
        self.last_qps = qps_h.copy()
        qps_c = np.take_along_axis(qps_h, orders, axis=1)
        qps_d = torch.from_numpy(np.ascontiguousarray(qps_c.T)).to(self.dev)
        qps_ls_d = qps_d.repeat_interleave(self.S, dim=1).contiguous() if self.S > 1 else qps_d
        cuts_c = np.take_along_axis(cuts_h, orders, axis=1)
        cuts_d = torch.from_numpy(np.ascontiguousarray(cuts_c.T)).to(self.dev)
        if self._wp_steps is not None:
            for t, st in enumerate(steps):
                if self._wp_steps[t] is not None:
                    st["wp"], st["wp_src"] = self._wp_steps[t]
        bno = self._batch_no
        self._batch_no += 1
        self.err = self.err_bufs[bno & 1]
        self.err.zero_()
        sse = torch.zeros((F, B, 3), dtype=torch.int64, device=self.dev)
        ssim = torch.zeros((F, B), dtype=torch.float32, device=self.dev)
        pending: list[cf.Future] = [None, None]
        outs: list[list[tuple[bytes, int]]] = [None] * F
        import threading
        copied = [threading.Event() for _ in range(F)]
        copy_futs: list = [None] * F
        wrap_futs: list = [None] * F

        def wait_copied(i: int):
            while not copied[i].wait(0.5):
                if copy_futs[i].done() and copy_futs[i].exception() is not None:
                    raise copy_futs[i].exception()
        cabac_gpu = self.entropy == "gpu" and self.p.cabac
        groups = self._cabac_groups(F, self.cab_G) if cabac_gpu else [(t, 1) for t in range(F)]
        step_group = {}
        for gi, (a0, an) in enumerate(groups):
            for jj in range(an):
                step_group[a0 + jj] = (gi, jj)
        ngroups = len(groups)
        group_copied = [threading.Event() for _ in range(ngroups)]
        group_futs: list = [None] * ngroups

        def wait_group(i: int):
            while not group_copied[i].wait(0.5):
                if group_futs[i].done() and group_futs[i].exception() is not None:
                    raise group_futs[i].exception()
        recons = None
        records: list = []
        if keep_recon:
            recons = [tuple(torch.empty_like(p[:, 0]) for p in self.rec_pool) for _ in range(F)]
        main = torch.cuda.current_stream(self.dev)
        for t in range(F):
            k = t & 1
            pics = steps_pics[t]
            st = steps[t]
            qpt = qps_c[:, t]
            tw = time.perf_counter()
            if cabac_gpu:
                gi, jj = step_group[t]
                if jj == 0 and gi >= 2:
                    wait_group(gi - 2)
                elif jj == 0 and self._ring_last[gi & 1] is not None:
                    ev, fut, _ = self._ring_last[gi & 1]
                    while not ev.wait(0.5):
                        if fut.done() and fut.exception() is not None:
                            break
            elif self.entropy == "gpu" and t >= 2:
                wait_copied(t - 2)
            elif pending[k] is not None:
                outs[t - 2] = pending[k].result()
                pending[k] = None
            self.timings["host_blocked_s"] = self.timings.get("host_blocked_s", 0.0) + time.perf_counter() - tw
            main.wait_event(self.copy_done[k])
            self._prep_step(y, u, v, orders[:, t], orders_d[t], st)
            st["disp_d"] = orders_d[t]
            self.qp.copy_(qps_d[t])
            self._encode_step(st, self.hdr[k], self.coef[k], cuts_d[t] if (t > 0 and cuts_c[:, t].any()) else None)
            if metrics:
                P = self._ptr
                self.hip.sse(B, self.W, self.H, self.p.width, self.p.height, P(self.src[0]), P(self.src[1]),
                             P(self.src[2]), P(self.rec_pool[0]), P(self.rec_pool[1]), P(self.rec_pool[2]),
                             sse[t].data_ptr(), ssim[t].data_ptr(), self._stream(), st["route"], self.nbuf)
            if self.keep_records:
                records.append((self.hdr[k].clone(), self.dref.clone()))
            if keep_recon:
                bufs = torch.tensor([pic.buf for pic in pics], dtype=torch.long, device=self.dev)
                slots = torch.arange(B, device=self.dev)
                for d in sorted({pic.d for pic in pics}):
                    sel = torch.tensor([b for b in range(B) if pics[b].d == d], dtype=torch.long, device=self.dev)
                    for c in range(3):
                        recons[d][c][sel] = self.rec_pool[c][slots[sel], bufs[sel]]
            if self.entropy == "gpu" and not self.p.cabac:
                self._gpu_cavlc(k, t, pics, qpt, idr_ids)
            self.compute_done[k].record(main)
            with torch.cuda.stream(self.copy_stream):
                self.copy_stream.wait_event(self.compute_done[k])
                if cabac_gpu:
                    self._gpu_cabac_bin(k, gi, jj, t, pics, qpt, idr_ids, qps_d[t], st["route"])
                elif self.entropy == "gpu":
                    self.h_sizes[k].copy_(self.cav_sizes[k], non_blocking=True)
                else:
                    self.h_hdr[k].copy_(self.hdr[k], non_blocking=True)
                    self.h_coef[k].copy_(self.coef[k], non_blocking=True)
                self.copy_done[k].record(self.copy_stream)
            if cabac_gpu:
                if jj == groups[gi][1] - 1:
                    t0 = groups[gi][0]
                    tw = time.perf_counter()
                    if gi >= 2:
                        a0, an = groups[gi - 2]
                        for tt in range(a0, a0 + an):
                            wrap_futs[tt].result()
                    elif self._ring_last[gi & 1] is not None:
                        for f in self._ring_last[gi & 1][2]:
                            try:
                                f.result()
                            except Exception:
                                pass
                        self._ring_last[gi & 1] = None
                    self.timings["host_blocked_s"] += time.perf_counter() - tw
                    self._gpu_cabac_code(gi, t0, t - t0 + 1, qps_ls_d,
                                         err_to=self.h_err[bno & 1] if gi == ngroups - 1 else None)
                    group_futs[gi] = self.copy_pool.submit(self._copy_out_group, gi, t0, t - t0 + 1, group_copied,
                                                           wrap_futs, steps_pics, groups)
            elif self.entropy == "gpu":
                copy_futs[t] = self.copy_pool.submit(self._copy_out, t, k, pics, copied, wrap_futs)
            else:
                pending[k] = self.pool.submit(self._write_slices, k, t, pics, qpt, idr_ids)
        B_ = B
        counters = torch.stack([self.p_intra_mbs, self.far_ref_mbs, self.sfix_mbs, self.sconv_mbs,
                                self.una_mbs]).to(torch.int64)
        self.p_intra_mbs.zero_()
        self.far_ref_mbs.zero_()
        self.sfix_mbs.zero_()
        self.sconv_mbs.zero_()
        self.una_mbs.zero_()
        h_counters = torch.empty((5,), dtype=torch.int64).pin_memory()
        h_counters.copy_(counters, non_blocking=True)
        h_sse = h_ssim = None
        if metrics:
            h_sse = torch.empty(sse.shape, dtype=sse.dtype).pin_memory()
            h_ssim = torch.empty(ssim.shape, dtype=ssim.dtype).pin_memory()
            h_sse.copy_(sse, non_blocking=True)
            h_ssim.copy_(ssim, non_blocking=True)
        batch_done = torch.cuda.Event()
        batch_done.record(main)
        if cabac_gpu:
            for gi in range(max(0, ngroups - 2), ngroups):
                a0, an = groups[gi]
                self._ring_last[gi & 1] = (group_copied[gi], group_futs[gi], wrap_futs[a0:a0 + an])
        keep = (y, u, v, steps, qps_d, qps_ls_d, orders_d, cuts_d, self._route_dev, self._cmap_dev, self._wp_steps,
                self._la_mv, self._mbtree, sse, ssim, counters, analysis)
        err_h = self.h_err[bno & 1]

        def finish() -> list[SegmentResult]:
            if cabac_gpu:
                for f in group_futs:
                    f.result()
                for t in range(F):
                    outs[t] = wrap_futs[t].result()
            elif self.entropy == "gpu":
                for t in range(F):
                    copy_futs[t].result()
                for t in range(F):
                    outs[t] = wrap_futs[t].result()
            for t in range(max(0, F - 2), F):
                k = t & 1
                if pending[k] is not None:
                    outs[t] = pending[k].result()
                    pending[k] = None
            batch_done.synchronize()
            nonlocal keep
            keep = None
            c = h_counters.numpy()
            if F > 1:
                self.stats["p_intra_ratio"] = float(c[0]) / (B_ * (F - 1) * self.nmb)
                n_p = sum(1 for plan in plans for pic in plan if pic.kind == "P")
                if self.nref > 1 and n_p:
                    self.stats["p_far_ref_ratio"] = float(c[1]) / (n_p * self.nmb)
                nbp = sum(1 for plan in plans for pic in plan if pic.kind == "B")
                self.stats["b_ratio"] = nbp / float(B_ * F)
# ... 66 lines not shown
```

Before: 16930.

## Compute CABAC block nonzero masks inside the inter encode kernel

The inter encode kernel now records per-macroblock nonzero bitmasks for luma 4x4 blocks, chroma DC and chroma AC while it quantizes, writing them to a new mask_pre buffer. The CABAC mask kernel copies those precomputed masks for P/B slots and only rescans coefficients for macroblocks flagged as intra (sentinel bit). This removes a full re-read of the coefficient arrays in the mask pass. The cost is extra ballots and stores in the encode kernel, a double-buffered mask array, and a risk of mask mismatches, which host test bindings are added to check.

Result: no change. 17130, median of 6 (+1.2%).

```diff
diff --git a/csrc/common/h264_cabac.h b/csrc/common/h264_cabac.h
--- a/csrc/common/h264_cabac.h
+++ b/csrc/common/h264_cabac.h
@@ -1069,10 +1069,11 @@
 
 inline size_t cabac_write_slice_data_symbols(const CabacSliceInfo& si, CabacNb* nb, uint8_t* states, CabacBuf* out,
                                              const MbHeader* hdr, const int16_t* coef, int n, uint16_t* syms,
-                                             size_t cap_syms, int* nsyms_out) {
+                                             size_t cap_syms, int* nsyms_out, const uint32_t* masks = nullptr) {
   const int end = si.first_mb + n;
   for (int a = end - 1; a >= si.first_mb; --a)
-    cabac_prepare_mb(si, hdr, a, cabac_block_mask(hdr[a], coef + static_cast<size_t>(a) * kCoefPerMb), nb[a]);
+    cabac_prepare_mb(si, hdr, a,
+                     masks ? masks[a] : cabac_block_mask(hdr[a], coef + static_cast<size_t>(a) * kCoefPerMb), nb[a]);
   cabac_qp_chain(si, nb, n);
   size_t total = 0;
   for (int a = si.first_mb; a < end; ++a) {
diff --git a/csrc/common/h264_mb.h b/csrc/common/h264_mb.h
--- a/csrc/common/h264_mb.h
+++ b/csrc/common/h264_mb.h
@@ -35,6 +35,7 @@
   COEF_CHROMA_AC = 280,
   kCoefPerMb = 408,
 };
+constexpr uint32_t kBlockMaskIntra = 0x80000000u;
 
 enum : uint8_t {
   MBF_SKIP = 1,
diff --git a/csrc/host/bindings.cc b/csrc/host/bindings.cc
--- a/csrc/host/bindings.cc
+++ b/csrc/host/bindings.cc
@@ -10,6 +10,7 @@
 
 #include "../common/h264_enc_math.h"
 #include "annexb.h"
+#include "../common/h264_cabac.h"
 #include "cabac_writer.h"
 #include "cavlc_writer.h"
 #include "cpu_encoder.h"
@@ -696,6 +697,31 @@
     int nsyms = 0;
     std::vector<uint8_t> b = cabac_slice_data_symbols(sps, pps, sh, mh, coef.data(), nmb, &nsyms);
     return py::make_tuple(to_bytes(a), to_bytes(b), nsyms);
+  });
+  m.def("cabac_block_masks", [](py::array_t<uint8_t, py::array::c_style> hdr, py::array_t<int16_t, py::array::c_style> coef) {
+    const py::ssize_t nmb = hdr.size() / static_cast<py::ssize_t>(sizeof(MbHeader));
+    if (hdr.size() != nmb * static_cast<py::ssize_t>(sizeof(MbHeader)) || coef.size() != nmb * kCoefPerMb)
+      throw std::runtime_error("header / coef arrays have wrong sizes");
+    const MbHeader* mh = reinterpret_cast<const MbHeader*>(hdr.data());
+    py::array_t<uint32_t> out(nmb);
+    for (py::ssize_t a = 0; a < nmb; ++a) out.mutable_at(a) = cabac_block_mask(mh[a], coef.data() + a * kCoefPerMb);
+    return out;
+  });
+  m.def("cabac_slice_data_masks", [](const py::dict& cfg, const py::dict& fp, py::array_t<uint8_t, py::array::c_style> hdr,
+                                      py::array_t<int16_t, py::array::c_style> coef,
+                                      py::array_t<uint32_t, py::array::c_style> masks) {
+    EncoderConfig c = cfg_from(cfg);
+    c.cabac = 1;
+    SPS sps = make_sps(c);
+    PPS pps = make_pps(c);
+    int nmb = sps.width_mbs * sps.height_mbs;
+    if (hdr.size() != static_cast<py::ssize_t>(nmb * sizeof(MbHeader))) throw std::runtime_error("header array has wrong size");
+    if (coef.size() != static_cast<py::ssize_t>(nmb) * kCoefPerMb) throw std::runtime_error("coef array has wrong size");
+    if (masks.size() != nmb) throw std::runtime_error("mask array has wrong size");
+    SliceHeader sh = slice_header_from(c, sps, pps, fp);
+    int nsyms = 0;
+    return to_bytes(cabac_slice_data_symbols(sps, pps, sh, reinterpret_cast<const MbHeader*>(hdr.data()), coef.data(), nmb,
+                                             &nsyms, masks.data()));
   });
 
   m.def(
diff --git a/csrc/host/cabac_writer.cc b/csrc/host/cabac_writer.cc
--- a/csrc/host/cabac_writer.cc
+++ b/csrc/host/cabac_writer.cc
@@ -55,7 +55,7 @@
 }
 
 std::vector<uint8_t> cabac_slice_data_symbols(const SPS& sps, const PPS& pps, const SliceHeader& sh, const MbHeader* mbs,
-                                              const int16_t* coef, int num_mbs, int* nsyms) {
+                                              const int16_t* coef, int num_mbs, int* nsyms, const uint32_t* masks) {
   const int nmb = sps.width_mbs * sps.height_mbs;
   CabacSliceInfo si{};
   si.slice_type = sh.slice_type;
@@ -71,7 +71,8 @@
   std::vector<uint8_t> out(static_cast<size_t>(num_mbs) * 4000 + 4096);
   uint8_t states[kCabacContexts];
   CabacBuf buf{out.data(), out.size(), 0, 0};
-  cabac_write_slice_data_symbols(si, nb.data(), states, &buf, mbs, coef, num_mbs, syms.data(), syms.size(), nsyms);
+  cabac_write_slice_data_symbols(si, nb.data(), states, &buf, mbs, coef, num_mbs, syms.data(), syms.size(), nsyms,
+                                 masks);
   if (buf.overflow) throw std::runtime_error("CABAC symbol path overflow");
   out.resize(buf.n);
   return out;
diff --git a/csrc/host/cabac_writer.h b/csrc/host/cabac_writer.h
--- a/csrc/host/cabac_writer.h
+++ b/csrc/host/cabac_writer.h
@@ -16,7 +16,8 @@
                                       const int16_t* coef, int num_mbs, SliceStats* stats = nullptr);
 
 std::vector<uint8_t> cabac_slice_data_symbols(const SPS& sps, const PPS& pps, const SliceHeader& sh, const MbHeader* mbs,
-                                              const int16_t* coef, int num_mbs, int* nsyms);
+                                              const int16_t* coef, int num_mbs, int* nsyms,
+                                              const uint32_t* masks = nullptr);
 
 }
 }
diff --git a/csrc/kernels/bindings_hip.cc b/csrc/kernels/bindings_hip.cc
--- a/csrc/kernels/bindings_hip.cc
+++ b/csrc/kernels/bindings_hip.cc
@@ -89,7 +89,7 @@
                               int bmode, int t8, const int16_t* mv8, void* stream, const int* w1, int nref,
                               const uint8_t* const* xref_u, const uint8_t* const* xref_v, const int8_t* mref,
                               const int* wp, int trellis, float trellis_lambda, const void* route, int nbuf,
-                              uint8_t* qp_flags);
+                              uint8_t* qp_flags, uint32_t* mask_pre);
 void mivc_launch_wp_stats16(const uint16_t* y, const uint16_t* u, const uint16_t* v, int w, int h, int npics,
                             unsigned long long* out, void* stream);
 void mivc_launch_wp_stats(const uint8_t* y, const uint8_t* u, const uint8_t* v, int w, int h, int npics,
@@ -174,7 +174,7 @@
                            int* cnt, long long* off, int* tot, uint16_t* pool, long long pool_cap,
                            long long* pool_used, long long* base, int* total, const int* slot_qp, int slice_type,
                            int num_ref_l0, int num_ref_l1, int t8x8_mode, int* err, void* stream, const void* route,
-                           int slice_rows);
+                           int slice_rows, const uint32_t* pre);
 void mivc_launch_cabac_code(int L, int B, uint16_t* pool, const long long* base, const int* total,
                             const uint32_t* hdr_bits, const int* hdr_nbits, const int* slot_qp,
                             unsigned long long itypes, int* bytes, uint8_t* out, long long* out_off, int* err,
@@ -213,6 +213,7 @@
 PYBIND11_MODULE(_hip, m) {
   m.doc() = "govideocompressor_amd gfx950 kernels (raw-pointer launch shims)";
   m.attr("arch") = "gfx950";
+  m.attr("inter_block_mask") = true;
   m.def("route_bytes", []() { return static_cast<int>(sizeof(mivc::gpu::SlotRoute)); });
 
   m.def("synth", [](uintptr_t y, uintptr_t u, uintptr_t v, int w, int h, int slots, int frames, int frame0,
@@ -427,7 +428,8 @@
            uintptr_t intra_flag, uintptr_t intra_count, uintptr_t stream, uintptr_t aq, uintptr_t ref1_u,
            uintptr_t ref1_v, int bmode, int t8, uintptr_t mv8, std::vector<int> w1, std::vector<uintptr_t> xref_u,
            std::vector<uintptr_t> xref_v, uintptr_t mref, uintptr_t wp, int trellis, float trellis_lambda,
-           uintptr_t route, int nbuf, uintptr_t qp_flags) {
+           uintptr_t route, int nbuf, uintptr_t qp_flags, uintptr_t mask_pre) {
+          if (mask_pre & 3) throw std::invalid_argument("encode_inter: mask_pre must be 4-byte aligned");
           if (bmode && (!ref1_u || !ref1_v)) throw std::invalid_argument("encode_inter: B mode needs the list-1 chroma");
           const size_t n = xref_u.size() + 1;
           if (n > 4 || xref_v.size() != xref_u.size()) throw std::invalid_argument("encode_inter: at most 4 list-0 pictures");
@@ -449,7 +451,7 @@
                                    P<int>(intra_count), P<int8_t>(aq), P<uint8_t>(ref1_u), P<uint8_t>(ref1_v), bmode,
                                    t8, P<int16_t>(mv8), S(stream), w.data(), static_cast<int>(n), xu, xv,
                                    bmode ? nullptr : P<int8_t>(mref), P<int>(wp), trellis, trellis_lambda, P<void>(route),
-                                   nbuf, P<uint8_t>(qp_flags));
+                                   nbuf, P<uint8_t>(qp_flags), P<uint32_t>(mask_pre));
         }, py::arg("B"), py::arg("wmb"), py::arg("hmb"), py::arg("sy"), py::arg("su"), py::arg("sv"), py::arg("fy"),
         py::arg("fu"), py::arg("fv"), py::arg("ry"), py::arg("ru"), py::arg("rv"), py::arg("pred"), py::arg("mv"),
         py::arg("me_cost"), py::arg("intra_cost"), py::arg("qp"), py::arg("cqo"), py::arg("hdr"), py::arg("coef"),
@@ -457,7 +459,8 @@
         py::arg("ref1_u") = 0, py::arg("ref1_v") = 0, py::arg("bmode") = 0, py::arg("t8") = 0, py::arg("mv8") = 0,
         py::arg("w1") = std::vector<int>{32}, py::arg("xref_u") = std::vector<uintptr_t>{},
         py::arg("xref_v") = std::vector<uintptr_t>{}, py::arg("mref") = 0, py::arg("wp") = 0, py::arg("trellis") = 0,
-        py::arg("trellis_lambda") = 1.0f, py::arg("route") = 0, py::arg("nbuf") = 0, py::arg("qp_flags") = 0);
+        py::arg("trellis_lambda") = 1.0f, py::arg("route") = 0, py::arg("nbuf") = 0, py::arg("qp_flags") = 0,
+        py::arg("mask_pre") = 0);
   m.def("wp_stats16", [](uintptr_t y, uintptr_t u, uintptr_t v, int w, int h, int npics, uintptr_t out, uintptr_t stream) {
     if (w % 2 || h % 2 || npics <= 0) throw std::invalid_argument("wp_stats16: even picture sizes, npics > 0");
     mivc_launch_wp_stats16(P<uint16_t>(y), P<uint16_t>(u), P<uint16_t>(v), w, h, npics, P<unsigned long long>(out),
@@ -799,18 +802,19 @@
                         uintptr_t cnt, uintptr_t off, uintptr_t tot, uintptr_t pool, long long pool_cap,
                         uintptr_t pool_used, uintptr_t base, uintptr_t total, uintptr_t slot_qp, int slice_type,
                         int num_ref_l0, int num_ref_l1, int t8x8_mode, uintptr_t err, uintptr_t stream, uintptr_t route,
-                        int slice_rows) {
+                        int slice_rows, uintptr_t pre) {
+    if (pre && !route) throw std::invalid_argument("cabac_bin: pre needs the step's route");
     if ((pool & 15) != 0) throw std::invalid_argument("cabac_bin: symbol pool must be 16-byte aligned");
     if (B < 1 || wmb < 1 || hmb < 1) throw std::invalid_argument("cabac_bin: bad geometry");
     mivc_launch_cabac_bin(B, wmb, hmb, P<void>(hdr), P<int16_t>(coef), P<uint32_t>(mask), P<void>(nb), P<int>(cnt),
                           P<long long>(off), P<int>(tot), P<uint16_t>(pool), pool_cap, P<long long>(pool_used),
                           P<long long>(base), P<int>(total), P<int>(slot_qp), slice_type, num_ref_l0, num_ref_l1,
-                          t8x8_mode, P<int>(err), S(stream), P<void>(route), slice_rows);
+                          t8x8_mode, P<int>(err), S(stream), P<void>(route), slice_rows, P<uint32_t>(pre));
   }, py::arg("B"), py::arg("wmb"), py::arg("hmb"), py::arg("hdr"), py::arg("coef"), py::arg("mask"), py::arg("nb"),
      py::arg("cnt"), py::arg("off"), py::arg("tot"), py::arg("pool"), py::arg("pool_cap"), py::arg("pool_used"),
      py::arg("base"), py::arg("total"), py::arg("slot_qp"), py::arg("slice_type"), py::arg("num_ref_l0"),
      py::arg("num_ref_l1"), py::arg("t8x8_mode"), py::arg("err"), py::arg("stream"), py::arg("route") = 0,
-     py::arg("slice_rows") = 0);
+     py::arg("slice_rows") = 0, py::arg("pre") = 0);
   m.def("cabac_code", [](int L, int B, uintptr_t pool, uintptr_t base, uintptr_t total, uintptr_t hdr_bits,
                          uintptr_t hdr_nbits, uintptr_t slot_qp, unsigned long long itypes, uintptr_t bytes,
                          uintptr_t out, uintptr_t out_off, uintptr_t err, uintptr_t stream, uintptr_t host_out,
diff --git a/csrc/kernels/cabac.hip b/csrc/kernels/cabac.hip
--- a/csrc/kernels/cabac.hip
+++ b/csrc/kernels/cabac.hip
@@ -32,7 +32,9 @@
   int* err;
   const SlotRoute* rt;
   int slice_mbs, per_slot;
+  const uint32_t* pre;
 };
+
 
 __device__ __forceinline__ int slice_first(const CabacBinArgs& a, int mb) { return (mb / a.slice_mbs) * a.slice_mbs; }
 __device__ __forceinline__ int slice_end(const CabacBinArgs& a, int mb) {
@@ -60,16 +62,24 @@
 __global__ __launch_bounds__(64) void cabac_mask(CabacBinArgs a) {
   const Geom& g = a.g;
   const int lane = threadIdx.x, sub = lane & 31;
-  const int slot = blockIdx.y;
+  const int slot = blockIdx.y, nmb = g.nmb();
+  const bool routed = a.pre && a.rt && (a.rt[slot].kind == SK_P || a.rt[slot].kind == SK_B);
+  const int mb_l = blockIdx.x * (2 * kMaskSpan) + lane;
+  const bool mine = lane < 2 * kMaskSpan && mb_l < nmb;
+  const size_t o_l = static_cast<size_t>(slot) * nmb + (mine ? mb_l : 0);
+  const uint32_t pw = (routed && mine) ? a.pre[o_l] : h264::kBlockMaskIntra;
+  if (mine && pw != h264::kBlockMaskIntra) a.mask[o_l] = pw;
+  const unsigned long long need = __ballot(mine && pw == h264::kBlockMaskIntra);
   for (int it = 0; it < kMaskSpan; ++it) {
+  if (((need >> (2 * it)) & 3ull) == 0) continue;
   const int mb = (blockIdx.x * kMaskSpan + it) * 2 + (lane >> 5);
-  if ((blockIdx.x * kMaskSpan + it) * 2 >= g.nmb()) break;
-  const bool live = mb < g.nmb();
-  const size_t o = static_cast<size_t>(slot) * g.nmb() + (live ? mb : 0);
+  const bool rd = (need >> (2 * it + (lane >> 5))) & 1ull;
+  const size_t o = static_cast<size_t>(slot) * nmb + (rd ? mb : 0);
   const int16_t* c = a.coef + o * h264::kCoefPerMb;
-  const bool i16 = a.hdr[o].kind == h264::MBK_I16x16;
+  const bool i16 = rd && a.hdr[o].kind == h264::MBK_I16x16;
   bool nz = false;
-  if (sub < 16 || (sub >= 19 && sub < 27)) {
+  if (!rd) {
+  } else if (sub < 16 || (sub >= 19 && sub < 27)) {
     const int16_t* p = sub < 16 ? c + h264::COEF_LUMA + sub * 16 : c + h264::COEF_CHROMA_AC + (sub - 19) * 16;
     const uint4 q0 = reinterpret_cast<const uint4*>(p)[0];
     const uint4 q1 = reinterpret_cast<const uint4*>(p)[1];
@@ -85,7 +95,7 @@
   }
   const unsigned long long bal = __ballot(nz);
   const uint32_t m = static_cast<uint32_t>((bal >> (lane & 32)) & 0x7FFFFFFull);
-  if (live && sub == 0) a.mask[o] = m;
+  if (rd && sub == 0) a.mask[o] = m;
   }
 }
 
@@ -483,8 +493,10 @@
                                       void* nb, int* cnt, long long* off, int* tot, uint16_t* pool,
                                       long long pool_cap, long long* pool_used, long long* base, int* total,
                                       const int* slot_qp, int slice_type, int num_ref_l0, int num_ref_l1,
-                                      int t8x8_mode, int* err, void* stream, const void* route, int slice_rows) {
+                                      int t8x8_mode, int* err, void* stream, const void* route, int slice_rows,
+                                      const uint32_t* pre) {
   CabacBinArgs a;
+  a.pre = route ? pre : nullptr;
   const int rows = (slice_rows > 0 && slice_rows < hmb) ? slice_rows : hmb;
   a.slice_mbs = rows * wmb;
   a.per_slot = (hmb + rows - 1) / rows;
diff --git a/csrc/kernels/encode_inter.hip b/csrc/kernels/encode_inter.hip
--- a/csrc/kernels/encode_inter.hip
+++ b/csrc/kernels/encode_inter.hip
@@ -37,6 +37,7 @@
   const SlotRoute* rt;
   int nbuf;
   uint8_t* qp_flags;
+  uint32_t* mask_pre;
 };
 
 
@@ -351,10 +352,14 @@
     }
 
     bool any = false;
+    bool lnz = false;
     if (use8_wave) {
       if (use8) {
 #pragma unroll
-        for (int i = 0; i < 16; ++i) lv[i] = keep8 ? lv[i] : 0;
+        for (int i = 0; i < 16; ++i) {
+          lv[i] = keep8 ? lv[i] : 0;
+          lnz |= lv[i] != 0;
+        }
         store_levels(coef + h264::COEF_LUMA + l * 16, lv);
         const int m = qp % 6, q6 = qp / 6;
 #pragma unroll
@@ -391,6 +396,7 @@
         sv[i] = keep4 ? lv[h264::kZigzag4x4[i]] : 0;
         any |= sv[i] != 0;
       }
+      lnz = any;
       store_levels(coef + h264::COEF_LUMA + l * 16, sv);
       int dv[3];
 #pragma unroll
@@ -403,6 +409,10 @@
     if (a.qp_flags) {
       const uint64_t luma_any = __ballot(any);
       if (live && l == 0) a.qp_flags[o] = !work ? 2 : (((luma_any >> (16 * q)) & 0xFFFFu) != 0 ? 1 : 0);
+    }
+    if (a.mask_pre) {
+      const uint64_t luma_nz = __ballot(lnz);
+      if (live && l == 0) a.mask_pre[o] = work ? static_cast<uint32_t>((luma_nz >> (16 * q)) & 0xFFFFu) : h264::kBlockMaskIntra;
     }
     if (work) {
       uint8_t* recy = a.rec_y + rcur * g.ysize() + static_cast<size_t>(Y0 + lby) * W + X0 + lbx;
@@ -557,18 +567,19 @@
   const int score_c = sum4(score);
   const bool keep_ac = score_c >= 7;
   bool any_c = false;
+  bool any_ac = false, any_dc = false;
   if (work) {
     const int f[4] = {d0 + d1 + d2 + d3, d0 - d1 + d2 - d3, d0 + d1 - d2 - d3, d0 - d1 - d2 + d3};
     int cl[4];
 #pragma unroll
     for (int i = 0; i < 4; ++i) cl[i] = h264::quant_coef(f[i], mfc[0], 15 + qpc / 6 + 1, 11);
     int sv[16];
-    bool any_ac = false;
 #pragma unroll
     for (int i = 0; i < 16; ++i) {
       sv[i] = (keep_ac && i > 0) ? lv[h264::kZigzag4x4[i]] : 0;
       any_ac |= sv[i] != 0;
     }
+    any_dc = (cl[0] | cl[1] | cl[2] | cl[3]) != 0;
     store_levels(coef + h264::COEF_CHROMA_AC + (comp * 4 + cb) * 16, sv);
     if (cb == 0) {
       auto p2 = [](int lo, int hi) { return (static_cast<uint32_t>(lo) & 0xFFFFu) | (static_cast<uint32_t>(hi) << 16); };
@@ -580,7 +591,7 @@
 #pragma unroll
     for (int r = 0; r < 16; ++r) res[r] = (keep_ac && r > 0) ? (lv[r] * dvc[h264::kPosClass[r]]) << (qpc / 6) : 0;
     res[0] = ((fcb * ls) << (qpc / 6)) >> 5;
-    const bool any = any_ac || c0 || c1 || c2 || c3;
+    const bool any = any_ac || any_dc;
     any_c = any;
     if (any) h264::inverse_core4x4(res);
     uint8_t* recc = (comp == 0 ? a.rec_u : a.rec_v) + rcur * g.csize() + static_cast<size_t>(my * 8 + cby) * cw + mx * 8 + cbx;
@@ -596,6 +607,12 @@
   if (a.qp_flags) {
     const uint64_t chroma_any = __ballot(any_c);
     if (work && (lane & 7) == 0 && ((chroma_any >> (8 * m)) & 0xFFu) != 0) a.qp_flags[o] = 1;
+  }
+  if (a.mask_pre) {
+    const uint64_t ac_nz = __ballot(any_ac), dc_nz = __ballot(any_dc);
+    const uint32_t ac = static_cast<uint32_t>((ac_nz >> (8 * m)) & 0xFFu), dcb = static_cast<uint32_t>((dc_nz >> (8 * m)) & 0xFFu);
+    const uint32_t bits = (ac << 19) | ((dcb & 1u) << 17) | (((dcb >> 4) & 1u) << 18);
+    if (work && (lane & 7) == 0 && bits) a.mask_pre[o] |= bits;
   }
 }
 
@@ -614,9 +631,10 @@
                                          int t8, const int16_t* mv8, void* stream, const int* w1, int nref,
                                          const uint8_t* const* xref_u, const uint8_t* const* xref_v,
                                          const int8_t* mref, const int* wp, int trellis, float trellis_lambda,
-                                         const void* route, int nbuf, uint8_t* qp_flags) {
+                                         const void* route, int nbuf, uint8_t* qp_flags, uint32_t* mask_pre) {
   InterArgs a;
   a.qp_flags = qp_flags;
+  a.mask_pre = mask_pre;
   a.rt = static_cast<const SlotRoute*>(route);
   a.nbuf = nbuf;
   a.trellis = trellis;
diff --git a/govideocompressor_amd/models/h264_gpu.py b/govideocompressor_amd/models/h264_gpu.py
--- a/govideocompressor_amd/models/h264_gpu.py
+++ b/govideocompressor_amd/models/h264_gpu.py
@@ -335,6 +335,11 @@
             self.aq_terms = torch.zeros((B, nmb), dtype=torch.float32, device=dev)
         self.qp_flags = torch.zeros((B, nmb), dtype=u8, device=dev)
         self.qp_pre = torch.zeros((B, nmb), dtype=u8, device=dev)
+        self._use_mask_pre = True
+        self.mask_pre = None
+        if entropy == "gpu" and params.cabac and hasattr(self.hip, "inter_block_mask"):
+            self.mask_pre = [torch.zeros((B, nmb), dtype=i32, device=dev) for _ in range(2)]
+        self._poison_levels = False
         self.intra_count = torch.zeros((B,), dtype=i32, device=dev)
         self.qp = torch.zeros((B,), dtype=i32, device=dev)
         self.err_bufs = [torch.zeros((1,), dtype=i32, device=dev) for _ in range(2)]
@@ -495,7 +500,7 @@
         tx = tdiv(16384 + abs(tdiv(td, 2)), td)
         return max(-1024, min(1023, (tb * tx + 32) >> 6)), 0
 
-    def _encode_step(self, st: dict, hdr, coef, cut=None):
+    def _encode_step(self, st: dict, hdr, coef, cut=None, mask_pre=None):
         s = self._stream()
         B, wmb, hmb = self.B, self.wmb, self.hmb
         P = self._ptr
@@ -522,6 +527,11 @@
         cqo = self.p.chroma_qp_offset
         inter = st["P"] or st["B"]
         pre = {"qp_flags": P(self.qp_pre)} if (aq and inter and hasattr(self.hip, "prep_aq")) else {}
+        ikw = dict(pre)
+        if mask_pre is not None:
+            ikw.update(mask_pre=P(mask_pre))
+        if self._poison_levels:
+            coef.fill_(0x5A5A)
         if inter:
             self.intra_count.zero_()
         seed0 = seed1 = 0
@@ -585,7 +595,7 @@
                                       P(self.nz), P(self.intra_flag), P(self.intra_count), s, aq,
                                       t8=int(self.p.eff_t8x8()), mv8=mv8, mref=P(self.mref), wp=wp,
                                       trellis=int(self.p.trellis), trellis_lambda=float(self.p.trellis_lambda),
-                                      route=rt, nbuf=NB, **pre)
+                                      route=rt, nbuf=NB, **ikw)
         if st["B"]:
             br = self.p.b_me_range
             spatial = self.p.direct == "spatial"
@@ -634,7 +644,7 @@
                                       P(self.cost_b), P(self.intra_cost), P(self.qp), cqo, P(hdr), P(coef),
                                       P(self.nz), P(self.intra_flag), P(self.intra_count), s, aq, pu, pv, 1,
                                       int(self.p.eff_t8x8()), 0, [32], [], [], 0, 0, int(self.p.trellis),
-                                      float(self.p.trellis_lambda), rt, NB, **pre)
+                                      float(self.p.trellis_lambda), rt, NB, **ikw)
         if inter:
             self.p_intra_mbs += self.intra_count.sum()
             flag_ptr, count_ptr = P(self.intra_flag), P(self.intra_count)
@@ -877,7 +887,7 @@
         return out
 
     def _gpu_cabac_bin(self, k: int, g: int, j: int, t: int, pics: list[PicPlan], qps_t, idr_ids: list[int],
-                       qp_dev: torch.Tensor, route: int):
+                       qp_dev: torch.Tensor, route: int, mask_pre: torch.Tensor | None = None):
         B, BS = self.B, self.B * self.S
         r = g & 1
         if j == 0:
@@ -890,7 +900,8 @@
                            P(self.cab_cnt), P(self.cab_off), P(self.cab_tot), P(self.cab_pool[r]), self.cab_pool_cap,
                            self.cab_pool_used[r].data_ptr(), self.cab_base[r][j * BS:].data_ptr(),
                            self.cab_total[r][j * BS:].data_ptr(), P(qp_dev), pics[0].slice_type, 1, 1,
-                           int(self.p.eff_t8x8()), P(self.err), self.copy_stream.cuda_stream, route, self.slice_rows)
+                           int(self.p.eff_t8x8()), P(self.err), self.copy_stream.cuda_stream, route, self.slice_rows,
+                           **({"pre": P(mask_pre)} if mask_pre is not None else {}))
 
     def _gpu_cabac_code(self, g: int, t0: int, n: int, qps_d: torch.Tensor, err_to: torch.Tensor | None = None):
         BS = self.B * self.S
@@ -1310,7 +1321,9 @@
             self._prep_step(y, u, v, orders[:, t], orders_d[t], st)
             st["disp_d"] = orders_d[t]
             self.qp.copy_(qps_d[t])
-            self._encode_step(st, self.hdr[k], self.coef[k], cuts_d[t] if (t > 0 and cuts_c[:, t].any()) else None)
+            mpre = self.mask_pre[k] if (cabac_gpu and self.mask_pre is not None and self._use_mask_pre) else None
+            self._encode_step(st, self.hdr[k], self.coef[k], cuts_d[t] if (t > 0 and cuts_c[:, t].any()) else None,
+                              mask_pre=mpre)
             if metrics:
                 P = self._ptr
                 self.hip.sse(B, self.W, self.H, self.p.width, self.p.height, P(self.src[0]), P(self.src[1]),
@@ -1331,7 +1344,7 @@
             with torch.cuda.stream(self.copy_stream):
                 self.copy_stream.wait_event(self.compute_done[k])
                 if cabac_gpu:
-                    self._gpu_cabac_bin(k, gi, jj, t, pics, qpt, idr_ids, qps_d[t], st["route"])
+                    self._gpu_cabac_bin(k, gi, jj, t, pics, qpt, idr_ids, qps_d[t], st["route"], mpre)
                 elif self.entropy == "gpu":
                     self.h_sizes[k].copy_(self.cav_sizes[k], non_blocking=True)
                 else:
```
